# YukeWang96/TC-GNN_ATC23

Hardware: AMD Instinct MI355X
Metric: SpMM/SDDMM GTEPS + GCN/AGNN ms/epoch, Reddit h=64, 1xMI355X (higher is better)
Workload: dtype f16 x f16 -> f32 (MFMA), f32 I/O; 1 GPU; reddit-shape synthetic graph N=232965 nnz=114615892, SpMM D=64 (GCN aggregation, fwd = bwd); tc_blocks_16x8=13626429, parallelism=1 GPU

## Files before the change

tc-gnn_atc23_amd/csrc/tcgnn_device.hip:

```cpp
#include <hip/hip_runtime.h>

#include <algorithm>
#include <atomic>
#include <chrono>
#include <cmath>
#include <cstdint>
#include <cstdlib>
#include <cstring>
#include <mutex>
#include <new>
#include <numeric>
#include <type_traits>
#include <vector>

#include "tcgnn.h"
#include "tcgnn_internal.h"

using namespace tcgnn;

#define LDS_AS __attribute__((address_space(3)))
#define GLB_AS __attribute__((address_space(1)))

typedef _Float16 half8 __attribute__((ext_vector_type(8)));
typedef _Float16 half4 __attribute__((ext_vector_type(4)));
typedef float floatx4 __attribute__((ext_vector_type(4)));
typedef __attribute__((__vector_size__(4 * sizeof(__fp16)))) __fp16 fp16x4_raw;

#define HIP_TRY(expr)                                                                       \
    do {                                                                                    \
        hipError_t e_ = (expr);                                                             \
        if (e_ != hipSuccess) return fail(TCGNN_ERR_HIP, "%s -> %s", #expr, hipGetErrorString(e_)); \
    } while (0)
static inline int hip_rc(hipError_t e) { return e == hipErrorOutOfMemory ? TCGNN_ERR_OOM : TCGNN_ERR_HIP; }
template <class T> struct DevBuf {
    T* ptr = nullptr;
    size_t bytes = 0;
    DevBuf() = default;
    DevBuf(DevBuf&& o) noexcept : ptr(o.ptr), bytes(o.bytes) { o.ptr = nullptr; o.bytes = 0; }
    DevBuf& operator=(DevBuf&& o) noexcept { std::swap(ptr, o.ptr); std::swap(bytes, o.bytes); return *this; }
    DevBuf(const DevBuf&) = delete;
    DevBuf& operator=(const DevBuf&) = delete;
    ~DevBuf() { reset(); }
    hipError_t alloc(size_t count) {
        reset();
        const hipError_t e = hipMalloc(&ptr, count * sizeof(T));
        if (e == hipSuccess) bytes = count * sizeof(T); else ptr = nullptr;
        return e;
    }
    void reset() { if (ptr) (void)hipFree(ptr); ptr = nullptr; bytes = 0; }
    size_t release(T*& to) { const size_t b = bytes; to = ptr; ptr = nullptr; bytes = 0; return b; }
    operator T*() const { return ptr; }
};

struct tcgnn_plan {
    int32_t N = 0, nw = 0, nw_eff = 0;
    double near_frac = 0;
    int32_t Nc = 0;
    int32_t row_off = 0;
    int32_t* d_sym = nullptr;
    int64_t E = 0, tc_blocks = 0, total_wb = 0, max_wb = 0;
    int canonical = 0, waves = 1;
    int32_t max_degree = 0;
    const int32_t *rowptr = nullptr, *col = nullptr, *bp = nullptr, *e2c = nullptr, *e2r = nullptr;
    int64_t* d_wb_ptr = nullptr;
    int32_t* d_order = nullptr;
    int32_t* d_cols = nullptr;
    uint32_t* d_mask = nullptr;
    int32_t* d_ebase = nullptr;
    int32_t nbuckets = 0, bucket_rows = 0;
    uint32_t* d_bptr = nullptr;
    int32_t num_cus = 256;
    size_t bytes = 0;
    uint32_t* d_stage = nullptr;
    struct SyncTables {
        int32_t S = 0, R = 0, nwx = 0, kmax = 0, fb_shift = 0;
        uint32_t* d_T = nullptr;
        int32_t* d_nk = nullptr;
        double hot_frac = 0, avg_k = 0;
        int32_t max_k = 0;
        bool ok = false;
    } sync;
    struct CellStream {
        std::atomic<int32_t> nranges{0};
        int32_t nwg = 0;
        int64_t tiles = 0;
        int32_t* d_order = nullptr;
        int32_t npairs = 0;
        int32_t* d_rbase = nullptr;
        int32_t* d_rlist = nullptr;
        uint32_t* d_rl2 = nullptr;
        int32_t dense_entries = 0;
        int64_t cold_tiles = 0, hot_cols = 0, cold_cols = 0, cold_max = 0;
        uint32_t* d_parts = nullptr;
        int32_t nsplit = 0;
        int64_t* d_cold_ptr = nullptr;
        int32_t* d_cold_cols = nullptr;
        uint32_t* d_cold_mask = nullptr;
        uint32_t* d_cell_ptr = nullptr;
        uint32_t* d_cell_tiles = nullptr;
        int32_t flat_tpc = 0;
        uint32_t* d_flat = nullptr;
        int32_t* d_wcold_ptr = nullptr;
        uint32_t* d_wcold = nullptr;
        int32_t* d_eidx = nullptr;
        int32_t* d_cold_eidx = nullptr;
        uint16_t* d_eidx16 = nullptr;
        uint16_t* d_cold_eidx16 = nullptr;
    };
    CellStream lds[7];
    int64_t* d_xwb_ptr = nullptr;
    int32_t* d_xcols = nullptr;
    uint32_t* d_xmask = nullptr;
    int32_t* d_xeidx = nullptr;
    int64_t total_xwb = 0;
    std::atomic<int8_t> val_choice{-1};
    mutable std::atomic<int8_t> lds_choice[65];
    tcgnn_plan() { for (auto& c : lds_choice) c.store(-1, std::memory_order_relaxed); }
    mutable std::vector<hipEvent_t> ev;
    mutable std::atomic<int> ev_used{0};
    mutable std::atomic<const char*> last_kernel{""};
    std::atomic<int8_t> spmm_mode{-1}, range_guard{-1};
    std::vector<int32_t> h_bp;
    mutable std::atomic<int> lds_extra[2] = {{-1}, {-1}};
};

struct KernelTimer {
    const tcgnn_plan* p; hipStream_t s; int slot = -1;
    KernelTimer(const tcgnn_plan* plan, hipStream_t stream, const char* kernel_name = nullptr) : p(plan), s(stream) {
        if (p && kernel_name) p->last_kernel.store(kernel_name, std::memory_order_relaxed);
        if (p && !p->ev.empty()) {
            const int k = p->ev_used.fetch_add(1, std::memory_order_relaxed);
            if (2 * k + 1 < (int)p->ev.size()) { slot = k; (void)hipEventRecord(p->ev[2 * slot], s); }
            else p->ev_used.store((int)p->ev.size() / 2, std::memory_order_relaxed);
        }
    }
    void stop() { if (slot >= 0) { (void)hipEventRecord(p->ev[2 * slot + 1], s); slot = -1; } }
    ~KernelTimer() { stop(); }
};

static inline int round_up(int x, int m) { return (x + m - 1) / m * m; }
static constexpr int kXcds = 8;

__device__ __forceinline__ float relu_if(int on, float v) { return on ? fmaxf(v, 0.0f) : v; }
struct Epi { const float* rs; const float* bias; };
__device__ __forceinline__ float epi_apply(int relu, const Epi& e, int64_t row, int col, float v) {
#pragma clang fp contract(off)
    if (e.rs) v = v * e.rs[row];
    if (e.bias) v = v + e.bias[col];
    return relu_if(relu, v);
}

template <int NT>
struct TileImage {
    static constexpr int C = 2 * NT;
    __device__ static __forceinline__ int slot(int row, int c) {
        if constexpr (NT == 1) {
            int rp = (row & ~0xC) | ((row & 4) << 1) | ((row & 8) >> 1);
            return rp * 2 + c;
        } else if constexpr (NT == 2) {
            return row * 4 + (c ^ (((row >> 3) & 1) << 1));
        } else if constexpr (NT == 4) {
            return row * 8 + (c ^ ((((row >> 1) & 1) << 1) | (((row >> 3) & 1) << 2)));
        } else if constexpr (NT == 8) {
            return row * 16 + (c ^ (((row & 3) | (((row >> 3) & 1) << 2)) << 1));
        } else {
            return row * C + c;
        }
    }
    __device__ static __forceinline__ void unslot(int q, int& row, int& c) {
        if constexpr (NT == 1) {
            int rp = q >> 1;
            row = (rp & ~0xC) | ((rp & 4) << 1) | ((rp & 8) >> 1);
            c = q & 1;
        } else if constexpr (NT == 2) {
            row = q >> 2;
            c = (q & 3) ^ (((row >> 3) & 1) << 1);
        } else if constexpr (NT == 4) {
            row = q >> 3;
            c = (q & 7) ^ ((((row >> 1) & 1) << 1) | (((row >> 3) & 1) << 2));
        } else if constexpr (NT == 8) {
            row = q >> 4;
            c = (q & 15) ^ (((row & 3) | (((row >> 3) & 1) << 2)) << 1);
        } else {
            row = q / C;
            c = q - row * C;
        }
    }
};

__device__ __forceinline__ half4 lds_read_tr16(const char* p) {
    fp16x4_raw v = __builtin_amdgcn_ds_read_tr16_b64_v4f16((LDS_AS fp16x4_raw*)(p));
    return __builtin_bit_cast(half4, v);
}

#include "tcgnn_launch.inc"
#include "tcgnn_stage.inc"
#include "tcgnn_pack.inc"

#include "tcgnn_gather_spmm.inc"
#include "tcgnn_sync_walk.inc"


#include "tcgnn_small_spmm.inc"
#include "tcgnn_lds_spmm.inc"
#include "tcgnn_lds_flat.inc"
#include "tcgnn_lds_val.inc"

#include "tcgnn_sddmm.inc"

#include "tcgnn_agnn.inc"

#include "tcgnn_small_fallback.inc"
#include "tcgnn_heads.inc"

#include "tcgnn_transpose.inc"

#include "tcgnn_edge_softmax.inc"
#include "tcgnn_gat.inc"
#include "tcgnn_segment_max.inc"
#include "tcgnn_segment_stats.inc"
#include "tcgnn_gatv2.inc"

static const char* test_knob(const char* name) { return getenv(name); }
static int verbose_level() { const char* e = getenv("TCGNN_VERBOSE"); return e ? atoi(e) : 0; }
static constexpr int g_bucket_min_tiles = 2;
static int g_lds_auto = [] { const char* e = test_knob("TCGNN_LDS_AUTO"); return e ? atoi(e) : 1; }();
#ifdef TCGNN_DEBUG_TIMERS
static int g_lds_dbg = [] { const char* e = getenv("TCGNN_LDS_DBG"); return e ? atoi(e) : 0; }();
#else
static constexpr int g_lds_dbg = 0;
#endif
static constexpr int g_lds_fill_quota = 1;
static int g_spmm_mode = [] { const char* e = getenv("TCGNN_SPMM_MODE"); return e ? atoi(e) : 0; }();
static inline int spmm_mode_of(const tcgnn_plan* p) { const int m = p ? (int)p->spmm_mode.load(std::memory_order_relaxed) : -1; return m >= 0 ? m : g_spmm_mode; }
static constexpr size_t kBlockedMinBytes = 6u << 20;
static constexpr size_t kRangeTargetBytes = 1u << 20;

static constexpr int kAgnnMaxSlices = 16;
static size_t agnn_partial_bytes(const tcgnn_plan* plan) {
    const size_t slots = std::max<size_t>((size_t)std::max(plan->nw_eff, 1), (size_t)kAgnnMaxSlices * (((size_t)std::max(plan->nw_eff, 1) + 3) / 4));
    return (slots * sizeof(double) + 255) / 256 * 256;
}

static bool has_locality(const tcgnn_plan* plan) { return plan->near_frac > 0.5; }
static bool windows_balanced(const tcgnn_plan* plan) {
    return plan->nw_eff > 0 && plan->max_wb * (int64_t)plan->nw_eff <= 8 * std::max<int64_t>(plan->total_wb, 1);
}
static bool ranges_fit_l2(const tcgnn_plan* plan, size_t x16_bytes) {
    return plan->nbuckets > 0 && x16_bytes / (size_t)plan->nbuckets <= ((size_t)8 << 20) && plan->nw_eff >= 32 * plan->num_cus;
}
static bool range_walk_pays(const tcgnn_plan* plan, size_t x16_bytes) {
    return x16_bytes > kBlockedMinBytes && windows_balanced(plan) && ranges_fit_l2(plan, x16_bytes) && !has_locality(plan);
}
static int range_count(const tcgnn_plan* plan, size_t x16_bytes, size_t range_bytes) {
    if (const char* e = test_knob("TCGNN_RANGE_KB")) range_bytes = (size_t)atol(e) << 10;
    int nranges = 1;
    while (nranges < plan->nbuckets && x16_bytes / nranges > range_bytes) nranges <<= 1;
    return nranges;
}
static int check_output_aligned(const char* call, const char* what, const void* p) {
    if (reinterpret_cast<uintptr_t>(p) & 15) return fail(TCGNN_ERR_INVALID_ARG, "%s: %s must be 16-byte aligned, got %p", call, what, p);
    return TCGNN_OK;
// ... 201 lines not shown
```

tc-gnn_atc23_amd/csrc/tcgnn_lds_flat.inc:

```

struct SpmmFlatArgs {
    const uint32_t* blocks;
    const int32_t* order;
    const _Float16* x16;
    const uint32_t* hdr;
    float* y;
    int32_t N, D, stride , chunk0, xrows, nw, nwg;
    int32_t dbg, relu;
    const int32_t* rbase;
    const uint32_t* rl2;
    int32_t nent;
    const float* w;
    int32_t dout, accumulate;
    int32_t fill_quota;
    const int32_t* wcold_ptr;
    const uint32_t* wcold;
    SpmmSmallArgs fb;
};

typedef uint32_t uintx2 __attribute__((ext_vector_type(2)));

template <int T> struct FlatMeta { uint32_t idw[T]; uint32_t mk[(T + 3) / 4]; };
template <int T> __device__ __forceinline__ void flat_meta_block(uint32_t idaddr, uint32_t maddr, FlatMeta<T>& m) {
    if constexpr (T == 8) {
// ... 6 lines not shown
#pragma unroll
        for (int k = 0; k < 4; ++k) { m.idw[k] = q0[k]; m.idw[4 + k] = q1[k]; }
        m.mk[0] = b[0]; m.mk[1] = b[1];
    } else if constexpr (T == 4) {
        uintx4 q0; uint32_t b;
        asm volatile("ds_read_b128 %0, %2\n\t"
                     "ds_read_b32 %1, %3\n\t"
                     "s_waitcnt lgkmcnt(0)"
                     : "=&v"(q0), "=&v"(b) : "v"(idaddr), "v"(maddr) : "memory");
#pragma unroll
        for (int k = 0; k < 4; ++k) m.idw[k] = q0[k];
        m.mk[0] = b;
    } else {
        static_assert(T == 16, "flat streams: 4, 8 or 16 tiles per wavefront and range");
        uintx4 q0, q1, q2, q3, b;
        asm volatile("ds_read_b128 %0, %5\n\t"
                     "ds_read_b128 %1, %5 offset:16\n\t"
                     "ds_read_b128 %2, %5 offset:32\n\t"
                     "ds_read_b128 %3, %5 offset:48\n\t"
                     "ds_read_b128 %4, %6\n\t"
                     "s_waitcnt lgkmcnt(0)"
                     : "=&v"(q0), "=&v"(q1), "=&v"(q2), "=&v"(q3), "=&v"(b) : "v"(idaddr), "v"(maddr) : "memory");
#pragma unroll
        for (int k = 0; k < 4; ++k) { m.idw[k] = q0[k]; m.idw[4 + k] = q1[k]; m.idw[8 + k] = q2[k]; m.idw[12 + k] = q3[k]; m.mk[k] = b[k]; }
    }
}

template <int NT, int PLANE> __device__ __forceinline__ void flat_issue(uint32_t ad0, uint32_t ad1, half4* nlo, half4* nhi) {
    if constexpr (NT == 1) lds_flat_issue1<PLANE>(ad0, ad1, nlo, nhi);
    else if constexpr (NT == 2) lds_flat_issue2<PLANE>(ad0, ad1, nlo, nhi);
    else if constexpr (NT == 3) lds_flat_issue3<PLANE>(ad0, ad1, nlo, nhi);
    else lds_flat_issue4<PLANE>(ad0, ad1, nlo, nhi);
}
template <int NT, int PLANE> __device__ __forceinline__ void flat_step(uint32_t ad0, uint32_t ad1, half4* nlo, half4* nhi, half4* clo, half4* chi) {
    if constexpr (NT == 1) lds_flat_step1<PLANE>(ad0, ad1, nlo, nhi, clo, chi);
    else if constexpr (NT == 2) lds_flat_step2<PLANE>(ad0, ad1, nlo, nhi, clo, chi);
    else if constexpr (NT == 3) lds_flat_step3<PLANE>(ad0, ad1, nlo, nhi, clo, chi);
    else lds_flat_step4<PLANE>(ad0, ad1, nlo, nhi, clo, chi);
}
template <int NT, int PLANE> __device__ __forceinline__ void flat_step_if(uint32_t on, uint32_t ad0, uint32_t ad1, half4* nlo, half4* nhi, half4* clo, half4* chi) {
    if constexpr (NT == 1) lds_flat_step_if1<PLANE>(on, ad0, ad1, nlo, nhi, clo, chi);
    else if constexpr (NT == 2) lds_flat_step_if2<PLANE>(on, ad0, ad1, nlo, nhi, clo, chi);
    else if constexpr (NT == 3) lds_flat_step_if3<PLANE>(on, ad0, ad1, nlo, nhi, clo, chi);
    else lds_flat_step_if4<PLANE>(on, ad0, ad1, nlo, nhi, clo, chi);
}
template <int NT> __device__ __forceinline__ void flat_drain(half4* clo, half4* chi) {
    if constexpr (NT == 1) lds_flat_drain1(clo, chi);
    else if constexpr (NT == 2) lds_flat_drain2(clo, chi);
    else if constexpr (NT == 3) lds_flat_drain3(clo, chi);
    else lds_flat_drain4(clo, chi);
}

template <int B> __device__ __forceinline__ half8 flat_afrag(uint32_t mkw) {
    const uint32_t mm = __builtin_amdgcn_perm(mkw, mkw, 0x0c000c00u | (uint32_t)B | ((uint32_t)B << 16));
    uintx4 q;
#pragma unroll
    for (int j = 0; j < 4; ++j) {
        const ushort2v k = {(unsigned short)(1u << (14 - 2 * j)), (unsigned short)(1u << (13 - 2 * j))};
        q[j] = __builtin_bit_cast(uint32_t, (ushort2v)(__builtin_bit_cast(ushort2v, mm) * k)) & 0x40004000u;
    }
    return __builtin_bit_cast(half8, q);
}

typedef short short2v __attribute__((ext_vector_type(2)));
template <int B> __device__ __forceinline__ half8 flat_amask(uint32_t mkw) {
    const uint32_t mm = __builtin_amdgcn_perm(mkw, mkw, 0x0c000c00u | (uint32_t)B | ((uint32_t)B << 16));
    uintx4 q;
#pragma unroll
    for (int j = 0; j < 4; ++j) {
        const ushort2v k = {(unsigned short)(1u << (15 - 2 * j)), (unsigned short)(1u << (14 - 2 * j))};
        const short2v sh = __builtin_bit_cast(short2v, (ushort2v)(__builtin_bit_cast(ushort2v, mm) * k)) >> (short2v){15, 15};
        q[j] = __builtin_bit_cast(uint32_t, sh);
    }
    return __builtin_bit_cast(half8, q);
}

__global__ __launch_bounds__(256) void flat_transpose_kernel(const uint32_t* __restrict__ tiles, uint32_t* __restrict__ blocks, int64_t nblocks, int32_t T,
                                                             const uint32_t* __restrict__ rl2 = nullptr) {
    const int64_t k = (int64_t)blockIdx.x * blockDim.x + threadIdx.x;
    const int words = 32 * T;
    if (k >= nblocks * words) return;
    const int64_t blk = k / words;
    if (rl2 && (rl2[(blk / kLdsWaves) * 4] >> 31)) { blocks[k] = tiles[k]; return; }
    const int o = (int)(k - blk * words);
    const uint32_t* src = tiles + blk * words;
    uint32_t v;
    if (o < 16 * T) {
        const int c = o / T, x = o % T;
        v = src[x * 32 + c];
    } else {
        v = 0u;
        const int b0 = (o - 16 * T) * 4;
#pragma unroll
        for (int q = 0; q < 4; ++q) {
            const int b = b0 + q, lane = b / T, x = b % T;
            const int g = lane >> 4, i = lane & 15;
            v |= ((src[x * 32 + 16 + i] >> (8 * g)) & 0xffu) << (8 * q);
        }
    }
    blocks[k] = v;
}

__global__ __launch_bounds__(256) void flat_cold_records_kernel(const uint32_t* __restrict__ list, int64_t n, const int32_t* __restrict__ ccols, const uint32_t* __restrict__ cmask,
                                                                uint32_t* __restrict__ rec) {
    const int64_t k = (int64_t)blockIdx.x * blockDim.x + threadIdx.x;
    if (k >= n * 64) return;
    const uint32_t e = list[k >> 6];
    const int64_t t = e & 0x0fffffffu;
    const int o = (int)(k & 63);
    rec[k] = o < 32 ? ((uint32_t)ccols[t * kWbCols + o] | (e & 0xf0000000u)) : (o < 48 ? cmask[t * kWinRows + (o - 32)] : 0u);
}

__device__ __forceinline__ uint32_t lane_id_now() {
    uint32_t l;
    asm volatile("v_mbcnt_lo_u32_b32 %0, -1, 0\n\tv_mbcnt_hi_u32_b32 %0, -1, %0" : "=v"(l));
    return l;
}

template <int NT, int BR>
struct FlatRangeFiller {
    static constexpr int IPP = BR / 32, TOTAL = NT * IPP, kMinFillers = 12, MAXC = (TOTAL + kMinFillers - 1) / kMinFillers;
    __amdgpu_buffer_rsrc_t xrsrc;
    uint32_t zrow;
    int rank, nfill, plane0, nplanes, xrows;
    __device__ __forceinline__ FlatRangeFiller(const _Float16* x16p, int xrows_, int plane0_, int nplanes_, int rank_, int nfill_, int lane) {
        xrsrc = __builtin_amdgcn_make_buffer_rsrc((void*)x16p, (short)32, nplanes_ * xrows_, 0x00020000);
        zrow = (uint32_t)(xrows_ - 1);
        (void)lane;
        rank = rank_; nfill = nfill_; plane0 = plane0_; nplanes = nplanes_; xrows = xrows_;
    }
    __device__ __forceinline__ void fill(int r0, uint32_t buf) const {
        if (rank < 0) return;
        const uint32_t l2 = lane_id_now();
        const uint32_t lrow = l2 >> 1;
        const int hoff = (int)(l2 & 1u) * 16;
#pragma unroll
        for (int q = 0; q < MAXC; ++q) {
            const int k = rank + nfill * q;
            if (k < TOTAL) {
                const int plane = k / IPP, blk = k - plane * IPP;
                const bool real_plane = plane0 + plane < nplanes;
                const uint32_t row = (uint32_t)(blk * 32) + lrow;
                const uint32_t want = (uint32_t)r0 + row;
                const uint32_t srow = (row < (uint32_t)(BR - 8) && real_plane && want < zrow) ? want : zrow;
                const int pbase = real_plane ? (plane0 + plane) * xrows : 0;
                __builtin_amdgcn_struct_ptr_buffer_load_lds(xrsrc, (LDS_AS void*)(uintptr_t)(buf + (uint32_t)plane * (BR * 32u) + (uint32_t)blk * 1024u), 16,
                                                            pbase + (int)srow, hoff, 0, 0, 0);
            }
        }
    }
};

static constexpr bool flat_dense_ok(int nt, int maxw, int tpc) { return tpc == 1 && nt <= 2 && maxw * tpc <= 15; }
static constexpr int flat_lds_main(int nt, int maxw, int tpc) { return 2 * nt * lds_buf_rows(nt, maxw) * 32 + kLdsWaves * 2 * (maxw * tpc * 128); }
static constexpr bool flat_cold_fits(int nt, int maxw, int tpc) { return flat_lds_main(nt, maxw, tpc) + kLdsWaves * nt * 1024 <= 160 * 1024; }
static constexpr int flat_lds_bytes(int nt, int maxw, int tpc) { return flat_lds_main(nt, maxw, tpc) + (flat_cold_fits(nt, maxw, tpc) ? kLdsWaves * nt * 1024 : (flat_dense_ok(nt, maxw, tpc) ? 128 : 0)); }

#define TCGNN_KERNEL_NAME spmm_lds_flat_kernel
#define TCGNN_KERNEL_PARAM const SpmmFlatArgs a
#define TCGNN_KERNEL_PROLOGUE
#define TCGNN_KERNEL_STORE(relu, row, col, v) relu_if(relu, v)
#include "tcgnn_lds_flat_kernel.inc"
#undef TCGNN_KERNEL_NAME
#undef TCGNN_KERNEL_PARAM
#undef TCGNN_KERNEL_PROLOGUE
#undef TCGNN_KERNEL_STORE
struct SpmmFlatEpiArgs { SpmmFlatArgs a; Epi epi; };
#define TCGNN_KERNEL_NAME spmm_lds_flat_epi_kernel
#define TCGNN_KERNEL_PARAM const SpmmFlatEpiArgs e
#define TCGNN_KERNEL_PROLOGUE const SpmmFlatArgs& a = e.a;
#define TCGNN_KERNEL_STORE(relu, row, col, v) epi_apply(relu, e.epi, row, col, v)
#include "tcgnn_lds_flat_kernel.inc"
#undef TCGNN_KERNEL_NAME
#undef TCGNN_KERNEL_PARAM
#undef TCGNN_KERNEL_PROLOGUE
#undef TCGNN_KERNEL_STORE

template __global__ void spmm_lds_flat_kernel<1, 4, 1, false, false>(const SpmmFlatArgs);
template __global__ void spmm_lds_flat_kernel<1, 4, 1, false, true>(const SpmmFlatArgs);
template __global__ void spmm_lds_flat_kernel<2, 4, 1, false, false>(const SpmmFlatArgs);
template __global__ void spmm_lds_flat_kernel<2, 4, 1, false, true>(const SpmmFlatArgs);
template __global__ void spmm_lds_flat_kernel<3, 4, 1, false, false>(const SpmmFlatArgs);
template __global__ void spmm_lds_flat_kernel<4, 4, 1, false, false>(const SpmmFlatArgs);
template __global__ void spmm_lds_flat_kernel<1, 8, 1, false, false>(const SpmmFlatArgs);
template __global__ void spmm_lds_flat_kernel<1, 8, 1, false, true>(const SpmmFlatArgs);
template __global__ void spmm_lds_flat_kernel<2, 8, 1, false, false>(const SpmmFlatArgs);
template __global__ void spmm_lds_flat_kernel<2, 8, 1, false, true>(const SpmmFlatArgs);
template __global__ void spmm_lds_flat_kernel<1, 4, 2, false, false>(const SpmmFlatArgs);
template __global__ void spmm_lds_flat_kernel<2, 4, 2, false, false>(const SpmmFlatArgs);
template __global__ void spmm_lds_flat_kernel<3, 4, 2, false, false>(const SpmmFlatArgs);
template __global__ void spmm_lds_flat_kernel<4, 4, 2, false, false>(const SpmmFlatArgs);
template __global__ void spmm_lds_flat_kernel<1, 8, 2, false, false>(const SpmmFlatArgs);
template __global__ void spmm_lds_flat_kernel<2, 8, 2, false, false>(const SpmmFlatArgs);
#ifdef TCGNN_DEBUG_TIMERS
template __global__ void spmm_lds_flat_kernel<1, 4, 1, true, false>(const SpmmFlatArgs);
template __global__ void spmm_lds_flat_kernel<1, 4, 1, true, true>(const SpmmFlatArgs);
template __global__ void spmm_lds_flat_kernel<2, 4, 1, true, false>(const SpmmFlatArgs);
template __global__ void spmm_lds_flat_kernel<2, 4, 1, true, true>(const SpmmFlatArgs);
template __global__ void spmm_lds_flat_kernel<3, 4, 1, true, false>(const SpmmFlatArgs);
template __global__ void spmm_lds_flat_kernel<4, 4, 1, true, false>(const SpmmFlatArgs);
template __global__ void spmm_lds_flat_kernel<1, 8, 1, true, false>(const SpmmFlatArgs);
template __global__ void spmm_lds_flat_kernel<1, 8, 1, true, true>(const SpmmFlatArgs);
template __global__ void spmm_lds_flat_kernel<2, 8, 1, true, false>(const SpmmFlatArgs);
template __global__ void spmm_lds_flat_kernel<2, 8, 1, true, true>(const SpmmFlatArgs);
template __global__ void spmm_lds_flat_kernel<1, 4, 2, true, false>(const SpmmFlatArgs);
template __global__ void spmm_lds_flat_kernel<2, 4, 2, true, false>(const SpmmFlatArgs);
template __global__ void spmm_lds_flat_kernel<3, 4, 2, true, false>(const SpmmFlatArgs);
template __global__ void spmm_lds_flat_kernel<4, 4, 2, true, false>(const SpmmFlatArgs);
template __global__ void spmm_lds_flat_kernel<1, 8, 2, true, false>(const SpmmFlatArgs);
template __global__ void spmm_lds_flat_kernel<2, 8, 2, true, false>(const SpmmFlatArgs);
#endif

template __global__ void spmm_lds_flat_epi_kernel<1, 4, 1, false, false>(const SpmmFlatEpiArgs);
template __global__ void spmm_lds_flat_epi_kernel<1, 4, 1, false, true>(const SpmmFlatEpiArgs);
template __global__ void spmm_lds_flat_epi_kernel<2, 4, 1, false, false>(const SpmmFlatEpiArgs);
template __global__ void spmm_lds_flat_epi_kernel<2, 4, 1, false, true>(const SpmmFlatEpiArgs);
template __global__ void spmm_lds_flat_epi_kernel<3, 4, 1, false, false>(const SpmmFlatEpiArgs);
template __global__ void spmm_lds_flat_epi_kernel<4, 4, 1, false, false>(const SpmmFlatEpiArgs);
template __global__ void spmm_lds_flat_epi_kernel<1, 8, 1, false, false>(const SpmmFlatEpiArgs);
template __global__ void spmm_lds_flat_epi_kernel<1, 8, 1, false, true>(const SpmmFlatEpiArgs);
template __global__ void spmm_lds_flat_epi_kernel<2, 8, 1, false, false>(const SpmmFlatEpiArgs);
template __global__ void spmm_lds_flat_epi_kernel<2, 8, 1, false, true>(const SpmmFlatEpiArgs);
template __global__ void spmm_lds_flat_epi_kernel<1, 4, 2, false, false>(const SpmmFlatEpiArgs);
template __global__ void spmm_lds_flat_epi_kernel<2, 4, 2, false, false>(const SpmmFlatEpiArgs);
template __global__ void spmm_lds_flat_epi_kernel<3, 4, 2, false, false>(const SpmmFlatEpiArgs);
template __global__ void spmm_lds_flat_epi_kernel<4, 4, 2, false, false>(const SpmmFlatEpiArgs);
template __global__ void spmm_lds_flat_epi_kernel<1, 8, 2, false, false>(const SpmmFlatEpiArgs);
template __global__ void spmm_lds_flat_epi_kernel<2, 8, 2, false, false>(const SpmmFlatEpiArgs);

static constexpr LaunchGeom flat_geom(int nt, int maxw, int tpc) { return {kLdsWaves * 64, flat_lds_bytes(nt, maxw, tpc), kLdsWaves / 4, maxw}; }

template <int NT, int MAXW, int TPC, bool DBG, bool WITH_DENSE>
static hipError_t launch_flat_dbg(const SpmmFlatArgs& args, int nchunks, hipStream_t stream, const Epi& epi) {
    constexpr LaunchGeom g = flat_geom(NT, MAXW, TPC);
    const dim3 grid((unsigned)args.nwg, (unsigned)nchunks);
    if constexpr (DBG) return launch_kernel<spmm_lds_flat_kernel<NT, MAXW, TPC, true, WITH_DENSE>, g.lds_bytes>(grid, g, stream, args);
    else return launch_plain_or_twin<spmm_lds_flat_kernel<NT, MAXW, TPC, false, WITH_DENSE>, spmm_lds_flat_epi_kernel<NT, MAXW, TPC, false, WITH_DENSE>, g.lds_bytes>(grid, g, stream, args, epi);
}
template <int NT, int MAXW, int TPC, bool DBG>
static hipError_t launch_flat_dense(const SpmmFlatArgs& args, int nchunks, hipStream_t stream, bool dense, const Epi& epi) {
    if constexpr (flat_dense_ok(NT, MAXW, TPC)) {
        if (dense) return launch_flat_dbg<NT, MAXW, TPC, DBG, true>(args, nchunks, stream, epi);
    }
    return launch_flat_dbg<NT, MAXW, TPC, DBG, false>(args, nchunks, stream, epi);
}
template <int NT, int MAXW, int TPC>
static hipError_t launch_flat_one(const SpmmFlatArgs& args, int nchunks, hipStream_t stream, bool dense, const Epi& epi) {
#ifdef TCGNN_DEBUG_TIMERS
    if (args.dbg) return launch_flat_dense<NT, MAXW, TPC, true>(args, nchunks, stream, dense, epi);
#endif
    return launch_flat_dense<NT, MAXW, TPC, false>(args, nchunks, stream, dense, epi);
}
template <int TPC>
static hipError_t launch_flat_tpc(int maxw, int nt, const SpmmFlatArgs& args, int nchunks, hipStream_t stream, bool dense, const Epi& epi) {
    if (maxw == kLdsMaxW2) return with_width<2>(nt, [&](auto NT) { return launch_flat_one<NT, kLdsMaxW2, TPC>(args, nchunks, stream, dense, epi); });
    return with_width<4>(nt, [&](auto NT) { return launch_flat_one<NT, kLdsMaxW, TPC>(args, nchunks, stream, dense, epi); });
}
static hipError_t launch_flat_any(int maxw, int nt, int tpc, const SpmmFlatArgs& args, int nchunks, hipStream_t stream, bool dense,
                                  const Epi& epi = Epi{nullptr, nullptr}) {
    return tpc == 2 ? launch_flat_tpc<2>(maxw, nt, args, nchunks, stream, dense, epi) : launch_flat_tpc<1>(maxw, nt, args, nchunks, stream, dense, epi);
}

struct ColdPlanarArgs {
    const int64_t* cold_ptr;
    const int32_t* ccols;
    const uint32_t* cmask;
    const _Float16* x16;
    const uint32_t* hdr;
    float* y;
    int32_t N, D, xrows, nw, col0, ncols, relu;
    Epi epi;
};
__global__ __launch_bounds__(256, 2) void spmm_cold_planar_kernel(const ColdPlanarArgs a) {
    const int lane = threadIdx.x & 63, wave = threadIdx.x >> 6;
    const int w = blockIdx.x * 4 + wave;
    if (w >= a.nw) return;
    const int64_t t0 = a.cold_ptr[w], t1 = a.cold_ptr[w + 1];
    if (t0 == t1 && !a.relu && !a.epi.rs && !a.epi.bias) return;
    const int r = lane >> 2, q = lane & 3;
    const int plane = (a.col0 >> 4) + (int)blockIdx.y * 4 + q;
    const bool live = plane * 16 < a.col0 + a.ncols && plane * 16 < ((a.D + 15) & ~15);
    float acc[16];
#pragma unroll
    for (int e = 0; e < 16; ++e) acc[e] = 0.0f;
    const int zrow = a.xrows - 1;
    const half8* xp = reinterpret_cast<const half8*>(a.x16 + (int64_t)(live ? plane : 0) * a.xrows * 16);
    int32_t cv = 0; uint32_t mv = 0u;
    if (t0 < t1) { cv = a.ccols[t0 * kWbCols + (lane & 31)]; mv = a.cmask[t0 * kWinRows + r]; }
    for (int64_t t = t0; t < t1; ++t) {
    if (range_is_wide(a.hdr, 0)) return;
        int32_t cvn = 0; uint32_t mvn = 0u;
        if (t + 1 < t1) { cvn = a.ccols[(t + 1) * kWbCols + (lane & 31)]; mvn = a.cmask[(t + 1) * kWinRows + r]; }
        while (__any(mv != 0u)) {
            int c[2];
#pragma unroll
            for (int it = 0; it < 2; ++it) {
                const bool v = mv != 0u;
                const int k = v ? __builtin_ctz(mv) : 0;
                mv &= mv - 1u;
                const int cc = __shfl(cv, k);
                c[it] = (v && live && cc < zrow) ? cc : zrow;
            }
            half8 x[2][2];
#pragma unroll
            for (int it = 0; it < 2; ++it) { x[it][0] = xp[(int64_t)c[it] * 2]; x[it][1] = xp[(int64_t)c[it] * 2 + 1]; }
#pragma unroll
            for (int it = 0; it < 2; ++it)
#pragma unroll
                for (int e = 0; e < 8; ++e) { acc[e] += (float)x[it][0][e]; acc[8 + e] += (float)x[it][1][e]; }
        }
        cv = cvn; mv = mvn;
    }
    const int64_t row = (int64_t)w * kWinRows + r;
    if (!live || row >= a.N) return;
    const float inv = pow2f(-scale_exp_from_bits(a.hdr[kHdrMaxX]));
    float* dst = a.y + row * a.D + plane * 16;
    if (plane * 16 + 16 <= a.D && (a.D & 3) == 0) {
#pragma unroll
        for (int e4 = 0; e4 < 4; ++e4) {
            float4 v = reinterpret_cast<float4*>(dst)[e4];
            const int c0 = plane * 16 + 4 * e4;
            v.x = epi_apply(a.relu, a.epi, row, c0, v.x + acc[4 * e4] * inv); v.y = epi_apply(a.relu, a.epi, row, c0 + 1, v.y + acc[4 * e4 + 1] * inv);
            v.z = epi_apply(a.relu, a.epi, row, c0 + 2, v.z + acc[4 * e4 + 2] * inv); v.w = epi_apply(a.relu, a.epi, row, c0 + 3, v.w + acc[4 * e4 + 3] * inv);
            reinterpret_cast<float4*>(dst)[e4] = v;
        }
    } else {
#pragma unroll
        for (int e = 0; e < 16; ++e)
            if (plane * 16 + e < a.D) dst[e] = epi_apply(a.relu, a.epi, row, plane * 16 + e, dst[e] + acc[e] * inv);
    }
}
```

tc-gnn_atc23_amd/csrc/tcgnn_lds_flat_kernel.inc:

```
template <int NT, int MAXW, int TPC, bool DBG, bool WITH_DENSE>
__global__ __launch_bounds__(kLdsWaves * 64) void TCGNN_KERNEL_NAME(TCGNN_KERNEL_PARAM) {
    TCGNN_KERNEL_PROLOGUE
    if (range_is_wide(a.hdr, 0)) { lds_own_fallback(a.fb); return; }
    const int dbg = DBG ? a.dbg : 0;
    constexpr int kLdsBufRows = lds_buf_rows(NT, MAXW), kLdsRows = kLdsBufRows - 8;
    constexpr int T = MAXW * TPC, PADB = T * 128, kLdsChunkDims = lds_chunk_dims(MAXW);
    static_assert(NT * MAXW <= 16, "accumulators: NT * MAXW * 4 VGPRs");
    extern __shared__ __attribute__((aligned(16))) char smem[];
    constexpr int PLANEB = kLdsBufRows * 32, BUFB = NT * PLANEB;
    const int lane = threadIdx.x & 63;
    const int wave = __builtin_amdgcn_readfirstlane(threadIdx.x >> 6);
    const int g = lane >> 4, i = lane & 15;
    const int wg = blockIdx.x;
    const int chunk_id = a.chunk0 + (int)blockIdx.y;
    const int coloff = chunk_id * kLdsChunkDims;
    const uint32_t lds0 = (uint32_t)(uintptr_t)((LDS_AS char*)smem);
    const uint32_t pad0 = lds0 + 2 * BUFB + (uint32_t)wave * (2 * PADB);
    const int kx = scale_exp_from_bits(a.hdr[kHdrMaxX]);

    floatx4 acc[MAXW][NT];
#pragma unroll
    for (int j = 0; j < MAXW; ++j) {
#pragma unroll
        for (int s = 0; s < NT; ++s) acc[j][s] = floatx4{0.f, 0.f, 0.f, 0.f};
    }
    const bool last_valid = MAXW == 1 || __builtin_amdgcn_readfirstlane(a.order[cell_position(wg, wave, MAXW - 1, MAXW)]) >= 0;
    const uint32_t last_on = (uint32_t)__builtin_amdgcn_readfirstlane(last_valid ? 1 : 0);
    const uint32_t lanebase = lds0 + (uint32_t)(i & 3) * 8u;
    const uint32_t idoff = (uint32_t)(4 * g + (i >> 2)) * (uint32_t)(T * 4);
    const uint32_t moff = (uint32_t)(64 * T) + (uint32_t)lane * (uint32_t)T;
    int fill_rank = wave, fill_n = kLdsWaves;
    {
        LDS_AS uint32_t* flags = (LDS_AS uint32_t*)smem;
        if (lane == 0) flags[wave] = last_valid ? 1u : 0u;
        __syncthreads();
        const uint32_t full = (uint32_t)(__ballot(lane < kLdsWaves && flags[lane < kLdsWaves ? lane : 0] != 0u) & 0xffffull);
        __syncthreads();
        const uint32_t light = ~full & 0xffffu;
        const int nlight = __builtin_popcount(light);
        if (nlight >= FlatRangeFiller<NT, kLdsBufRows>::kMinFillers && nlight < kLdsWaves && a.fill_quota) {
            fill_n = nlight;
            fill_rank = last_valid ? -1 : __builtin_popcount(light & ((1u << wave) - 1u));
        }
    }
    const FlatRangeFiller<NT, kLdsBufRows> filler(a.x16, a.xrows, chunk_id * (kLdsChunkDims / 16), a.stride, fill_rank, fill_n, lane);
    const int rb = a.rbase[wg], nr = a.rbase[wg + 1] - rb;
    const char* const bb0 = reinterpret_cast<const char*>(a.blocks) + ((int64_t)rb * kLdsWaves + wave) * PADB;
    const uint32_t lane16 = (uint32_t)lane * 16u;
    auto meta_dma = [&](int r, uint32_t padaddr) {
        const char* src = bb0 + (int64_t)r * (kLdsWaves * PADB);
#pragma unroll
        for (int q = 0; q < (PADB + 1023) / 1024; ++q)
            if (lane16 + 1024u * q < (uint32_t)PADB)
                __builtin_amdgcn_global_load_lds((GLB_AS const void*)(src + 1024 * q + lane16), (LDS_AS void*)(uintptr_t)(padaddr + 1024u * q), 16, 0, 0);
    };
    const uint32_t* const rlp = a.rl2 + (int64_t)rb * 4;
    auto load_info = [&](int r_) -> uintx2 { return *reinterpret_cast<const uintx2*>(rlp + (int64_t)r_ * 4); };
    const uint32_t* const dscp = a.rl2 + (int64_t)a.nent * 4 + ((int64_t)rb * kLdsWaves + wave);
    auto load_desc = [&](int r_) -> uint32_t { return dscp[(int64_t)r_ * kLdsWaves]; };
    constexpr bool DENSE = WITH_DENSE && flat_dense_ok(NT, MAXW, TPC);

    constexpr bool CAN_COLD = flat_cold_fits(NT, MAXW, TPC);
    const uint32_t cbuf = lds0 + (uint32_t)flat_lds_main(NT, MAXW, TPC) + (uint32_t)wave * (NT * 1024u);
    int cold_c = 0, cold_n = 0, j_cur = 0;
    bool have_g = false, have_n = false;
    uint32_t cid_n = 0u, mw_n = 0u, mw_cur = 0u;
    auto cold_request = [&]() {
        have_n = cold_c < cold_n;
        if (have_n) {
            const uint32_t* rec = a.wcold + (int64_t)cold_c * 64;
            const uint32_t l2 = lane_id_now();
            cid_n = rec[l2 >> 1]; mw_n = rec[32 + (l2 & 15u)];
            ++cold_c;
        }
    };
    auto cold_step = [&]() {
        if (have_g) {
            const uint32_t l2 = lane_id_now();
            const uint32_t ad0 = cbuf + ((l2 >> 4) * 8u + ((l2 & 15u) >> 2)) * 32u + (l2 & 3u) * 8u;
            half4 lo[NT], hi[NT];
            flat_issue<NT, 1024>(ad0, ad0 + 128u, lo, hi);
            flat_drain<NT>(lo, hi);
            const half8 af = afrag_from_byte((mw_cur >> (8 * g)) & 0xffu);
            floatx4 cacc[NT];
#pragma unroll
            for (int s = 0; s < NT; ++s) {
                const half8 bf = __builtin_shufflevector(lo[s], hi[s], 0, 1, 2, 3, 4, 5, 6, 7);
                cacc[s] = __builtin_amdgcn_mfma_f32_16x16x32_f16(af, bf, floatx4{0.f, 0.f, 0.f, 0.f}, 0, 0, 0);
            }
#pragma unroll
            for (int jj = 0; jj < MAXW; ++jj) {
                if (j_cur == jj) {
#pragma unroll
                    for (int s = 0; s < NT; ++s) acc[jj][s] += cacc[s];
                }
            }
        }
        have_g = have_n;
        if (have_n) {
            const int plane0 = chunk_id * (kLdsChunkDims / 16);
#pragma unroll
            for (int s = 0; s < NT; ++s) {
                const bool real = plane0 + s < a.stride;
                const int64_t recrow = real ? (int64_t)(plane0 + s) * a.xrows + (int64_t)(cid_n & 0x0fffffffu) : (int64_t)a.xrows - 1;
                const char* src = reinterpret_cast<const char*>(a.x16) + (recrow << 5) + (lane & 1) * 16;
                __builtin_amdgcn_global_load_lds((GLB_AS const void*)src, (LDS_AS void*)(uintptr_t)(cbuf + (uint32_t)s * 1024u), 16, 0, 0);
            }
            mw_cur = mw_n;
            j_cur = __builtin_amdgcn_readfirstlane((int)(cid_n >> 28));
        }
        cold_request();
    };
    if constexpr (CAN_COLD) {
        if (a.wcold_ptr) {
            cold_c = a.wcold_ptr[wg * kLdsWaves + wave];
            cold_n = a.wcold_ptr[wg * kLdsWaves + wave + 1];
            cold_request();
        }
    }
    uint32_t ew0 = 0u, ew1 = 0u, ew2 = ~0u;
    uintx2 einfo = {0u, ~0u};
    if (nr > 0) {
        const uintx2 e0 = load_info(0);
        ew0 = (uint32_t)__builtin_amdgcn_readfirstlane((int)e0[0]);
        ew2 = (uint32_t)__builtin_amdgcn_readfirstlane((int)e0[1]);
        meta_dma(0, pad0);
        if (nr > 1) meta_dma(1, pad0 + PADB);
        filler.fill((int)(ew0 & 0x3fffffffu) * kLdsRows, lds0);
        einfo = load_info(nr > 1 ? 1 : 0);
    }
    wait_vm0();
    __syncthreads();
    uint32_t ph[4] = {0, 0, 0, 0};
    uint32_t buf = 0u;
    int r = 0;
    uint32_t t0 = 0u, t1 = 0u, t2 = 0u;
    auto entry_top = [&]() {
        t0 = (dbg & 16) ? (uint32_t)__builtin_readcyclecounter() : 0u;
        if (ew2 != ~0u && !(dbg & 1)) filler.fill((int)((dbg & 128) ? (ew2 & 7u) : ew2) * kLdsRows, lds0 + (buf ^ 1u) * BUFB);
        t1 = (dbg & 16) ? (uint32_t)__builtin_readcyclecounter() : 0u;
    };
    uint32_t dnext = 0u;
    auto entry_end = [&](uint32_t padaddr, bool dense_phase) {
        t2 = (dbg & 16) ? (uint32_t)__builtin_readcyclecounter() : 0u;
        wait_vm0();
        const bool more = r + 2 < nr;
        ew0 = (uint32_t)__builtin_amdgcn_readfirstlane((int)einfo[0]);
        ew2 = (uint32_t)__builtin_amdgcn_readfirstlane((int)einfo[1]);
        if (dense_phase) ew1 = (uint32_t)__builtin_amdgcn_readfirstlane((int)dnext);
        if (ew0 & 0x40000000u) buf ^= 1u;
        if constexpr (CAN_COLD) { if (have_g || have_n) cold_step(); }
        if (more) {
            einfo = load_info(r + 2);
            if (dense_phase) dnext = load_desc(r + 2);
            if (!(dbg & 4)) meta_dma(r + 2, padaddr);
        }
        const uint32_t t3 = (dbg & 16) ? (uint32_t)__builtin_readcyclecounter() : 0u;
        if (!(dbg & 8)) __builtin_amdgcn_s_barrier();
        if (dbg & 16) { const uint32_t t4 = (uint32_t)__builtin_readcyclecounter(); ph[0] += t1 - t0; ph[1] += t2 - t1; ph[2] += t3 - t2; ph[3] += t4 - t3; }
    };
    for (; r < nr && !(ew0 >> 31); ++r) {
        entry_top();
        const uint32_t padaddr = pad0 + (uint32_t)(r & 1) * PADB, bb = lanebase + buf * BUFB;
        if (!(dbg & 2)) {
            FlatMeta<T> m;
            flat_meta_block<T>(padaddr + idoff, padaddr + moff, m);
            constexpr bool PIPE = NT <= 3;
            constexpr int SETS = PIPE ? 2 : 1;
            half4 lo[SETS][NT], hi[SETS][NT];
            if constexpr (PIPE) flat_issue<NT, PLANEB>(bb + (m.idw[0] & 0xffffu), bb + (m.idw[0] >> 16), lo[0], hi[0]);
#pragma unroll
            for (int x = 0; x < T; ++x) {
                if (x / TPC == MAXW - 1 && !last_valid) break;
                if (x % TPC == 0 && !(dbg & 32)) set_wave_priority(3 - (x / TPC) * 4 / MAXW);
                const int cs = PIPE ? (x & 1) : 0;
                if constexpr (!PIPE) { flat_issue<NT, PLANEB>(bb + (m.idw[x] & 0xffffu), bb + (m.idw[x] >> 16), lo[0], hi[0]); flat_drain<NT>(lo[0], hi[0]); }
                else if (x + 1 < T && (x + 1) / TPC == MAXW - 1 && x / TPC != MAXW - 1)
                    flat_step_if<NT, PLANEB>(last_on, bb + (m.idw[x + 1] & 0xffffu), bb + (m.idw[x + 1] >> 16), lo[(x + 1) & 1], hi[(x + 1) & 1], lo[cs], hi[cs]);
                else if (x + 1 < T) flat_step<NT, PLANEB>(bb + (m.idw[x + 1] & 0xffffu), bb + (m.idw[x + 1] >> 16), lo[(x + 1) & 1], hi[(x + 1) & 1], lo[cs], hi[cs]);
                else flat_drain<NT>(lo[cs], hi[cs]);
                half8 af;
                switch (x & 3) {
                    case 0: af = flat_afrag<0>(m.mk[x >> 2]); break;
                    case 1: af = flat_afrag<1>(m.mk[x >> 2]); break;
                    case 2: af = flat_afrag<2>(m.mk[x >> 2]); break;
                    default: af = flat_afrag<3>(m.mk[x >> 2]); break;
                }
#pragma unroll
                for (int s = 0; s < NT; ++s) {
                    const half8 bf = __builtin_shufflevector(lo[cs][s], hi[cs][s], 0, 1, 2, 3, 4, 5, 6, 7);
                    acc[x / TPC][s] = __builtin_amdgcn_mfma_f32_16x16x32_f16(af, bf, acc[x / TPC][s], 0, 0, 0);
                }
            }
        }
        entry_end(padaddr, false);
    }
    if constexpr (DENSE) {
    if (__builtin_expect(r < nr, 0)) {
        const uint32_t d0 = load_desc(r), d1 = load_desc(r + 1 < nr ? r + 1 : r);
        wait_vm0();
        ew1 = (uint32_t)__builtin_amdgcn_readfirstlane((int)d0);
        dnext = d1;
    }
    for (; __builtin_expect(r < nr, 0); ++r) {
        entry_top();
        const uint32_t padaddr = pad0 + (uint32_t)(r & 1) * PADB, bb = lanebase + buf * BUFB;
        if (!(dbg & 2)) {
            const uint32_t l2 = lane_id_now();
            const uint32_t gd = l2 >> 4, id_ = l2 & 15u;
            uint32_t idaddr = padaddr + (4u * gd + (id_ >> 2)) * 4u, maddr = padaddr + 64u + id_ * 4u + gd, idw, mb;
            lds_cell_ids(idaddr, maddr, idw, mb);
#pragma unroll
            for (int j = 0; j < MAXW; ++j) {
                const int nj = (int)((ew1 >> (4 * j)) & 15u);
                if (nj) {
                    floatx4 cacc[NT];
#pragma unroll
                    for (int s = 0; s < NT; ++s) cacc[s] = floatx4{0.f, 0.f, 0.f, 0.f};
                    for (int t = 0; t < nj; ++t) {
                        const uint32_t ad0 = bb + (idw & 0xffffu), ad1 = bb + (idw >> 16);
                        const half8 af = afrag_from_byte(mb);
                        half4 lo[NT], hi[NT];
                        uint32_t nidw, nmb;
                        lds_cell_block<NT, PLANEB>(ad0, ad1, idaddr, maddr, lo, hi, nidw, nmb);
#pragma unroll
                        for (int s = 0; s < NT; ++s) {
                            const half8 bf = __builtin_shufflevector(lo[s], hi[s], 0, 1, 2, 3, 4, 5, 6, 7);
                            cacc[s] = __builtin_amdgcn_mfma_f32_16x16x32_f16(af, bf, cacc[s], 0, 0, 0);
                        }
                        idw = nidw; mb = nmb;
                        idaddr += 128u; maddr += 128u;
                    }
#pragma unroll
                    for (int s = 0; s < NT; ++s) acc[j][s] += cacc[s];
                }
            }
        }
        entry_end(padaddr, true);
    }
    }
    if (!(dbg & 32)) __builtin_amdgcn_s_setprio(0);
    if constexpr (CAN_COLD) {
        while (have_g || have_n) { wait_vm0(); cold_step(); }
    }
    if (dbg & 16) {
        if (wg == 0 && blockIdx.y == 0 && lane == 0) {
#pragma unroll
            for (int k = 0; k < 4; ++k) a.y[wave * 8 + k] = (float)ph[k];
            a.y[wave * 8 + 7] = (float)(nr * T);
        }
        return;
    }

    const float inv1 = pow2f(-kx - 1);
    int wj[MAXW];
#pragma unroll
    for (int j = 0; j < MAXW; ++j) wj[j] = __builtin_amdgcn_readfirstlane(a.order[cell_position(wg, wave, j, MAXW)]);
    if (a.w) {
        __syncthreads();
        constexpr int DIN = NT * 16, LDP = DIN + 1;
        float* scratch = reinterpret_cast<float*>(smem) + wave * (16 * LDP);
        const int din = a.D - coloff < DIN ? a.D - coloff : DIN;
        const int tiles = (a.dout + 15) >> 4;
#pragma unroll
        for (int j = 0; j < MAXW; ++j) {
            if (wj[j] < 0) continue;
            __builtin_amdgcn_fence(__ATOMIC_RELEASE, "wavefront"); __builtin_amdgcn_wave_barrier();
#pragma unroll
            for (int s = 0; s < NT; ++s)
#pragma unroll
                for (int ii = 0; ii < 4; ++ii) scratch[(4 * g + ii) * LDP + 16 * s + i] = acc[j][s][ii] * inv1;
            __builtin_amdgcn_fence(__ATOMIC_RELEASE, "wavefront"); __builtin_amdgcn_wave_barrier();
            const int64_t row0 = (int64_t)wj[j] * kWinRows + 4 * g;
            for (int t = 0; t < tiles; ++t) {
                const floatx4 c = dense_update_tile(scratch, LDP, din, a.w, coloff, a.dout, t, g, i);
                const int colg = 16 * t + i;
                if (colg < a.dout) {
#pragma unroll
                    for (int ii = 0; ii < 4; ++ii) {
                        if (row0 + ii >= a.N) continue;
                        float* dst = a.y + (row0 + ii) * (int64_t)a.dout + colg;
                        if (a.accumulate) atomicAdd(dst, c[ii]);
                        else *dst = relu_if(a.relu, c[ii]);
                    }
                }
            }
        }
        return;
    }
#pragma unroll
    for (int j = 0; j < MAXW; ++j) {
        if (wj[j] < 0) continue;
        const int64_t row0 = (int64_t)wj[j] * kWinRows + 4 * g;
#pragma unroll
        for (int s = 0; s < NT; ++s) {
            const int colg = coloff + 16 * s + i;
            if (colg < a.D) {
#pragma unroll
                for (int ii = 0; ii < 4; ++ii)
                    if (row0 + ii < a.N) a.y[(row0 + ii) * a.D + colg] = TCGNN_KERNEL_STORE(a.relu, row0 + ii, colg, acc[j][s][ii] * inv1);
            }
        }
    }
}
```

tc-gnn_atc23_amd/csrc/tcgnn_lds_plan.inc:

```
static int g_lds_maxw = [] { const char* e = test_knob("TCGNN_LDS_MAXW"); const int v = e ? atoi(e) : 0; return (v == 4 || v == 8) ? v : 0; }();
struct LdsPass { int maxw, nt, chunk0, nchunks; };
static int lds_passes(int dpad, LdsPass (&passes)[2]) {
    int n = 0;
    if (g_lds_maxw) {
        const int cd = lds_chunk_dims(g_lds_maxw);
        if (dpad / cd) passes[n++] = {g_lds_maxw, cd / 16, 0, dpad / cd};
        if (dpad % cd) passes[n++] = {g_lds_maxw, (dpad % cd) / 16, dpad / cd, 1};
    } else {
        const int full = dpad / 64, rem = (dpad % 64) / 16;
        if (full || rem == 3) passes[n++] = {kLdsMaxW2, 2, 0, 2 * (full + (rem == 3 ? 1 : 0))};
        if (rem && rem != 3) passes[n++] = {kLdsMaxW, rem, full, 1};
    }
    return n;
}
static bool lds_has_hubs(const tcgnn_plan* p) {
    int64_t mx = 0;
    for (int w = 0; w < p->nw_eff; ++w) mx = std::max<int64_t>(mx, p->h_bp[(size_t)w]);
    return mx * p->nw_eff > 4 * std::max<int64_t>(p->tc_blocks, 1);
}
enum { kPlaceLocal = 0, kPlaceLocalSplit = 1, kPlaceGlobal = 2 };
static int lds_place_forced() {
    const char* env = test_knob("TCGNN_LDS_PLACE");
    if (!env) return -1;
    return !strcmp(env, "global") ? kPlaceGlobal : (!strcmp(env, "localsplit") ? kPlaceLocalSplit : kPlaceLocal);
}
static int lds_buf_rows_for_maxw(int maxw) { return maxw == kLdsMaxW2 ? 768 : 512; }
static double lds_window_weight(const tcgnn_plan* p, int w, double nranges_d) {
    const double cols = 8.0 * std::max(p->h_bp[(size_t)w], 1);
    return std::ceil(cols / 32.0 + nranges_d * (1.0 - std::exp(-cols / nranges_d)));
}
static int lds_workgroups_unsplit(const tcgnn_plan* p, int maxw, int extra_slots) {
    const int per_wg = kLdsWaves * maxw;
    const int64_t slots = (int64_t)p->nw_eff + extra_slots;
    int nwg = (int)((slots + per_wg - 1) / per_wg);
    const int cu_target = maxw == kLdsMaxW2 ? std::max(1, p->num_cus / 2) : p->num_cus;
    if (nwg < cu_target) nwg = std::max(nwg, std::min(cu_target, (p->nw_eff + kLdsWaves - 1) / kLdsWaves));
    return nwg;
}
static constexpr int kLdsMaxParts = 8, kLdsMaxFollowers = 32;
static int lds_split_parts(const tcgnn_plan* p, int maxw, std::vector<uint8_t>* parts, const std::vector<double>* exact = nullptr) {
    const int nw = p->nw_eff;
    if (parts) parts->assign((size_t)nw, 1);
    if (nw <= 0 || !lds_has_hubs(p)) return 0;
    const double nranges_d = std::max(1.0, std::ceil((double)p->Nc / (lds_buf_rows_for_maxw(maxw) - 8)));
    auto weight = [&](int w) { return exact ? (*exact)[(size_t)w] : lds_window_weight(p, w, nranges_d); };
    double total = 0;
    for (int w = 0; w < nw; ++w) total += weight(w);
    const double share = total / ((double)lds_workgroups_unsplit(p, maxw, 0) * kLdsWaves);
    int extra = 0;
    for (int w = 0; w < nw; ++w) {
        const double wt = weight(w);
        if (wt <= 1.5 * share) continue;
        const int k = (int)std::min<double>(kLdsMaxParts, std::ceil(wt / share));
        if (k < 2) continue;
        if (parts) (*parts)[(size_t)w] = (uint8_t)k;
        extra += k - 1;
    }
    return extra;
}
static int lds_workgroups(const tcgnn_plan* p, int maxw) {
    const int which = maxw == kLdsMaxW2 ? 1 : 0;
    int extra = p->lds_extra[which].load(std::memory_order_relaxed);
    if (extra < 0) { extra = lds_split_parts(p, maxw, nullptr); p->lds_extra[which].store(extra, std::memory_order_relaxed); }
    return lds_workgroups_unsplit(p, maxw, extra);
}

static double lds_estimate_us(const tcgnn_plan* p, int dpad) {
    LdsPass passes[2];
    const int np = lds_passes(dpad, passes);
    const double cols_per_window = 32.0 * (double)p->total_wb / std::max(p->nw_eff, 1);
    double t = 25.0;
    for (int i = 0; i < np; ++i) {
        const int maxw = passes[i].maxw, nt = passes[i].nt;
        const int rows = lds_stream_buf_rows(lds_stream_of(nt, maxw)) - 8;
        const double nranges = std::ceil((double)p->Nc / rows);
        const int nwg = lds_workgroups(p, maxw);
        const double rounds = std::ceil((double)nwg * passes[i].nchunks / std::max(p->num_cus, 1));
        const double c = cols_per_window / nranges;
        const double tiles_per_cell = c <= 24.0 ? 1.0 - std::exp(-c) : c / 32.0 + 0.5;
        const double windows_per_wave = (double)p->nw_eff / ((double)nwg * kLdsWaves);
        static const double fixed4[4] = {0.47, 0.60, 0.89, 1.16};
        const double a = maxw == kLdsMaxW2 ? 0.80 : fixed4[std::min(nt, 4) - 1];
        t += rounds * nranges * (a + 0.135 * windows_per_wave * tiles_per_cell);
    }
    return t;
}
static double gather_estimate_us(const tcgnn_plan* p, int dpad) {
    const double image = ((double)p->Nc + 1) * x16_pitch(dpad) * 2.0;
    double ps;
    if (image <= (double)kBlockedMinBytes) ps = 4.6 + std::max(0, dpad - 16) * (1.8 / 48.0);
    else if (dpad <= 32) ps = 8.5;
    else if (dpad <= 64) ps = 8.5 + (dpad - 32) * (1.1 / 32.0);
    else ps = 9.6 + (dpad - 64) * (6.9 / 64.0);
    if (image > 45.0e6) ps *= std::pow(image / 45.0e6, 0.3);
    return 20.0 + (double)p->E * ps * 1e-6;
}
static bool lds_chosen(const tcgnn_plan* p, int dpad) {
    if (!g_lds_auto || p->nw_eff <= 0 || p->total_wb <= 0) return false;
    const int k = dpad / 16;
    if (k <= 64 && p->lds_choice[k] >= 0) return p->lds_choice[k] != 0;
    LdsPass passes[2];
    const int np = lds_passes(dpad, passes);
    double cells = 0;
    for (int i = 0; i < np; ++i) {
        const int rows = lds_stream_buf_rows(lds_stream_of(passes[i].nt, passes[i].maxw)) - 8;
        cells += (double)lds_workgroups(p, passes[i].maxw) * kLdsWaves * passes[i].maxw * std::ceil((double)p->Nc / rows);
    }
    const bool yes = cells < 2.0e8 && lds_estimate_us(p, dpad) <= 0.95 * gather_estimate_us(p, dpad);
    if (k <= 64) p->lds_choice[k] = yes ? 1 : 0;
    return yes;
}

static bool lds_deal_workgroup(int g, int maxw, const std::vector<int32_t>& items, const std::vector<uint8_t>& k, const std::vector<double>& wt,
                               std::vector<int32_t>& order, std::vector<uint32_t>& parts_out, int& nsplit) {
    double load[kLdsWaves] = {0};
    int used[kLdsWaves] = {0};
    uint32_t next_fol = 0;
    for (const int32_t w : items) {
        const int kk = k.empty() ? 1 : k[(size_t)w];
        uint32_t taken = 0u;
        const uint32_t fol0 = next_fol;
        for (int part = 0; part < kk; ++part) {
            int best = -1;
            for (int v = 0; v < kLdsWaves; ++v)
                if (used[v] < maxw && !((taken >> v) & 1u) && (best < 0 || load[v] < load[best])) best = v;
            if (best < 0)
                for (int v = 0; v < kLdsWaves; ++v) if (used[v] < maxw && (best < 0 || load[v] < load[best])) best = v;
            if (best < 0) return false;
            const size_t pos = (size_t)cell_position(g, best, used[best], maxw);
            order[pos] = w;
            if (kk > 1) parts_out[pos] = (uint32_t)part | ((uint32_t)kk << 8) | ((part == 0 ? fol0 : fol0 + (uint32_t)part - 1u) << 16);
            taken |= 1u << best;
            load[best] += wt[(size_t)w] / kk;
            ++used[best];
        }
        if (kk > 1) { next_fol += (uint32_t)kk - 1u; ++nsplit; }
    }
    return true;
}
static bool lds_place_windows(const tcgnn_plan* p, int nwg, int maxw, std::vector<int32_t>& order, std::vector<uint32_t>& parts_out, int& nsplit,
                              const std::vector<double>& exact, int mode) {
    const int nw = p->nw_eff, cap = kLdsWaves * maxw;
    order.assign((size_t)nwg * cap, -1);
    parts_out.clear();
    nsplit = 0;
    if (mode == kPlaceGlobal) {
        std::vector<uint8_t> k;
        const int extra = lds_split_parts(p, maxw, &k, &exact);
        const std::vector<double>& wt = exact;
        std::vector<int32_t> idx((size_t)nw);
        std::iota(idx.begin(), idx.end(), 0);
        std::stable_sort(idx.begin(), idx.end(), [&](int32_t x, int32_t y) { return wt[(size_t)x] > wt[(size_t)y]; });
        std::vector<double> wg_load((size_t)nwg, 0.0);
        std::vector<int> wg_free((size_t)nwg, cap), wg_fol((size_t)nwg, 0);
// ... 16 lines not shown
        if (extra > 0) parts_out.assign((size_t)nwg * cap, 0u); else k.clear();
        for (int g = 0; g < nwg; ++g)
            if (!lds_deal_workgroup(g, maxw, wg_items[(size_t)g], k, wt, order, parts_out, nsplit)) return false;
        if (nsplit == 0) parts_out.clear();
        return true;
    }
    const std::vector<double>& wt = exact;
    double total = 0;
    for (int w = 0; w < nw; ++w) total += wt[(size_t)w];
    std::vector<uint8_t> k;
    const int extra = mode == kPlaceLocalSplit ? lds_split_parts(p, maxw, &k, &exact) : 0;
    if (extra > 0) {
        int64_t slots = 0;
        for (int w = 0; w < nw; ++w) slots += k[(size_t)w];
        for (int level = kLdsMaxParts; slots > (int64_t)nwg * cap && level > 1; --level)
            for (int w = 0; w < nw && slots > (int64_t)nwg * cap; ++w)
                if (k[(size_t)w] == level) { --k[(size_t)w]; --slots; }
        parts_out.assign((size_t)nwg * cap, 0u);
    } else k.clear();
    std::vector<int64_t> slots_after((size_t)nw + 1, 0);
    for (int w = nw - 1; w >= 0; --w) slots_after[(size_t)w] = slots_after[(size_t)w + 1] + (k.empty() ? 1 : k[(size_t)w]);
    std::vector<int32_t> blk;
    double acc = 0;
    int wg = 0, blk_slots = 0, blk_fol = 0;
    bool ok = true;
    auto deal = [&]() {
        double mx = 0, sum = 0;
        for (const int32_t w : blk) { mx = std::max(mx, wt[(size_t)w]); sum += wt[(size_t)w]; }
        if (mx * (double)blk.size() > 1.5 * sum) {
            const double heavy = 2.0 * sum / (double)blk.size();
            auto mid = std::stable_partition(blk.begin(), blk.end(), [&](int32_t x) { return wt[(size_t)x] > heavy; });
            std::stable_sort(blk.begin(), mid, [&](int32_t x, int32_t y) { return wt[(size_t)x] > wt[(size_t)y]; });
        }
        ok = lds_deal_workgroup(wg, maxw, blk, k, wt, order, parts_out, nsplit) && ok;
        blk.clear(); blk_slots = 0; blk_fol = 0;
    };
    for (int w = 0; w < nw && ok; ++w) {
        int kk = k.empty() ? 1 : k[(size_t)w];
        const int wgs_left0 = nwg - (wg + 1);
        if (kk > 1 && blk_fol + kk - 1 > kLdsMaxFollowers) { k[(size_t)w] = 1; kk = 1; }
        if (blk_slots + kk > cap) {
            if (wgs_left0 > 0 && slots_after[(size_t)w] <= (int64_t)wgs_left0 * cap) { deal(); ++wg; }
            else { if (kk > 1) k[(size_t)w] = 1; kk = 1; }
            if (blk_slots + kk > cap) { ok = false; break; }
        }
        blk.push_back(w);
        blk_slots += kk; blk_fol += kk - 1;
        acc += wt[(size_t)w];
        const int wgs_left = nwg - (wg + 1);
        const bool full = blk_slots == cap;
        const bool heavy_enough = acc >= total * (double)(wg + 1) / nwg;
        if (wgs_left > 0 && (full || (heavy_enough && slots_after[(size_t)w + 1] <= (int64_t)wgs_left * cap))) { deal(); ++wg; }
    }
    if (ok && !blk.empty()) deal();
    if (nsplit == 0) parts_out.clear();
    return ok;
}


struct CellPlacement {
    int mode = kPlaceLocal, nsplit = 0;
    uint32_t hot_min = 1u;
    double est_us = 0;
    std::vector<int32_t> sorder;
    std::vector<uint32_t> sparts, paircols, pairmax, pairover, pairtiles;
    DevBuf<uint32_t> d_cellcols, d_firstq, d_parts;
    DevBuf<int32_t> d_sorder;
};
struct FlatEntries {
    std::vector<int32_t> ent2, nd, wg_first;
    std::vector<uint32_t> xbase, rl2;
    int64_t nentries = 0;
};
static FlatEntries flat_entries(int nwg, int maxw, const std::vector<int32_t>& rbase, const std::vector<int32_t>& rlist, const std::vector<uint32_t>& cnt,
                                const std::vector<uint32_t>& dense_mx, bool dense_on, bool records) {
    FlatEntries f;
    const int64_t npairs = rbase[(size_t)nwg];
    f.ent2.assign((size_t)npairs * 2 + 2, -1); f.nd.assign((size_t)npairs, 0); f.wg_first.assign((size_t)nwg + 1, 0);
    int32_t eidx = 0;
    for (int wg = 0; wg < nwg; ++wg) {
        f.wg_first[(size_t)wg] = eidx;
        for (int64_t k = rbase[(size_t)wg]; k < rbase[(size_t)wg + 1]; ++k) f.ent2[(size_t)k * 2] = eidx++;
        for (int64_t k = rbase[(size_t)wg]; k < rbase[(size_t)wg + 1]; ++k) {
            f.nd[(size_t)k] = dense_on ? (int32_t)((dense_mx[(size_t)k] + maxw - 1) / maxw) : 0;
            f.ent2[(size_t)k * 2 + 1] = f.nd[(size_t)k] ? eidx : -1;
            eidx += f.nd[(size_t)k];
        }
    }
    f.wg_first[(size_t)nwg] = eidx;
    f.nentries = eidx;
    if (!records) return f;
    const std::vector<int32_t>& nd = f.nd;
    std::vector<uint32_t>& xbase = f.xbase;
    if (dense_on) {
        xbase.assign((size_t)(npairs * kLdsWaves * maxw), 0u);
        for (int64_t k = 0; k < npairs; ++k) {
            if (!nd[(size_t)k]) continue;
            for (int v = 0; v < kLdsWaves; ++v) {
                uint32_t run = 0;
                for (int j = 0; j < maxw; ++j) { const size_t c = (size_t)((k * kLdsWaves + v) * maxw + j); xbase[c] = run; run += cnt[c] > 1u ? cnt[c] - 1u : 0u; }
            }
        }
    }
    const int64_t nrec = std::max<int64_t>(f.nentries, 1);
    f.rl2.assign((size_t)nrec * (4 + kLdsWaves), 0u);
    auto put = [&](int64_t en, int v, uint32_t w0, uint32_t w1, uint32_t w2) {
        uint32_t* q = &f.rl2[(size_t)(en * 4)];
        q[0] = w0; q[1] = w2; q[3] = 0u;
        f.rl2[(size_t)(nrec * 4 + en * kLdsWaves + v)] = w1;
    };
    for (int wg = 0; wg < nwg; ++wg)
        for (int64_t en = f.wg_first[(size_t)wg]; en < f.wg_first[(size_t)wg + 1]; ++en) f.rl2[(size_t)(en * 4 + 2)] = (uint32_t)(rbase[(size_t)wg + 1] - rbase[(size_t)wg]);
    for (int wg = 0; wg < nwg; ++wg) {
        const int64_t k0 = rbase[(size_t)wg], k1 = rbase[(size_t)wg + 1];
        std::vector<int64_t> dk;
        for (int64_t k = k0; k < k1; ++k) if (nd[(size_t)k]) dk.push_back(k);
        for (int64_t k = k0; k < k1; ++k) {
            const uint32_t r = (uint32_t)rlist[(size_t)k];
            const uint32_t nextr = k + 1 < k1 ? (uint32_t)rlist[(size_t)k + 1] : (dk.empty() ? 0xffffffffu : (uint32_t)rlist[(size_t)dk[0]]);
            for (int v = 0; v < kLdsWaves; ++v) put(f.ent2[(size_t)k * 2], v, r | (k > k0 ? 0x40000000u : 0u), 0u, nextr);
        }
        for (size_t gi = 0; gi < dk.size(); ++gi) {
            const int64_t k = dk[gi];
            const uint32_t r = (uint32_t)rlist[(size_t)k];
            const uint32_t nextr = gi + 1 < dk.size() ? (uint32_t)rlist[(size_t)dk[gi + 1]] : 0xffffffffu;
            for (int64_t d = 0; d < nd[(size_t)k]; ++d)
                for (int v = 0; v < kLdsWaves; ++v) {
                    uint32_t desc = 0u;
                    for (int j = 0; j < maxw; ++j) {
                        const size_t c = (size_t)((k * kLdsWaves + v) * maxw + j);
                        const int64_t lo = xbase[c], hi = lo + (cnt[c] > 1u ? cnt[c] - 1u : 0u);
                        const int64_t a0 = std::max<int64_t>(lo, d * maxw), a1 = std::min<int64_t>(hi, (d + 1) * maxw);
                        if (a1 > a0) desc |= (uint32_t)(a1 - a0) << (4 * j);
                    }
                    put(f.ent2[(size_t)k * 2 + 1] + d, v, r | 0x80000000u | (d == 0 ? 0x40000000u : 0u), desc, d == 0 ? nextr : 0xffffffffu);
                }
        }
    }
    return f;
}

struct CellBuild {
    tcgnn_plan* p; hipStream_t stream; int slot;
    bool val;
    const int64_t* s_wb; const int32_t* s_cols; const uint32_t* s_mask; const int32_t* s_eidx;
    int maxw, rows, nranges, per_wg, nwg, nw;
    int64_t ncell, npairs_all;
    bool verbose;
    std::vector<double> exact;
    CellPlacement best;
    std::vector<int32_t> kmap, rbase, rlist;
    int64_t npairs = 0, ncell_hot = 0, hot_cols = 0, cold_cols = 0;
    std::vector<uint32_t> cnt;
    std::vector<uint32_t> dense_mx;
    int64_t over_dense = 0, dense_steps = 0, ndense_pairs = 0, ndense_entries = 0;
    int flat_tpc = 0;
    int64_t over_cols = 0;
    FlatEntries ent;
    int64_t ntiles = 0, nwords = 0, cold_tiles = 0, cold_max = 0;
    std::vector<int64_t> cptr;
    std::vector<int32_t> wptr;
    std::vector<uint32_t> wlist;
    DevBuf<int32_t> d_kmap, d_rbase, d_rlist, d_ent, d_ccols, d_eidx, d_cold_eidx, d_wcold_ptr;
    DevBuf<uint32_t> d_cnt, d_tiles, d_flat, d_rl2, d_xbase, d_cmask, d_wcold;
    DevBuf<int64_t> d_cold_ptr;
    bool with_dense() const { return flat_tpc == 1 && ndense_pairs > 0; }
};

static int cells_window_weights(CellBuild& b) {
    const tcgnn_plan* p = b.p;
    b.exact.assign((size_t)p->nw_eff, 1.0);
    DevBuf<uint32_t> d_wt;
    std::vector<uint32_t> h_wt((size_t)p->nw_eff, 0u);
    hipError_t e = d_wt.alloc(h_wt.size());
    if (e == hipSuccess) e = hipMemsetAsync(d_wt, 0, h_wt.size() * sizeof(uint32_t), b.stream);
    if (e == hipSuccess) {
        const int64_t nth = (int64_t)p->nw_eff * b.nranges;
        hipLaunchKernelGGL(window_tiles_kernel, dim3((unsigned)((nth + 255) / 256)), dim3(256), 0, b.stream, b.s_wb, b.s_cols, p->nw_eff, b.nranges, p->Nc, b.rows, d_wt.ptr);
        e = hipGetLastError();
    }
    if (e == hipSuccess) e = hipMemcpyAsync(h_wt.data(), d_wt, h_wt.size() * sizeof(uint32_t), hipMemcpyDeviceToHost, b.stream);
    if (e == hipSuccess) e = hipStreamSynchronize(b.stream);
    if (e != hipSuccess) return fail(hip_rc(e), "window weights: %s", hipGetErrorString(e));
    for (size_t w = 0; w < h_wt.size(); ++w) b.exact[w] = std::max<double>(1.0, h_wt[w]);
    return TCGNN_OK;
}
static hipError_t cells_prepare_placement(const CellBuild& b, int mode, CellPlacement& c) {
    const tcgnn_plan* p = b.p;
    const int nwg = b.nwg, nranges = b.nranges, maxw = b.maxw;
    const int64_t npairs_all = b.npairs_all;
    c.mode = mode;
    if (!lds_place_windows(p, nwg, maxw, c.sorder, c.sparts, c.nsplit, b.exact, mode)) {
        c.mode = kPlaceLocal;
        if (!lds_place_windows(p, nwg, maxw, c.sorder, c.sparts, c.nsplit, b.exact, kPlaceLocal)) return hipErrorInvalidValue;
    }
    c.hot_min = maxw == kLdsMaxW2 ? 1000u : 400u;
    if (spmm_mode_of(p) == 3 || c.mode == kPlaceGlobal) c.hot_min = 1u;
    if (const char* env = test_knob("TCGNN_LDS_HOT_COLS")) c.hot_min = (uint32_t)std::max(1, atoi(env));
    DevBuf<uint32_t> d_pc, d_pm, d_po, d_pt;
    hipError_t e = c.d_cellcols.alloc((size_t)(b.ncell + 1));
    if (e == hipSuccess && c.nsplit > 0) {
        e = c.d_parts.alloc(c.sparts.size());
        if (e == hipSuccess) e = hipMemcpyAsync(c.d_parts, c.sparts.data(), c.sparts.size() * sizeof(uint32_t), hipMemcpyHostToDevice, b.stream);
    }
    if (e == hipSuccess) e = c.d_firstq.alloc((size_t)b.nw * nranges);
    if (e == hipSuccess) e = c.d_sorder.alloc(c.sorder.size());
    if (e == hipSuccess) e = d_pc.alloc((size_t)npairs_all);
    if (e == hipSuccess) e = d_pm.alloc((size_t)npairs_all);
    if (e == hipSuccess) e = d_po.alloc((size_t)npairs_all * 2);
    if (e == hipSuccess) e = d_pt.alloc((size_t)npairs_all);
    if (e == hipSuccess) e = hipMemcpyAsync(c.d_sorder, c.sorder.data(), c.sorder.size() * sizeof(int32_t), hipMemcpyHostToDevice, b.stream);
    if (e == hipSuccess) e = hipMemsetAsync(c.d_cellcols, 0, (size_t)(b.ncell + 1) * sizeof(uint32_t), b.stream);
    c.pairmax.resize((size_t)npairs_all);
    c.paircols.resize((size_t)npairs_all);
    c.pairover.resize((size_t)npairs_all * 2);
    c.pairtiles.resize((size_t)npairs_all);
    if (e == hipSuccess) {
        const int64_t nthreads = (int64_t)b.nw * nranges;
        hipLaunchKernelGGL(cell_count_kernel, dim3((unsigned)((nthreads + 255) / 256)), dim3(256), 0, b.stream, b.s_wb, c.d_sorder.ptr, b.s_cols, b.nw, nwg,
                           nranges, p->Nc, maxw, b.rows, c.d_cellcols.ptr, c.d_firstq.ptr, c.d_parts.ptr);
        hipLaunchKernelGGL(cell_pair_cols_kernel, dim3((unsigned)((npairs_all + 255) / 256)), dim3(256), 0, b.stream, c.d_cellcols.ptr, npairs_all, b.per_wg, maxw, d_pc.ptr, d_pm.ptr,
                           d_po.ptr, d_pt.ptr);
        e = hipGetLastError();
    }
    if (e == hipSuccess) e = hipMemcpyAsync(c.paircols.data(), d_pc, c.paircols.size() * sizeof(uint32_t), hipMemcpyDeviceToHost, b.stream);
    if (e == hipSuccess) e = hipMemcpyAsync(c.pairover.data(), d_po, c.pairover.size() * sizeof(uint32_t), hipMemcpyDeviceToHost, b.stream);
    if (e == hipSuccess) e = hipMemcpyAsync(c.pairtiles.data(), d_pt, c.pairtiles.size() * sizeof(uint32_t), hipMemcpyDeviceToHost, b.stream);
    if (e == hipSuccess) e = hipMemcpyAsync(c.pairmax.data(), d_pm, c.pairmax.size() * sizeof(uint32_t), hipMemcpyDeviceToHost, b.stream);
    if (e == hipSuccess) e = hipStreamSynchronize(b.stream);
    if (e != hipSuccess) return e;
    const double rounds = std::max(1.0, std::ceil((double)nwg * (maxw == kLdsMaxW2 ? 2 : 1) / std::max(p->num_cus, 1)));
    auto estimate = [&](uint32_t hot_min) {
        double worst = 0, cold = 0;
        for (int wg = 0; wg < nwg; ++wg) {
            double t = 0;
            for (int r = 0; r < nranges; ++r) {
                const size_t k = (size_t)wg * nranges + r;
                if (c.paircols[k] >= hot_min) t += 0.80 + 0.135 * c.pairmax[k]; else cold += c.paircols[k];
            }
            worst = std::max(worst, t);
        }
        return worst * rounds + cold * 20e-6;
    };
    c.est_us = estimate(c.hot_min);
    if (b.verbose && c.mode != kPlaceGlobal)
        for (uint32_t h : {1u, 125u, 250u, 500u, 1000u, 2000u}) fprintf(stderr, "[tcgnn]   placement %d, hot threshold %u: estimated %.0f us\n", c.mode, h, estimate(h));
    return hipSuccess;
}
static int cells_choose_placement(CellBuild& b) {
    const int forced = lds_place_forced();
    const bool hubs = lds_has_hubs(b.p);
    hipError_t e = cells_prepare_placement(b, forced >= 0 ? forced : (hubs ? kPlaceGlobal : kPlaceLocal), b.best);
    if (e == hipSuccess && forced < 0 && hubs) {
        CellPlacement other;
        e = cells_prepare_placement(b, kPlaceLocalSplit, other);
        if (b.verbose) fprintf(stderr, "[tcgnn] cell stream %d: estimated %.0f us longest-first over the graph, %.0f us contiguous blocks (+ cold remainder)\n", b.slot, b.best.est_us, other.est_us);
        if (e == hipSuccess && other.est_us < b.best.est_us) std::swap(b.best, other);
    }
    if (e != hipSuccess) return fail(hip_rc(e), "cell table: %s", hipGetErrorString(e));
    return TCGNN_OK;
}
static int cells_hot_pairs(CellBuild& b) {
    const std::vector<uint32_t>& paircols = b.best.paircols;
    hipError_t e = b.d_kmap.alloc((size_t)b.npairs_all);
    if (e != hipSuccess) return fail(hip_rc(e), "cell table: %s", hipGetErrorString(e));
    b.kmap.assign((size_t)b.npairs_all, -1); b.rbase.assign((size_t)b.nwg + 1, 0);
    std::vector<int32_t>& rlist = b.rlist;
    for (int wg = 0; wg < b.nwg; ++wg) {
        b.rbase[(size_t)wg] = (int32_t)rlist.size();
        for (int r = 0; r < b.nranges; ++r) {
            const uint32_t c = paircols[(size_t)wg * b.nranges + r];
            if (c >= b.best.hot_min) { b.kmap[(size_t)wg * b.nranges + r] = (int32_t)rlist.size(); rlist.push_back(r); b.hot_cols += c; }
            else b.cold_cols += c;
        }
    }
    b.rbase[(size_t)b.nwg] = (int32_t)rlist.size();
    b.npairs = (int64_t)rlist.size();
    rlist.resize(rlist.size() + 4, 0);
    b.ncell_hot = b.npairs * b.per_wg;
    e = b.d_cnt.alloc((size_t)(b.ncell_hot + 1));
    if (e == hipSuccess) e = b.d_rbase.alloc(b.rbase.size());
    if (e == hipSuccess) e = b.d_rlist.alloc(rlist.size());
    if (e == hipSuccess) e = hipMemsetAsync(b.d_cnt, 0, (size_t)(b.ncell_hot + 1) * sizeof(uint32_t), b.stream);
    if (e == hipSuccess) e = hipMemcpyAsync(b.d_kmap, b.kmap.data(), b.kmap.size() * sizeof(int32_t), hipMemcpyHostToDevice, b.stream);
    if (e == hipSuccess) e = hipMemcpyAsync(b.d_rbase, b.rbase.data(), b.rbase.size() * sizeof(int32_t), hipMemcpyHostToDevice, b.stream);
    if (e == hipSuccess) e = hipMemcpyAsync(b.d_rlist, rlist.data(), rlist.size() * sizeof(int32_t), hipMemcpyHostToDevice, b.stream);
    if (e != hipSuccess) return fail(hip_rc(e), "cell table: %s", hipGetErrorString(e));
    if (b.ncell > 0) hipLaunchKernelGGL(cell_compact_kernel, dim3((unsigned)((b.ncell + 255) / 256)), dim3(256), 0, b.stream, b.best.d_cellcols.ptr, b.d_kmap.ptr, b.npairs_all, b.per_wg, b.d_cnt.ptr);
    b.cnt.resize((size_t)b.ncell_hot + 1);
    e = hipGetLastError();
    if (e == hipSuccess) e = hipMemcpyAsync(b.cnt.data(), b.d_cnt, b.cnt.size() * sizeof(uint32_t), hipMemcpyDeviceToHost, b.stream);
    if (e == hipSuccess) e = hipStreamSynchronize(b.stream);
    if (e != hipSuccess) return fail(TCGNN_ERR_HIP, "cell count: %s", hipGetErrorString(e));
    return TCGNN_OK;
}
static void cells_dense_pairs(CellBuild& b) {
    const int maxw = b.maxw;
    uint32_t dense_min = 1024u, dense_cell_tiles = 3u;
    if (const char* env = test_knob("TCGNN_LDS_DENSE_COLS")) { dense_min = (uint32_t)std::max(1, atoi(env)); dense_cell_tiles = 0xffffffffu; }
    if (!flat_dense_ok(lds_stream_nt(b.slot), maxw, 1)) dense_min = dense_cell_tiles = 0xffffffffu;
    std::vector<int64_t> kall_of((size_t)b.npairs, 0);
    for (int64_t ka = 0; ka < b.npairs_all; ++ka) if (b.kmap[(size_t)ka] >= 0) kall_of[(size_t)b.kmap[(size_t)ka]] = ka;
    b.dense_mx.assign((size_t)b.npairs, 0u);
    for (int64_t k = 0; k < b.npairs; ++k) {
        if (dense_min == 0xffffffffu && dense_cell_tiles == 0xffffffffu) break;
        uint32_t mx = 0, cell_mx = 0;
        for (int v = 0; v < kLdsWaves; ++v) {
            uint32_t ex = 0;
            for (int j = 0; j < maxw; ++j) { const uint32_t c = b.cnt[(size_t)((k * kLdsWaves + v) * maxw + j)]; ex += c > 1u ? c - 1u : 0u; cell_mx = std::max(cell_mx, c); }
            mx = std::max(mx, ex);
        }
        if (!mx || (b.best.pairover[(size_t)kall_of[(size_t)k]] < dense_min && cell_mx < dense_cell_tiles)) continue;
        b.dense_mx[(size_t)k] = mx;
        b.over_dense += b.best.pairover[(size_t)kall_of[(size_t)k]];
        b.dense_steps += mx; ++b.ndense_pairs; b.ndense_entries += (mx + maxw - 1) / maxw;
    }
}
static void cells_flat_or_ordinary(CellBuild& b) {
    const CellPlacement& best = b.best;
    const int maxw = b.maxw;
    const int64_t npairs = b.npairs, npairs_all = b.npairs_all;
    int64_t classic_tiles = 0, classic_steps = 0, over[2] = {0, 0};
    for (int64_t k = 0; k < npairs_all; ++k)
        if (b.kmap[(size_t)k] >= 0) { classic_tiles += best.pairtiles[(size_t)k]; classic_steps += best.pairmax[(size_t)k];
                                      over[0] += best.pairover[(size_t)k]; over[1] += best.pairover[(size_t)(npairs_all + k)]; }
    const char* fenv = test_knob("TCGNN_LDS_FLAT");
    const int forced_flat = fenv ? atoi(fenv) : -1;
    if (best.nsplit == 0 && npairs > 0 && forced_flat != 0) {
        double best_cost = 0.0;
        for (int tpc = 1; tpc <= 2; ++tpc) {
            if (maxw * tpc > 16 || (b.val && tpc != 1)) break;
            const int64_t kept = tpc == 1 ? b.over_dense : 0, extra_steps = tpc == 1 ? b.dense_steps : 0;
            const bool few_cold = (double)(b.cold_cols + over[tpc - 1] - kept) <= 0.04 * (double)std::max<int64_t>(b.hot_cols + b.cold_cols, 1);
            const bool no_more_steps = (double)(npairs * maxw * tpc + extra_steps) <= 1.2 * (double)std::max<int64_t>(classic_steps, 1);
            if (forced_flat == tpc) { b.flat_tpc = tpc; b.over_cols = over[tpc - 1] - kept; break; }
            if (forced_flat >= 0 || !few_cold || !no_more_steps) continue;
            const double cost = (double)(npairs * maxw * tpc) + (tpc == 1 ? 1.6 * (double)b.dense_steps + 4.0 * (double)b.ndense_entries : 0.0);
            if (!b.flat_tpc || cost < best_cost) { b.flat_tpc = tpc; b.over_cols = over[tpc - 1] - kept; best_cost = cost; }
        }
    }
    if (b.verbose) fprintf(stderr, "[tcgnn] cell stream %d: %lld tiles ordinary, %lld steps of the busiest wavefronts; flat would take %lld steps (+%lld columns cold; %lld dense pairs keep %lld columns "
                                   "in %lld dense entries, %lld steps) / %lld (+%lld): %s\n", b.slot,
                           (long long)classic_tiles, (long long)classic_steps, (long long)(npairs * maxw), (long long)(over[0] - b.over_dense), (long long)b.ndense_pairs, (long long)b.over_dense,
                           (long long)b.ndense_entries, (long long)b.dense_steps, (long long)(2 * npairs * maxw), (long long)over[1],
                           b.flat_tpc ? (b.flat_tpc == 1 ? "flat, 1 tile per cell" : "flat, 2 tiles per cell") : "ordinary");
}
static int cells_hub_row_trial(CellBuild& b) {
    hipError_t e = hipSuccess;
    if (b.with_dense()) {
        b.ent = flat_entries(b.nwg, b.maxw, b.rbase, b.rlist, b.cnt, b.dense_mx, true, false);
        e = b.d_ent.alloc(b.ent.ent2.size());
        if (e == hipSuccess) e = hipMemcpyAsync(b.d_ent, b.ent.ent2.data(), b.ent.ent2.size() * sizeof(int32_t), hipMemcpyHostToDevice, b.stream);
        if (e != hipSuccess) return fail(hip_rc(e), "flat stream entries: %s", hipGetErrorString(e));
    }
    if (!b.flat_tpc || test_knob("TCGNN_LDS_FLAT")) return TCGNN_OK;
    DevBuf<uint32_t> d_trial;
    std::vector<uint32_t> trial((size_t)b.p->nw_eff, 0u);
    e = d_trial.alloc(trial.size());
    if (e == hipSuccess) e = hipMemsetAsync(d_trial, 0, trial.size() * sizeof(uint32_t), b.stream);
    if (e == hipSuccess) {
        hipLaunchKernelGGL(cell_cold_count_kernel, dim3((unsigned)((b.nw + 255) / 256)), dim3(256), 0, b.stream, b.best.d_cellcols.ptr, b.d_kmap.ptr, b.best.d_sorder.ptr, b.nw, b.nranges, b.maxw,
                           d_trial.ptr, (uint32_t)(32 * b.flat_tpc), b.d_ent.ptr);
        e = hipGetLastError();
    }
    if (e == hipSuccess) e = hipMemcpyAsync(trial.data(), d_trial, trial.size() * sizeof(uint32_t), hipMemcpyDeviceToHost, b.stream);
    if (e == hipSuccess) e = hipStreamSynchronize(b.stream);
    if (e != hipSuccess) return fail(hip_rc(e), "cell table: %s", hipGetErrorString(e));
    uint32_t worst = 0;
    for (uint32_t c : trial) worst = std::max(worst, (c + 31u) / 32u);
    if (worst > 16u) {
        if (b.verbose) fprintf(stderr, "[tcgnn] cell stream %d: ordinary after all - one window would leave %u cold tiles behind\n", b.slot, worst);
        b.flat_tpc = 0; b.over_cols = 0;
    }
    return TCGNN_OK;
}
static int cells_entries(CellBuild& b) {
    if (!b.with_dense()) { (void)hipStreamSynchronize(b.stream); b.d_ent.reset(); }
    FlatEntries ent = flat_entries(b.nwg, b.maxw, b.rbase, b.rlist, b.cnt, b.dense_mx, b.with_dense(), b.flat_tpc != 0);
    hipError_t e = hipSuccess;
    if (b.flat_tpc) {
        e = b.d_rl2.alloc(ent.rl2.size());
        if (e == hipSuccess) e = hipMemcpyAsync(b.d_rl2, ent.rl2.data(), ent.rl2.size() * sizeof(uint32_t), hipMemcpyHostToDevice, b.stream);
        if (e == hipSuccess && b.with_dense()) {
            e = b.d_xbase.alloc(ent.xbase.size());
            if (e == hipSuccess) e = hipMemcpyAsync(b.d_xbase, ent.xbase.data(), ent.xbase.size() * sizeof(uint32_t), hipMemcpyHostToDevice, b.stream);
        }
        if (e == hipSuccess) e = hipStreamSynchronize(b.stream);
    }
    if (e != hipSuccess) return fail(hip_rc(e), "flat stream entries: %s", hipGetErrorString(e));
    b.ent = std::move(ent);
    return TCGNN_OK;
}
static int cells_fill_tiles(CellBuild& b) {
    const tcgnn_plan* p = b.p;
    const int flat_tpc = b.flat_tpc;
    b.hot_cols -= b.over_cols; b.cold_cols += b.over_cols;
    uint64_t run = 0;
    if (flat_tpc) run = (uint64_t)b.ent.nentries * (uint64_t)b.per_wg * (uint64_t)flat_tpc;
    else for (size_t k = 0; k < b.cnt.size(); ++k) { const uint32_t c = b.cnt[k]; b.cnt[k] = (uint32_t)run; run += c; }
    if (run >= (1ull << 32)) return fail(TCGNN_ERR_BAD_GRAPH, "LDS-range SpMM: %llu tiles overflow the 32-bit cell table", (unsigned long long)run);
    const int64_t ntiles = b.ntiles = (int64_t)run;
    const int64_t nwords = b.nwords = std::max<int64_t>(ntiles, 1) * kCellWords;
    hipError_t e = b.d_tiles.alloc((size_t)nwords);
    if (e == hipSuccess) e = hipMemcpyAsync(b.d_cnt, b.cnt.data(), b.cnt.size() * sizeof(uint32_t), hipMemcpyHostToDevice, b.stream);
    if (e != hipSuccess) return fail(hip_rc(e), "cell stream (%lld tiles): %s", (long long)ntiles, hipGetErrorString(e));
    hipLaunchKernelGGL(cell_init_kernel, dim3((unsigned)((nwords + 255) / 256)), dim3(256), 0, b.stream, b.d_tiles.ptr, nwords, b.rows);
    if (b.val) {
        e = b.d_eidx.alloc((size_t)std::max<int64_t>(ntiles, 1) * 32);
        if (e == hipSuccess) e = hipMemsetAsync(b.d_eidx, 0xff, b.d_eidx.bytes, b.stream);
        if (e != hipSuccess) return fail(hip_rc(e), "edge index of the cell stream: %s", hipGetErrorString(e));
    }
    hipLaunchKernelGGL(cell_fill_kernel, dim3((unsigned)b.nw), dim3(256), 0, b.stream, b.s_wb, b.best.d_sorder.ptr, b.s_cols, b.s_mask, b.nwg, b.nranges, p->Nc,
                       b.maxw, b.rows, b.d_cnt.ptr, b.best.d_firstq.ptr, b.d_tiles.ptr, b.d_kmap.ptr, b.best.d_parts.ptr, b.best.d_cellcols.ptr, flat_tpc, b.s_eidx, b.d_eidx.ptr, b.d_ent.ptr, b.d_xbase.ptr);
    if (ntiles > 0) hipLaunchKernelGGL(cell_optimize_kernel, dim3((unsigned)((ntiles + 255) / 256)), dim3(256), 0, b.stream, b.d_tiles.ptr, ntiles, b.rows, b.d_eidx.ptr);
    e = hipGetLastError();
    if (e != hipSuccess) return fail(hip_rc(e), "cell fill: %s", hipGetErrorString(e));
    if (!flat_tpc) return TCGNN_OK;
    e = b.d_flat.alloc((size_t)nwords);
    if (e == hipSuccess) {
        hipLaunchKernelGGL(flat_transpose_kernel, dim3((unsigned)((nwords + 255) / 256)), dim3(256), 0, b.stream, b.d_tiles.ptr, b.d_flat.ptr, b.ent.nentries * kLdsWaves, b.maxw * flat_tpc, b.d_rl2.ptr);
        e = hipGetLastError();
    }
    if (e == hipSuccess) e = hipStreamSynchronize(b.stream);
    b.d_tiles.reset();
    b.d_cnt.reset();
    if (e != hipSuccess) return fail(hip_rc(e), "flat cell stream: %s", hipGetErrorString(e));
    return TCGNN_OK;
}
static int cells_cold_remainder(CellBuild& b) {
    if (b.cold_cols <= 0) return TCGNN_OK;
    const tcgnn_plan* p = b.p;
    const int nwe = p->nw_eff;
    const uint32_t cap = (uint32_t)(32 * b.flat_tpc);
    std::vector<uint32_t> coldc((size_t)nwe, 0);
    DevBuf<uint32_t> d_coldcols;
    hipError_t e = d_coldcols.alloc((size_t)nwe);
    if (e == hipSuccess) e = hipMemsetAsync(d_coldcols, 0, (size_t)nwe * sizeof(uint32_t), b.stream);
    if (e == hipSuccess) {
        hipLaunchKernelGGL(cell_cold_count_kernel, dim3((unsigned)((b.nw + 255) / 256)), dim3(256), 0, b.stream, b.best.d_cellcols.ptr, b.d_kmap.ptr, b.best.d_sorder.ptr, b.nw, b.nranges, b.maxw,
                           d_coldcols.ptr, cap, b.d_ent.ptr);
        e = hipGetLastError();
    }
    if (e == hipSuccess) e = hipMemcpyAsync(coldc.data(), d_coldcols, coldc.size() * sizeof(uint32_t), hipMemcpyDeviceToHost, b.stream);
    if (e == hipSuccess) e = hipStreamSynchronize(b.stream);
    b.cptr.assign((size_t)nwe + 1, 0);
    for (int w = 0; w < nwe; ++w) { b.cptr[(size_t)w + 1] = b.cptr[(size_t)w] + (coldc[(size_t)w] + 31) / 32; b.cold_max = std::max<int64_t>(b.cold_max, (coldc[(size_t)w] + 31) / 32); }
    b.cold_tiles = b.cptr[(size_t)nwe];
    const size_t ncold = (size_t)std::max<int64_t>(b.cold_tiles, 1);
    if (e == hipSuccess) e = b.d_cold_ptr.alloc(b.cptr.size());
    if (e == hipSuccess) e = b.d_ccols.alloc(ncold * kWbCols);
    if (e == hipSuccess) e = b.d_cmask.alloc(ncold * kWinRows);
    if (e == hipSuccess) e = hipMemcpyAsync(b.d_cold_ptr, b.cptr.data(), b.d_cold_ptr.bytes, hipMemcpyHostToDevice, b.stream);
    if (e == hipSuccess) e = hipMemsetAsync(b.d_cmask, 0, b.d_cmask.bytes, b.stream);
    if (e == hipSuccess) {
        const int64_t nfill = (int64_t)ncold * kWbCols;
        hipLaunchKernelGGL(fill_i32_kernel, dim3((unsigned)std::min<int64_t>((nfill + 255) / 256, 65535)), dim3(256), 0, b.stream, b.d_ccols.ptr, nfill, p->Nc);
        e = hipGetLastError();
    }
    if (e == hipSuccess && b.val) {
        e = b.d_cold_eidx.alloc(ncold * 32);
        if (e == hipSuccess) e = hipMemsetAsync(b.d_cold_eidx, 0xff, b.d_cold_eidx.bytes, b.stream);
    }
    if (e == hipSuccess) {
        hipLaunchKernelGGL(cell_cold_fill_kernel, dim3((unsigned)b.nw), dim3(256), 0, b.stream, b.s_wb, b.best.d_sorder.ptr, b.s_cols, b.s_mask, b.d_kmap.ptr, b.nranges, p->Nc,
                           b.maxw, b.rows, b.d_cold_ptr.ptr, b.d_ccols.ptr, b.d_cmask.ptr, b.best.d_parts.ptr, b.best.d_firstq.ptr, cap, b.s_eidx, b.d_cold_eidx.ptr, b.d_ent.ptr);
        e = hipGetLastError();
    }
    if (e != hipSuccess) return fail(hip_rc(e), "cell fill: %s", hipGetErrorString(e));
    return TCGNN_OK;
}
static int cells_wavefront_cold_lists(CellBuild& b) {
    hipError_t e = hipSuccess;
    if (!b.val && b.flat_tpc && b.cold_tiles > 0 && b.cold_tiles < (1ll << 28) && flat_cold_fits(lds_stream_nt(b.slot), b.maxw, b.flat_tpc)) {
        std::vector<int32_t>& wptr = b.wptr;
        std::vector<uint32_t>& wlist = b.wlist;
        wptr.assign((size_t)b.nwg * kLdsWaves + 1, 0);
        wlist.reserve((size_t)b.cold_tiles);
        for (int g2 = 0; g2 < b.nwg; ++g2)
            for (int v = 0; v < kLdsWaves; ++v) {
                wptr[(size_t)g2 * kLdsWaves + v] = (int32_t)wlist.size();
                for (int j = 0; j < b.maxw; ++j) {
                    const int w = b.best.sorder[(size_t)cell_position(g2, v, j, b.maxw)];
                    if (w < 0) continue;
                    for (int64_t t = b.cptr[(size_t)w]; t < b.cptr[(size_t)w + 1]; ++t) wlist.push_back((uint32_t)t | ((uint32_t)j << 28));
                }
            }
        wptr[(size_t)b.nwg * kLdsWaves] = (int32_t)wlist.size();
        DevBuf<uint32_t> d_wlist;
        e = b.d_wcold_ptr.alloc(wptr.size());
        if (e == hipSuccess) e = d_wlist.alloc(std::max<size_t>(wlist.size(), 1));
        if (e == hipSuccess) e = b.d_wcold.alloc(std::max<size_t>(wlist.size(), 1) * 64);
        if (e == hipSuccess) e = hipMemcpyAsync(b.d_wcold_ptr, wptr.data(), wptr.size() * sizeof(int32_t), hipMemcpyHostToDevice, b.stream);
        if (e == hipSuccess && !wlist.empty()) e = hipMemcpyAsync(d_wlist, wlist.data(), wlist.size() * sizeof(uint32_t), hipMemcpyHostToDevice, b.stream);
        if (e == hipSuccess && !wlist.empty()) {
            const int64_t nwordsw = (int64_t)wlist.size() * 64;
            hipLaunchKernelGGL(flat_cold_records_kernel, dim3((unsigned)((nwordsw + 255) / 256)), dim3(256), 0, b.stream, d_wlist.ptr, (int64_t)wlist.size(), b.d_ccols.ptr, b.d_cmask.ptr, b.d_wcold.ptr);
            e = hipGetLastError();
        }
        if (e == hipSuccess) e = hipStreamSynchronize(b.stream);
    }
    if (e == hipSuccess) e = hipStreamSynchronize(b.stream);
    if (e != hipSuccess) return fail(hip_rc(e), "cell fill: %s", hipGetErrorString(e));
    return TCGNN_OK;
}
static int cells_flat_rbase(CellBuild& b) {
    if (!b.flat_tpc) return TCGNN_OK;
    hipError_t e = hipMemcpyAsync(b.d_rbase, b.ent.wg_first.data(), b.ent.wg_first.size() * sizeof(int32_t), hipMemcpyHostToDevice, b.stream);
    if (e == hipSuccess) e = hipStreamSynchronize(b.stream);
    if (e != hipSuccess) return fail(TCGNN_ERR_HIP, "flat stream entries: %s", hipGetErrorString(e));
    return TCGNN_OK;
}
static void cells_publish(CellBuild& b, size_t* build_only_bytes) {
    tcgnn_plan::CellStream& cs = b.p->lds[b.slot];
    const int64_t nentries = b.ent.nentries;
    const bool wcold = b.d_wcold_ptr != nullptr;
    size_t bytes = 0, build_only = 0;
    bytes += b.best.d_sorder.release(cs.d_order);
    bytes += b.d_cnt.release(cs.d_cell_ptr);
    bytes += b.d_tiles.release(cs.d_cell_tiles);
    bytes += b.d_flat.release(cs.d_flat);
    bytes += b.d_wcold_ptr.release(cs.d_wcold_ptr);
    bytes += b.d_wcold.release(cs.d_wcold);
    build_only += b.d_eidx.release(cs.d_eidx);
    build_only += b.d_cold_eidx.release(cs.d_cold_eidx);
    bytes += b.d_rbase.release(cs.d_rbase);
    bytes += b.d_rlist.release(cs.d_rlist);
    bytes += b.d_rl2.release(cs.d_rl2);
    bytes += b.best.d_parts.release(cs.d_parts);
    bytes += b.d_cold_ptr.release(cs.d_cold_ptr);
    bytes += b.d_ccols.release(cs.d_cold_cols);
    bytes += b.d_cmask.release(cs.d_cold_mask);
    cs.flat_tpc = b.flat_tpc;
    cs.nwg = b.nwg; cs.tiles = b.ntiles;
    cs.npairs = (int32_t)nentries; cs.dense_entries = (int32_t)(nentries - b.npairs);
    cs.cold_tiles = b.cold_tiles; cs.hot_cols = b.hot_cols; cs.cold_cols = b.cold_cols; cs.cold_max = b.cold_max;
    cs.nsplit = b.best.nsplit;
    if (b.verbose)
        fprintf(stderr, "[tcgnn] cell stream %d (%d windows per wavefront, %d-row ranges): %d workgroups x %d ranges, %lld of %lld pairs hot (>= %u columns), "
                        "%lld columns hot / %lld cold, %lld tiles + %lld cold gather tiles, placement %s\n",
                b.slot, b.maxw, b.rows, b.nwg, b.nranges, (long long)b.npairs, (long long)b.npairs_all, b.best.hot_min, (long long)b.hot_cols, (long long)b.cold_cols,
                (long long)b.ntiles, (long long)b.cold_tiles, b.best.mode == kPlaceGlobal ? "longest-first over the graph" : "contiguous blocks");
    if (b.verbose && b.flat_tpc) fprintf(stderr, "[tcgnn]   flat: %d tile(s) per cell, %lld entries (%lld dense), %lld columns beyond the cells' tiles moved to the cold remainder (%s)\n", b.flat_tpc,
                                         (long long)nentries, (long long)(nentries - b.npairs), (long long)b.over_cols,
                                         wcold ? "multiplied inside the kernel, one tile per range" : "added by spmm_cold_planar_kernel");
    if (b.verbose && b.best.nsplit) fprintf(stderr, "[tcgnn]   %d windows split over several wavefronts\n", b.best.nsplit);
    b.p->bytes += bytes + build_only;
    if (build_only_bytes) *build_only_bytes = build_only;
    cs.nranges.store(b.nranges, std::memory_order_release);
}

static void release_cell_stream(tcgnn_plan::CellStream& cs) {
    for (void* q : {(void*)cs.d_order, (void*)cs.d_rbase, (void*)cs.d_rlist, (void*)cs.d_rl2, (void*)cs.d_parts, (void*)cs.d_cold_ptr, (void*)cs.d_cold_cols, (void*)cs.d_cold_mask,
                    (void*)cs.d_cell_ptr, (void*)cs.d_cell_tiles, (void*)cs.d_flat, (void*)cs.d_wcold_ptr, (void*)cs.d_wcold, (void*)cs.d_eidx, (void*)cs.d_cold_eidx, (void*)cs.d_eidx16,
                    (void*)cs.d_cold_eidx16}) (void)hipFree(q);
}

static int build_lds_cells(tcgnn_plan* p, hipStream_t stream, int slot, size_t* build_only_bytes = nullptr) {
    static std::mutex mu;
    std::lock_guard<std::mutex> lock(mu);
    if (p->lds[slot].nranges > 0) return TCGNN_OK;
    if (p->nw_eff <= 0 || p->Nc <= 0) return fail(TCGNN_ERR_INVALID_ARG, "LDS-range SpMM: empty graph");
    CellBuild b;
    b.p = p; b.stream = stream; b.slot = slot;
    b.val = slot == kLdsValSlot;
    if (b.val && !p->d_xwb_ptr) return fail(TCGNN_ERR_INVALID_ARG, "edge-valued LDS-resident SpMM: the single-edge stream has not been built");
    b.s_wb = b.val ? p->d_xwb_ptr : p->d_wb_ptr;
    b.s_cols = b.val ? p->d_xcols : p->d_cols;
    b.s_mask = b.val ? p->d_xmask : p->d_mask;
    b.s_eidx = b.val ? p->d_xeidx : nullptr;
    b.maxw = lds_stream_maxw(slot);
    b.rows = lds_stream_buf_rows(slot) - 8;
    b.nranges = (p->Nc + b.rows - 1) / b.rows;
    b.per_wg = kLdsWaves * b.maxw;
    b.nwg = lds_workgroups(p, b.maxw);
    b.nw = b.nwg * b.per_wg;
    b.ncell = (int64_t)b.nwg * b.nranges * b.per_wg;
    b.npairs_all = (int64_t)b.nwg * b.nranges;
    b.verbose = verbose_level() > 0;
    if (const int rc = cells_window_weights(b)) return rc;
    if (const int rc = cells_choose_placement(b)) return rc;
    if (const int rc = cells_hot_pairs(b)) return rc;
    cells_dense_pairs(b);
    cells_flat_or_ordinary(b);
    if (const int rc = cells_hub_row_trial(b)) return rc;
    if (const int rc = cells_entries(b)) return rc;
    if (b.val && b.flat_tpc != 1)
        return fail(TCGNN_ERR_UNSUPPORTED, "edge-valued LDS-resident SpMM: the single-edge cells of this graph are not uniform enough for a flat stream");
    if (const int rc = cells_fill_tiles(b)) return rc;
    if (const int rc = cells_cold_remainder(b)) return rc;
    if (const int rc = cells_wavefront_cold_lists(b)) return rc;
    if (const int rc = cells_flat_rbase(b)) return rc;
    cells_publish(b, build_only_bytes);
    return TCGNN_OK;
}

static int val_source_stream(tcgnn_plan* p, hipStream_t stream, bool* usable, size_t* bytes) {
    const int nw = p->nw_eff;
    *usable = false; *bytes = 0;
    DevBuf<int32_t> d_ew, d_flags, d_xc, d_xe;
    DevBuf<int64_t> d_xp;
    DevBuf<uint32_t> d_xm;
    std::vector<int32_t> ew((size_t)nw, 0);
    hipError_t e = d_ew.alloc((size_t)nw);
    if (e == hipSuccess) e = d_flags.alloc(1);
    if (e == hipSuccess) e = hipMemsetAsync(d_flags, 0, sizeof(int32_t), stream);
    if (e == hipSuccess) {
        hipLaunchKernelGGL(window_edges_kernel, dim3((unsigned)((nw + 255) / 256)), dim3(256), 0, stream, p->rowptr, p->N, nw, d_ew.ptr);
        e = hipGetLastError();
    }
    if (e == hipSuccess) e = hipMemcpyAsync(ew.data(), d_ew, (size_t)nw * sizeof(int32_t), hipMemcpyDeviceToHost, stream);
    if (e == hipSuccess) e = hipStreamSynchronize(stream);
    d_ew.reset();
    std::vector<int64_t> xptr((size_t)nw + 1, 0);
    for (int w = 0; w < nw; ++w) xptr[(size_t)w + 1] = xptr[(size_t)w] + (ew[(size_t)w] + kWbCols - 1) / kWbCols;
    const int64_t total = std::max<int64_t>(xptr[(size_t)nw], 1);
    if (e == hipSuccess) e = d_xp.alloc(xptr.size());
    if (e == hipSuccess) e = d_xc.alloc((size_t)total * kWbCols);
    if (e == hipSuccess) e = d_xe.alloc((size_t)total * kWbCols);
    if (e == hipSuccess) e = d_xm.alloc((size_t)total * kWinRows);
    if (e == hipSuccess) e = hipMemcpyAsync(d_xp, xptr.data(), xptr.size() * sizeof(int64_t), hipMemcpyHostToDevice, stream);
    if (e == hipSuccess) e = hipMemsetAsync(d_xe, 0xff, d_xe.bytes, stream);
    if (e == hipSuccess) e = hipMemsetAsync(d_xm, 0, d_xm.bytes, stream);
    if (e == hipSuccess) {
        const int64_t nfill = total * kWbCols;
        hipLaunchKernelGGL(fill_i32_kernel, dim3((unsigned)std::min<int64_t>((nfill + 255) / 256, 65535)), dim3(256), 0, stream, d_xc.ptr, nfill, p->Nc);
        e = hipGetLastError();
        if (e == hipSuccess) e = hipStreamSynchronize(stream);
    }
    int32_t bad = 0;
    if (e == hipSuccess && nw > 0) {
        hipLaunchKernelGGL(expand_edges_kernel, dim3((unsigned)nw), dim3(256), 0, stream, p->d_wb_ptr, p->d_cols, p->d_mask, p->d_ebase, d_xp.ptr, d_xc.ptr, d_xm.ptr, d_xe.ptr, p->Nc, d_flags.ptr);
        e = hipGetLastError();
    }
    if (e == hipSuccess) e = hipMemcpyAsync(&bad, d_flags, sizeof(int32_t), hipMemcpyDeviceToHost, stream);
    if (e == hipSuccess) e = hipStreamSynchronize(stream);
    if (e != hipSuccess) return fail(hip_rc(e), "single-edge tile stream: %s", hipGetErrorString(e));
    if (bad) return TCGNN_OK;
    *bytes = d_xp.release(p->d_xwb_ptr) + d_xc.release(p->d_xcols) + d_xm.release(p->d_xmask) + d_xe.release(p->d_xeidx);
    p->total_xwb = xptr[(size_t)nw];
    p->bytes += *bytes;
    *usable = true;
    return TCGNN_OK;
}
static bool val_index16(tcgnn_plan* p, hipStream_t stream) {
    tcgnn_plan::CellStream& cs = p->lds[kLdsValSlot];
    const size_t nt = (size_t)std::max<int64_t>(cs.tiles, 1), nc = (size_t)std::max<int64_t>(cs.cold_tiles, 1);
    DevBuf<uint16_t> d_e16, d_cold_e16;
    DevBuf<int32_t> d_bad;
    int32_t bad = 0;
    hipError_t e = d_e16.alloc(nt * 32);
    if (e == hipSuccess) e = d_cold_e16.alloc(nc * 32);
    if (e == hipSuccess) e = d_bad.alloc(1);
    if (e == hipSuccess) e = hipMemsetAsync(d_bad, 0, sizeof(int32_t), stream);
    if (e == hipSuccess) e = hipMemsetAsync(d_e16, 0xff, d_e16.bytes, stream);
    if (e == hipSuccess) {
        hipLaunchKernelGGL(val_index16_kernel, dim3((unsigned)(cs.nwg * kLdsWaves * kLdsMaxW2)), dim3(256), 0, stream, p->rowptr, cs.d_order, cs.d_eidx, cs.d_rbase, d_e16.ptr, p->N,
                           kLdsMaxW2, cs.cold_tiles > 0 ? cs.d_cold_ptr : nullptr, cs.d_cold_eidx, d_cold_e16.ptr, d_bad.ptr, cs.d_rl2, std::max(cs.npairs, 1));
        e = hipGetLastError();
    }
    if (e == hipSuccess) e = hipMemcpyAsync(&bad, d_bad, sizeof(int32_t), hipMemcpyDeviceToHost, stream);
    if (e == hipSuccess) e = hipStreamSynchronize(stream);
    if (e != hipSuccess || bad) return false;
    p->bytes += d_e16.release(cs.d_eidx16) + d_cold_e16.release(cs.d_cold_eidx16);
    return true;
}
static int build_val_stream(tcgnn_plan* p, hipStream_t stream) {
    static std::mutex mu;
    std::lock_guard<std::mutex> lock(mu);
    if (p->val_choice.load(std::memory_order_acquire) >= 0) return TCGNN_OK;
    bool usable;
    size_t source_bytes, eidx_bytes = 0;
    const int src = val_source_stream(p, stream, &usable, &source_bytes);
    if (!usable) { p->val_choice.store(0, std::memory_order_release); return src; }
    const int rc = build_lds_cells(p, stream, kLdsValSlot, &eidx_bytes);
    tcgnn_plan::CellStream& cs = p->lds[kLdsValSlot];
    const bool ok = rc == TCGNN_OK && cs.nranges > 0 && cs.flat_tpc == 1 && cs.nsplit == 0 && cs.d_eidx && val_index16(p, stream);
    if (cs.d_eidx) {
        (void)hipStreamSynchronize(stream);
        p->bytes -= eidx_bytes;
        (void)hipFree(cs.d_eidx); (void)hipFree(cs.d_cold_eidx); cs.d_eidx = nullptr; cs.d_cold_eidx = nullptr;
    }
    (void)hipStreamSynchronize(stream);
    p->bytes -= source_bytes;
    (void)hipFree(p->d_xwb_ptr); (void)hipFree(p->d_xcols); (void)hipFree(p->d_xmask); (void)hipFree(p->d_xeidx);
    p->d_xwb_ptr = nullptr; p->d_xcols = nullptr; p->d_xmask = nullptr; p->d_xeidx = nullptr;
    p->val_choice.store(ok ? 1 : 0, std::memory_order_release);
    return (rc == TCGNN_ERR_OOM || rc == TCGNN_ERR_HIP) ? rc : TCGNN_OK;
}
static size_t val_stream_bytes(const tcgnn_plan* p) {
    const tcgnn_plan::CellStream& cs = p->lds[kLdsValSlot];
    if (p->val_choice.load(std::memory_order_acquire) != 1) return 0;
    return ((size_t)(std::max<int64_t>(cs.tiles, 1) + std::max<int64_t>(cs.cold_tiles, 0)) * 64 + 255) / 256 * 256;
}
```

tc-gnn_atc23_amd/csrc/tcgnn_lds_spmm.inc:

```

static constexpr int kLdsWaves = 16;
static constexpr int kLdsMaxW = 4;
static constexpr int kLdsMaxW2 = 8;
static constexpr int kLdsStreams = 7;
static constexpr int kLdsValSlot = 6;
__host__ __device__ constexpr int lds_stream_of(int nt, int maxw) { return maxw == 8 ? (nt == 2 ? 4 : 5) : (nt >= 4 ? 0 : (nt == 2 ? 1 : (nt == 1 ? 2 : 3))); }
__host__ __device__ constexpr int lds_stream_buf_rows(int slot) { return slot == 0 ? 512 : (slot == 1 ? 768 : (slot == 2 ? 1536 : (slot == 3 ? 640 : (slot == 4 || slot == 6 ? 768 : 512)))); }
__host__ __device__ constexpr int lds_stream_maxw(int slot) { return slot >= 4 ? 8 : 4; }
__host__ __device__ constexpr int lds_stream_nt(int slot) { return slot == 0 ? 4 : (slot == 1 ? 2 : (slot == 2 ? 1 : (slot == 3 ? 3 : (slot == 4 || slot == 6 ? 2 : 1)))); }
__host__ __device__ constexpr int lds_buf_rows(int nt, int maxw) { return lds_stream_buf_rows(lds_stream_of(nt, maxw)); }
static constexpr int lds_pad_tiles(int maxw, int buf_rows) { return maxw != 4 ? (buf_rows == 768 ? 12 : 16) : (buf_rows == 512 ? 6 : (buf_rows == 1536 ? 12 : 8)); }
static constexpr int kCellWords = 32;
static constexpr int lds_chunk_dims(int maxw) { return 256 / maxw; }

__device__ __forceinline__ void lds_own_fallback(const SpmmSmallArgs& fb) {
    if (!fb.guard) return;
    const int wave = (int)(threadIdx.x >> 6), wpb = (int)(blockDim.x >> 6);
    const int lin = (int)blockIdx.x + (int)gridDim.x * (int)blockIdx.y;
    const int total = (int)(gridDim.x * gridDim.y) * wpb;
    for (int coloff = 0; coloff < fb.D; coloff += 64) spmm_small_windows(fb, lin * wpb + wave, total, coloff, (int)(threadIdx.x & 63));
}

struct SpmmLdsArgs {
    const uint32_t* cell_ptr;
    const uint32_t* tiles;
    const int32_t* order;
    const _Float16* x16;
    const uint32_t* hdr;
    float* y;
    int32_t N, D, stride , chunk0, xrows, nranges, nw, nwg;
    int32_t dbg, relu;
    const int32_t* rbase;
    const int32_t* rlist;
    const float* w;
    int32_t dout, accumulate;
    const uint32_t* parts;
    SpmmSmallArgs fb;
    Epi epi;
};

__host__ __device__ inline void cell_place(int p, int maxw, int& wg, int& wave, int& j) {
    j = p % maxw;
    wave = (p / maxw) % kLdsWaves;
    wg = p / (maxw * kLdsWaves);
}
__host__ __device__ inline int cell_position(int wg, int wave, int j, int maxw) { return (wg * kLdsWaves + wave) * maxw + j; }

__device__ __forceinline__ int64_t cell_lower_bound(const int32_t* base, int64_t n, int32_t x) {
    int64_t lo = 0, hi = n;
    while (lo < hi) {
        const int64_t mid = (lo + hi) >> 1;
        if (base[mid] < x) lo = mid + 1; else hi = mid;
    }
    return lo;
}

__global__ __launch_bounds__(256) void window_tiles_kernel(const int64_t* __restrict__ wb_ptr, const int32_t* __restrict__ cols, int32_t nw, int32_t nranges,
                                                           int32_t Nc, int32_t rows, uint32_t* __restrict__ tiles_of) {
    const int64_t idx = (int64_t)blockIdx.x * blockDim.x + threadIdx.x;
    if (idx >= (int64_t)nw * nranges) return;
    const int w = (int)(idx / nranges), r = (int)(idx % nranges);
    const int32_t* base = cols + wb_ptr[w] * kWbCols;
    const int64_t n = (wb_ptr[w + 1] - wb_ptr[w]) * kWbCols;
    const int64_t x0 = (int64_t)r * rows, x1 = x0 + rows;
    const int64_t lo = cell_lower_bound(base, n, (int32_t)(x0 < Nc ? x0 : Nc));
    const int64_t hi = cell_lower_bound(base, n, (int32_t)(x1 < Nc ? x1 : Nc));
    if (hi > lo) atomicAdd(&tiles_of[w], (uint32_t)((hi - lo + 31) / 32));
}

__global__ __launch_bounds__(256) void cell_count_kernel(const int64_t* __restrict__ wb_ptr, const int32_t* __restrict__ order,
                                                         const int32_t* __restrict__ cols, int32_t nw, int32_t nwg, int32_t nranges,
                                                         int32_t Nc, int32_t maxw, int32_t rows, uint32_t* __restrict__ cnt, uint32_t* __restrict__ firstq,
                                                         const uint32_t* __restrict__ parts) {
    const int64_t idx = (int64_t)blockIdx.x * blockDim.x + threadIdx.x;
    if (idx >= (int64_t)nw * nranges) return;
    const int p = (int)(idx / nranges), r = (int)(idx % nranges);
    const int w = order[p];
    if (w < 0) { firstq[idx] = 0u; return; }
    const int32_t* base = cols + wb_ptr[w] * kWbCols;
    const int64_t n = (wb_ptr[w + 1] - wb_ptr[w]) * kWbCols;
    const int64_t x0 = (int64_t)r * rows, x1 = x0 + rows;
    int64_t lo = cell_lower_bound(base, n, (int32_t)(x0 < Nc ? x0 : Nc));
    int64_t hi = cell_lower_bound(base, n, (int32_t)(x1 < Nc ? x1 : Nc));
    if (parts) {
        const uint32_t pi = parts[p], k = (pi >> 8) & 0xffu;
        if (k > 1u) {
            const int64_t q = pi & 0xffu, nt = (hi - lo + 31) / 32;
            const int64_t a = lo + 32 * (nt * q / k), b = lo + 32 * (nt * (q + 1) / k);
            lo = a < hi ? a : hi;
            hi = b < hi ? b : hi;
        }
    }
    int wg, wave, j;
    cell_place(p, maxw, wg, wave, j);
    cnt[(((int64_t)wg * nranges + r) * kLdsWaves + wave) * maxw + j] = (uint32_t)(hi - lo);
    firstq[idx] = (uint32_t)lo;
}

__global__ __launch_bounds__(256) void cell_pair_cols_kernel(const uint32_t* __restrict__ cellcols, int64_t npairs, int32_t per_wg, int32_t maxw,
                                                             uint32_t* __restrict__ paircols, uint32_t* __restrict__ pairmax,
                                                             uint32_t* __restrict__ pairover, uint32_t* __restrict__ pairtiles) {
    const int64_t k = (int64_t)blockIdx.x * blockDim.x + threadIdx.x;
    if (k >= npairs) return;
    uint32_t s = 0, mx = 0, o1 = 0, o2 = 0, tt = 0;
    for (int v = 0; v < per_wg / maxw; ++v) {
        uint32_t t = 0;
        for (int j = 0; j < maxw; ++j) {
            const uint32_t c = cellcols[k * per_wg + v * maxw + j];
            s += c; t += (c + 31u) / 32u;
            o1 += c > 32u ? c - 32u : 0u; o2 += c > 64u ? c - 64u : 0u;
        }
        mx = t > mx ? t : mx;
        tt += t;
    }
    paircols[k] = s;
    pairmax[k] = mx;
    if (pairover) { pairover[k] = o1; pairover[npairs + k] = o2; }
    if (pairtiles) pairtiles[k] = tt;
}
__global__ __launch_bounds__(256) void cell_compact_kernel(const uint32_t* __restrict__ cellcols, const int32_t* __restrict__ kmap, int64_t npairs, int32_t per_wg,
                                                           uint32_t* __restrict__ cnt) {
    const int64_t idx = (int64_t)blockIdx.x * blockDim.x + threadIdx.x;
    if (idx >= npairs * per_wg) return;
    const int64_t pair = idx / per_wg;
    const int k = kmap[pair];
    if (k >= 0) cnt[(int64_t)k * per_wg + (idx - pair * per_wg)] = (cellcols[idx] + 31u) / 32u;
}
__device__ __forceinline__ bool pair_is_dense(const int32_t* ent, int32_t k) { return ent && ent[2 * k + 1] >= 0; }
__global__ __launch_bounds__(256) void cell_cold_count_kernel(const uint32_t* __restrict__ cellcols, const int32_t* __restrict__ kmap, const int32_t* __restrict__ order,
                                                              int32_t nslots, int32_t nranges, int32_t maxw, uint32_t* __restrict__ coldcols, uint32_t cap,
                                                              const int32_t* __restrict__ ent = nullptr) {
    const int p = blockIdx.x * blockDim.x + threadIdx.x;
    if (p >= nslots) return;
    const int w = order[p];
    if (w < 0) return;
    int wg, wave, j;
    cell_place(p, maxw, wg, wave, j);
    uint32_t s = 0;
    for (int r = 0; r < nranges; ++r) {
        const uint32_t c = cellcols[(((int64_t)wg * nranges + r) * kLdsWaves + wave) * maxw + j];
        const int32_t kp = kmap[(int64_t)wg * nranges + r];
        if (kp < 0) s += c;
        else if (cap && c > cap && !pair_is_dense(ent, kp)) s += c - cap;
    }
    if (s) atomicAdd(&coldcols[w], s);
}
__global__ __launch_bounds__(256) void cell_cold_fill_kernel(const int64_t* __restrict__ wb_ptr, const int32_t* __restrict__ order, const int32_t* __restrict__ cols,
                                                             const uint32_t* __restrict__ mask, const int32_t* __restrict__ kmap, int32_t nranges, int32_t Nc,
                                                             int32_t maxw, int32_t rows, const int64_t* __restrict__ cold_ptr, int32_t* __restrict__ ccols,
                                                             uint32_t* __restrict__ cmask, const uint32_t* __restrict__ parts,
                                                             const uint32_t* __restrict__ firstq, uint32_t cap,
                                                             const int32_t* __restrict__ eidx_src = nullptr, int32_t* __restrict__ ceidx = nullptr,
                                                             const int32_t* __restrict__ ent = nullptr) {
    __shared__ uint32_t wsum[4];
    __shared__ uint32_t base_s;
    const int p = blockIdx.x;
    const int w = order[p];
    if (w < 0) return;
    if (parts && ((parts[p] >> 8) & 0xffu) > 1u && (parts[p] & 0xffu) != 0u) return;
    int wg, wave, j;
    cell_place(p, maxw, wg, wave, j);
    const int64_t tb = wb_ptr[w];
    const int64_t n = (wb_ptr[w + 1] - tb) * kWbCols;
    const int64_t cb = cold_ptr[w];
    if (cold_ptr[w + 1] == cb) return;
    if (threadIdx.x == 0) base_s = 0u;
    __syncthreads();
    const int lane = threadIdx.x & 63, wv = threadIdx.x >> 6;
    for (int64_t q0 = 0; q0 < n; q0 += blockDim.x) {
        const int64_t q = q0 + threadIdx.x;
        int32_t c = Nc;
        if (q < n) c = cols[tb * kWbCols + q];
        const int32_t kpc = c < Nc ? kmap[(int64_t)wg * nranges + c / rows] : 0;
        const bool cold = c < Nc && (kpc < 0 || (cap && (uint32_t)q - firstq[(int64_t)p * nranges + c / rows] >= cap && !pair_is_dense(ent, kpc)));
        const uint64_t bal = __ballot(cold);
        const uint32_t before = (uint32_t)__popcll(bal & ((1ull << lane) - 1ull));
        if (lane == 0) wsum[wv] = (uint32_t)__popcll(bal);
        __syncthreads();
        uint32_t off = base_s;
        for (int k = 0; k < wv; ++k) off += wsum[k];
        if (cold) {
            const uint32_t pos = off + before;
            const int64_t t = cb + (pos >> 5);
            const uint32_t k = pos & 31u;
            ccols[t * kWbCols + k] = c;
            if (ceidx) ceidx[t * 32 + k] = eidx_src[tb * kWbCols + q];
            const uint32_t* m = mask + (tb + (q >> 5)) * kWinRows;
            const uint32_t b = (uint32_t)(q & 31);
#pragma unroll
            for (int rr = 0; rr < kWinRows; ++rr)
                if ((m[rr] >> b) & 1u) atomicOr(&cmask[t * kWinRows + rr], 1u << k);
        }
        __syncthreads();
        if (threadIdx.x == 0) base_s += wsum[0] + wsum[1] + wsum[2] + wsum[3];
        __syncthreads();
    }
}

__host__ __device__ constexpr int cell_slot(int q, int h) { return ((q >> 1) * 2 + (h >> 2)) * 8 + (q & 1) * 4 + (h & 3); }
__host__ __device__ constexpr int cell_home(int k) { return ((k >> 3) & 1) * 4 + (k & 3); }
__global__ __launch_bounds__(256) void cell_init_kernel(uint32_t* __restrict__ tiles, int64_t nwords, int32_t rows) {
    const int64_t k = (int64_t)blockIdx.x * blockDim.x + threadIdx.x;
    if (k >= nwords) return;
    const int w = (int)(k & 31);
    tiles[k] = w >= 16 ? 0u : ((uint32_t)(rows + cell_home(2 * w)) | ((uint32_t)(rows + cell_home(2 * w + 1)) << 16));
}

__global__ __launch_bounds__(256) void cell_fill_kernel(const int64_t* __restrict__ wb_ptr, const int32_t* __restrict__ order,
                                                        const int32_t* __restrict__ cols, const uint32_t* __restrict__ mask, int32_t nwg,
                                                        int32_t nranges, int32_t Nc, int32_t maxw, int32_t rows, const uint32_t* __restrict__ cell_ptr,
                                                        const uint32_t* __restrict__ firstq, uint32_t* __restrict__ tiles, const int32_t* __restrict__ kmap,
                                                        const uint32_t* __restrict__ parts, const uint32_t* __restrict__ cellcols, int32_t tpc,
                                                        const int32_t* __restrict__ eidx_src = nullptr, int32_t* __restrict__ eidx_out = nullptr,
                                                        const int32_t* __restrict__ ent = nullptr, const uint32_t* __restrict__ xbase = nullptr) {
    const int p = blockIdx.x;
    const int w = order[p];
    if (w < 0) return;
    const bool split = parts && ((parts[p] >> 8) & 0xffu) > 1u;
    const int64_t tb = wb_ptr[w];
    const int64_t n = (wb_ptr[w + 1] - tb) * kWbCols;
    int wg, wave, j;
    cell_place(p, maxw, wg, wave, j);
    for (int64_t q = threadIdx.x; q < n; q += blockDim.x) {
        const int32_t c = cols[tb * kWbCols + q];
        if (c >= Nc) continue;
        const int r = c / rows;
        const int kp = kmap[(int64_t)wg * nranges + r];
        if (kp < 0) continue;
        const uint32_t first = firstq[(int64_t)p * nranges + r];
        if (split && ((uint32_t)q < first || (uint32_t)q >= first + cellcols[(((int64_t)wg * nranges + r) * kLdsWaves + wave) * maxw + j])) continue;
        const uint32_t pos = (uint32_t)q - first;
        const int64_t cell = ((int64_t)kp * kLdsWaves + wave) * maxw + j;
        int64_t t;
        if (!tpc) t = (int64_t)cell_ptr[cell] + (pos >> 5);
        else {
            const int64_t e = ent ? ent[2 * kp] : kp;
            if (pos < 32u * (uint32_t)tpc) t = (((int64_t)e * kLdsWaves + wave) * maxw + j) * tpc + (pos >> 5);
            else if (pair_is_dense(ent, kp)) {
                const int64_t P = (int64_t)xbase[cell] + (pos >> 5) - 1;
                t = ((int64_t)(ent[2 * kp + 1] + P / maxw) * kLdsWaves + wave) * maxw + P % maxw;
            } else continue;
        }
        const uint32_t k = pos & 31u;
        reinterpret_cast<uint16_t*>(tiles + t * kCellWords)[k] = (uint16_t)(c - r * rows);
        if (eidx_out) eidx_out[t * 32 + k] = eidx_src[tb * kWbCols + q];
        const uint32_t* m = mask + (tb + (q >> 5)) * kWinRows;
        const uint32_t b = (uint32_t)(q & 31);
#pragma unroll
        for (int rr = 0; rr < kWinRows; ++rr)
            if ((m[rr] >> b) & 1u) atomicOr(&tiles[t * kCellWords + 16 + rr], 1u << k);
    }
}

__global__ __launch_bounds__(256) void cell_optimize_kernel(uint32_t* __restrict__ tiles, int64_t ntiles, int32_t rows, int32_t* __restrict__ eidx = nullptr) {
    const int64_t t = (int64_t)blockIdx.x * blockDim.x + threadIdx.x;
    if (t >= ntiles) return;
    uint32_t* tile = tiles + t * kCellWords;
    uint32_t idw[16], mk[16];
#pragma unroll
    for (int k = 0; k < 16; ++k) { idw[k] = tile[k]; mk[k] = tile[16 + k]; }
    uint32_t taken = 0u, placed = 0u;
    uint8_t dst[32];
    for (int k = 0; k < 32; ++k) {
        const uint32_t id = (idw[k >> 1] >> (16 * (k & 1))) & 0xffffu;
        dst[k] = 255;
        if (id >= (uint32_t)rows) { placed |= 1u << k; continue; }
        for (int q = 0; q < 4; ++q) {
            const int ns = cell_slot(q, (int)(id & 7u));
            if (!((taken >> ns) & 1u)) { taken |= 1u << ns; dst[k] = (uint8_t)ns; placed |= 1u << k; break; }
        }
    }
    for (int k = 0; k < 32; ++k) {
        if ((placed >> k) & 1u) continue;
        const int ns = __ffs((int)~taken) - 1;
        taken |= 1u << ns;
        dst[k] = (uint8_t)ns;
    }
    uint16_t nid[32];
    for (int ns = 0; ns < 32; ++ns) nid[ns] = (uint16_t)(rows + cell_home(ns));
// ... 342 lines not shown
```

tc-gnn_atc23_amd/csrc/tcgnn_spmm_dispatch.inc:

```
static constexpr int kMaxGatherBlockDims = 4096;

struct Scales { const float* col = nullptr; const float* row = nullptr; const float* bias = nullptr; };
enum class StagedLayout { kNone, kRowMajor, kPlanar };
struct SpmmCall {
    const tcgnn_plan* plan = nullptr;
    const float *d_X = nullptr, *d_val = nullptr, *d_gate = nullptr;
    float* d_Y = nullptr;
    int32_t D = 0, relu = 0;
    void* ws = nullptr; size_t ws_bytes = 0;
    hipStream_t stream = nullptr;
    const void* d_image = nullptr; StagedLayout staged = StagedLayout::kNone;
    int64_t ld = 0; bool block_of_wider = false;
    const float* d_W = nullptr; int32_t D_out = 0;
    Scales sc;
    bool scaled() const { return sc.col || sc.row || sc.bias; }
    Epi epi() const { return Epi{sc.row, sc.bias}; }
    int64_t stride() const { return ld ? ld : D; }
    int dpad() const { return round_up(D, 16); }
};
enum class Walk { kValCsr, kSmall, kColumnBlocks, kLds, kValLds, kValSliced, kSync, kBlocked, kPerWindow };
struct SpmmRoute {
    Walk walk = Walk::kPerWindow;
    LdsPass passes[2]; int npass = 0;
    const tcgnn_plan::CellStream* cold = nullptr;
    bool own_fb = false;
    int accumulate = 0;
    int nslices = 0;
    bool planar() const { return walk == Walk::kLds || walk == Walk::kValLds; }
};
static bool lds_wanted(const tcgnn_plan* plan, int mode, int dpad) { return plan->nw_eff > 0 && (mode == 3 || (mode == 0 && lds_chosen(plan, dpad))); }
static bool planar_records_fit(const tcgnn_plan* plan, int dpad) { return (int64_t)(dpad / 16) * ((int64_t)plan->Nc + 1) * 32 < ((int64_t)1 << 32); }
static bool val_lds_width(int dp) { return (dp % 64 == 0 || dp % 64 == 48) && dp <= 2 * kMaxChunkDims; }
static bool val_lds_width_ok(const tcgnn_plan* plan, int dp) { return val_lds_width(dp) && plan->canonical && plan->nw_eff > 0 && planar_records_fit(plan, dp); }
static bool val_lds_wanted(const tcgnn_plan* plan, int mode, int dp) { return (mode == 0 || mode == 3) && val_lds_width_ok(plan, dp) && (mode == 3 || lds_chosen(plan, dp)); }
static void settle_on_gather_walks(const tcgnn_plan* plan, int dpad) { if (dpad / 16 <= 64) plan->lds_choice[dpad / 16] = 0; }
static bool flat_cold_behind(const tcgnn_plan::CellStream& cs) { return cs.flat_tpc && cs.cold_tiles > 0 && !cs.d_wcold_ptr; }
struct LdsStreamFacts { bool all_built, rows_cold, flat_cold, thin; };
static LdsStreamFacts lds_stream_facts(const tcgnn_plan* plan, const LdsPass* passes, int npass) {
    LdsStreamFacts f{npass > 0, false, false, false};
    for (int i = 0; i < npass; ++i) {
        const tcgnn_plan::CellStream& ci = plan->lds[lds_stream_of(passes[i].nt, passes[i].maxw)];
        if (ci.nranges == 0) { f.all_built = false; continue; }
        if (ci.flat_tpc) f.flat_cold = f.flat_cold || flat_cold_behind(ci);
        else f.rows_cold = f.rows_cold || ci.cold_tiles > 0;
        f.thin = f.thin || ci.hot_cols * 2 < ci.hot_cols + ci.cold_cols;
    }
    return f;
}
static bool lds_streams_serve(const tcgnn_plan* plan, int mode, const LdsPass* passes, int npass, bool dense_update, bool planar_staged, bool* settle,
                              const tcgnn_plan::CellStream** cold) {
    const LdsStreamFacts f = lds_stream_facts(plan, passes, npass);
    *settle = false; *cold = nullptr;
    if ((f.rows_cold && (npass > 1 || dense_update)) || (f.flat_cold && dense_update)) {
        *settle = f.rows_cold && npass > 1 && mode != 3;
        return false;
    }
    if (f.thin && mode != 3) { *settle = true; return false; }
    if (f.rows_cold && planar_staged) return false;
    if (f.rows_cold) *cold = &plan->lds[lds_stream_of(passes[0].nt, passes[0].maxw)];
    return true;
}
static bool stream_is_capturing(hipStream_t stream) {
    hipStreamCaptureStatus capturing = hipStreamCaptureStatusNone;
    return hipStreamIsCapturing(stream, &capturing) == hipSuccess && capturing != hipStreamCaptureStatusNone;
}
enum class LdsBuild {
    kInCall,
    kPrepare,
    kQuery
};
static int ensure_lds_streams(const tcgnn_plan* plan, hipStream_t stream, int mode, int dpad, const LdsPass* passes, int npass, LdsBuild who, bool* ok) {
    *ok = true;
    for (int i = 0; i < npass; ++i) {
        const int slot = lds_stream_of(passes[i].nt, passes[i].maxw);
        if (plan->lds[slot].nranges > 0) continue;
        if (who == LdsBuild::kInCall && stream_is_capturing(stream)) {
            *ok = false;
            return mode == 3 ? fail(TCGNN_ERR_INVALID_ARG, "LDS-resident SpMM: the cell stream of this width has to be built before the call is captured into a graph") : TCGNN_OK;
        }
        const int b = build_lds_cells(const_cast<tcgnn_plan*>(plan), stream, slot);
        if (!b) continue;
        *ok = false;
        if (who == LdsBuild::kQuery) return TCGNN_OK;
        if (mode == 3) return b;
        settle_on_gather_walks(plan, dpad);
        if (who == LdsBuild::kInCall) return TCGNN_OK;
    }
    return TCGNN_OK;
}
static int ensure_val_stream(const tcgnn_plan* plan, hipStream_t stream, int mode, bool in_call) {
    if (plan->val_choice.load(std::memory_order_acquire) >= 0 || (in_call && stream_is_capturing(stream))) return TCGNN_OK;
    const int b = build_val_stream(const_cast<tcgnn_plan*>(plan), stream);
    if (b && mode == 3) return b;
    if (b) const_cast<tcgnn_plan*>(plan)->val_choice.store(0, std::memory_order_release);
    return TCGNN_OK;
}
static int route_spmm(const SpmmCall& c, SpmmRoute* r) {
    const tcgnn_plan* const plan = c.plan;
    const int32_t D = c.D;
    const int dpad = c.dpad();
    const bool staged = c.staged != StagedLayout::kNone, planar_staged = c.staged == StagedLayout::kPlanar;
    if (c.d_val && (!plan->canonical || plan->E < 4)) { r->walk = Walk::kValCsr; return TCGNN_OK; }
    const int mode = spmm_mode_of(plan);
    if (!c.d_val && !staged && !c.d_W && plan->nw_eff > 0 && (mode == 4 || (mode == 0 && plan->total_wb <= kSmallMaxTiles))) { r->walk = Walk::kSmall; return TCGNN_OK; }
    bool lds = !c.d_val && (!staged || planar_staged) && !c.block_of_wider && lds_wanted(plan, mode, dpad) && planar_records_fit(plan, dpad);
    if (lds && c.d_W && !(dpad <= 64 && !g_lds_maxw)) lds = false;
    if (lds) {
        r->npass = lds_passes(dpad, r->passes);
        if (const int rc = ensure_lds_streams(plan, c.stream, mode, dpad, r->passes, r->npass, LdsBuild::kInCall, &lds)) return rc;
    }
    if (lds) {
        bool settle;
        lds = lds_streams_serve(plan, mode, r->passes, r->npass, c.d_W != nullptr, planar_staged, &settle, &r->cold);
        if (settle) settle_on_gather_walks(plan, dpad);
    }
    if (planar_staged && !lds)
        return fail(TCGNN_ERR_UNSUPPORTED, "tcgnn_spmm_staged_planar: the LDS-resident kernel does not take this plan at %d columns (tcgnn_spmm_staged_layout tells; stage row-major and call tcgnn_spmm_staged)", D);
    if (lds) {
        int total_chunks = 0;
        for (int i = 0; i < r->npass; ++i) total_chunks += r->passes[i].nchunks;
        r->accumulate = (c.d_W && total_chunks > 1) ? 1 : 0;
        r->own_fb = r->npass == 1 && !r->cold && !c.d_W && !staged && c.stride() == D && !flat_cold_behind(plan->lds[lds_stream_of(r->passes[0].nt, r->passes[0].maxw)]) &&
                    !c.scaled();
        r->walk = Walk::kLds;
        return TCGNN_OK;
    }
    if (!pitch_fits_descriptor(D)) {
        if (staged) return fail(TCGNN_ERR_UNSUPPORTED, "tcgnn_spmm_staged: rows of %d columns exceed the %d-byte descriptor stride", D, kMaxStructStride);
        if (c.block_of_wider) return fail(TCGNN_ERR_INVALID_ARG, "tcgnn_spmm: nested column blocks");
        r->walk = Walk::kColumnBlocks;
        return TCGNN_OK;
    }
    const bool plain_val = c.d_val && !staged && !c.block_of_wider && !c.d_gate && !c.relu;
    if (plain_val && !c.d_W && val_lds_wanted(plan, mode, dpad)) {
        if (const int rc = ensure_val_stream(plan, c.stream, mode, true)) return rc;
        if (plan->val_choice.load(std::memory_order_acquire) == 1 && c.ws_bytes >= workspace_bytes_for(plan->Nc, D) + val_stream_bytes(plan)) { r->walk = Walk::kValLds; return TCGNN_OK; }
    }
    if (plain_val && plan->nw_eff > 0 && mode == 0 && dpad > 32 && dpad <= kMaxChunkDims && agnn_supported(plan, D)) {
        const size_t need = workspace_bytes_for(plan->Nc, D) + agnn_partial_bytes(plan) + agnn_slice_bytes(plan, D);
        const AgnnRoute bw = agnn_plan_walk(plan, D, true);
        if (bw.walk == AgnnWalk::kSliced && bw.nslices > 0 && c.ws_bytes >= need) { r->nslices = bw.nslices; r->walk = Walk::kValSliced; return TCGNN_OK; }
    }
    const int pitch = x16_pitch(dpad);
    if (plan->nw_eff > 0 && !c.d_W && !image_is_big(plan->Nc, pitch) && sync_chosen(plan, pitch * 2, mode, c.d_val ? kSyncVal : kSyncSpmm, dpad / 16)) { r->walk = Walk::kSync; return TCGNN_OK; }
    const size_t x16_bytes = image_bytes(plan, pitch);
    const bool blocked = !c.d_W && plan->nbuckets > 0 && mode != 1 && (mode == 2 || (range_walk_pays(plan, x16_bytes) && (!c.d_val || x16_bytes > ((size_t)64 << 20))));
    r->walk = blocked ? Walk::kBlocked : Walk::kPerWindow;
    return TCGNN_OK;
}
static SpmmSmallArgs small_args(const SpmmCall& c, const uint32_t* guard_hdr) {
    const tcgnn_plan* const plan = c.plan;
    SpmmSmallArgs a{};
    a.wb_ptr = plan->d_wb_ptr; a.cols = plan->d_cols; a.mask = plan->d_mask; a.x = c.d_X; a.gate = c.d_gate; a.y = c.d_Y;
    a.N = plan->N; a.Nc = plan->Nc; a.D = c.D; a.relu = c.relu; a.nw = plan->nw_eff; a.guard = guard_hdr;
    return a;
}
static SpmmArgs spmm_args(const tcgnn_plan* plan, const StagedImage& im, float* d_Y, int32_t D) {
    SpmmArgs a{};
    a.wb_ptr = plan->d_wb_ptr; a.order = plan->d_order; a.cols = plan->d_cols; a.mask = plan->d_mask; a.ebase = plan->d_ebase;
    a.x16 = im.x16; a.hdr = im.hdr; a.y = d_Y;
    a.N = plan->N; a.D = D; a.stride = im.pitch; a.E = plan->E; a.xrows = plan->Nc + 1; a.ldy = D;
    a.big = image_is_big(plan->Nc, im.pitch);
    return a;
}
template <class F>
static int for_column_chunks(int dpad, F&& launch) {
    const int nfull = dpad / kMaxChunkDims, rem = (dpad % kMaxChunkDims) / 16;
    if (nfull) HIP_TRY(launch(8, 0, nfull));
    if (rem) HIP_TRY(launch(rem, nfull, 1));
    return TCGNN_OK;
}
static void launch_small_pair(const SpmmCall& c, unsigned grid_x, const uint32_t* guard_hdr) {
    const SpmmSmallArgs sa = small_args(c, guard_hdr);
    const dim3 grid(grid_x, (unsigned)((c.D + 63) / 64));
    if (c.scaled()) hipLaunchKernelGGL(spmm_small_scaled_kernel, grid, dim3(64), 0, c.stream, SpmmSmallScaledArgs{sa, c.sc.col, c.epi()});
    else hipLaunchKernelGGL(spmm_small_kernel, grid, dim3(64), 0, c.stream, sa);
}
static int launch_wide_fallback(const SpmmCall& c, const StagedImage& im) {
    const tcgnn_plan* const plan = c.plan;
    if (c.d_image) return TCGNN_OK;
    const int32_t D = c.D;
    const int64_t ld = c.stride();
    const unsigned grid = (unsigned)std::min<int64_t>(((int64_t)plan->N + 3) / 4, 4096);
    if (c.d_W) hipLaunchKernelGGL(spmm_gemm_wide_fallback_kernel, dim3(grid), dim3(256), 0, c.stream, im.hdr, plan->rowptr, plan->col, c.d_X, c.d_W, c.d_Y, plan->N, D, c.D_out, c.relu);
    else if (!c.d_val && ld == D) launch_small_pair(c, (unsigned)std::min(plan->nw_eff, 2048), im.hdr);
    else if (c.scaled()) hipLaunchKernelGGL(spmm_wide_fallback_scaled_kernel, dim3(grid), dim3(256), 0, c.stream, im.hdr, plan->rowptr, plan->col, c.d_X, c.d_gate, c.sc.col, c.epi(), c.d_Y,
                                            plan->N, D, ld, ld, c.relu, plan->canonical ? 0 : 1);
    else hipLaunchKernelGGL(spmm_wide_fallback_kernel, dim3(grid), dim3(256), 0, c.stream, im.hdr, c.d_val ? 1 : 0, plan->rowptr, plan->col, c.d_val, (const float*)nullptr, c.d_X, c.d_gate, c.d_Y,
                            plan->N, D, ld, ld, c.relu, (!c.d_val && !plan->canonical) ? 1 : 0);
    HIP_TRY(hipGetLastError());
    return TCGNN_OK;
}
static int run_spmm(const SpmmCall& c);
static int run_column_blocks(const SpmmCall& c) {
    const tcgnn_plan* const plan = c.plan;
    if (const int rc = check_workspace("staging", c.ws, c.ws_bytes, workspace_bytes_for(plan->Nc, c.D))) return rc;
    if (const int rc = fill_header(plan, static_cast<uint32_t*>(c.ws), c.d_X, c.d_gate, c.sc.col, c.D, guard_spmm(plan), c.d_val, plan->E, c.stream)) return rc;
    for (int c0 = 0; c0 < c.D; c0 += kMaxGatherBlockDims) {
        SpmmCall b = c;
        b.d_X = c.d_X + c0; b.d_Y = c.d_Y + c0; b.D = std::min(kMaxGatherBlockDims, c.D - c0);
        if (c.d_gate) b.d_gate = c.d_gate + c0;
        if (c.sc.bias) b.sc.bias = c.sc.bias + c0;
        b.ld = c.D; b.block_of_wider = true;
        if (const int rc = run_spmm(b)) return rc;
    }
    return TCGNN_OK;
}
static int launch_val_lds(const SpmmCall& c, const StagedImage& im) {
    const tcgnn_plan* const plan = c.plan;
    hipStream_t stream = c.stream;
    const tcgnn_plan::CellStream& cs = plan->lds[kLdsValSlot];
    const size_t image = workspace_bytes_for(plan->Nc, c.D);
    _Float16* const vals = reinterpret_cast<_Float16*>(static_cast<char*>(c.ws) + image);
    _Float16* const cvals = vals + (size_t)std::max<int64_t>(cs.tiles, 1) * 32;
    KernelTimer timer(plan, stream, cs.cold_tiles > 0 ? "val_permute_kernel + spmm_lds_val_kernel + spmm_cold_val_kernel (cold remainder)" : "val_permute_kernel + spmm_lds_val_kernel");
    constexpr LaunchGeom permute{kValThreads, kValSpanHalves * 2, 0, 0};
    HIP_TRY((launch_kernel<val_permute_kernel, permute.lds_bytes>(dim3((unsigned)(cs.nwg * kLdsWaves * (kLdsMaxW2 / kValWpb))), permute, stream, c.d_val, plan->rowptr, cs.d_order, cs.d_eidx16, cs.d_rbase, im.hdr,
                                                                 vals, plan->N, cs.cold_tiles > 0 ? cs.d_cold_ptr : nullptr, cs.d_cold_eidx16, cvals, cs.d_rl2, cs.dense_entries > 0 ? 1 : 0, std::max(cs.npairs, 1))));
    SpmmValArgs va{};
    va.blocks = cs.d_flat; va.vals = vals; va.order = cs.d_order; va.x16 = im.x16; va.hdr = im.hdr; va.y = c.d_Y;
    va.N = plan->N; va.D = c.D; va.stride = im.dpad / 16; va.xrows = plan->Nc + 1; va.nw = plan->nw_eff; va.nwg = cs.nwg;
    va.rbase = cs.d_rbase; va.rl2 = cs.d_rl2; va.nent = std::max(cs.npairs, 1);
    HIP_TRY(launch_lds_val(va, (im.dpad + 31) / 32, stream));
    if (cs.cold_tiles > 0) {
        ColdValArgs ca{};
        ca.cold_ptr = cs.d_cold_ptr; ca.ccols = cs.d_cold_cols; ca.cmask = cs.d_cold_mask; ca.cvals = cvals; ca.x16 = im.x16; ca.hdr = im.hdr; ca.y = c.d_Y;
        ca.N = plan->N; ca.D = c.D; ca.xrows = plan->Nc + 1; ca.nw = plan->nw_eff; ca.ncols = im.dpad;
        hipLaunchKernelGGL(spmm_cold_val_kernel, dim3((unsigned)((plan->nw_eff + 3) / 4), (unsigned)((im.dpad + 63) / 64)), dim3(256), 0, stream, ca);
        HIP_TRY(hipGetLastError());
    }
    return TCGNN_OK;
}
static int launch_cold_rows(const SpmmCall& c, const tcgnn_plan::CellStream* cold, const StagedImage& im, const _Float16* x16_rows) {
    const tcgnn_plan* const plan = c.plan;
    const int pitch_r = x16_pitch(im.dpad);
    SpmmArgs a = spmm_args(plan, im, c.d_Y, c.D);
    a.wb_ptr = cold->d_cold_ptr; a.cols = cold->d_cold_cols; a.mask = cold->d_cold_mask; a.ebase = reinterpret_cast<const int32_t*>(cold->d_cold_mask);
    a.x16 = x16_rows; a.stride = pitch_r; a.big = image_is_big(plan->Nc, pitch_r); a.relu = c.relu; a.accumulate = 1;
    constexpr int cold_w4 = 48;
    const int waves = (cold->cold_tiles >= (int64_t)cold_w4 * plan->nw_eff || cold->cold_max >= 512) ? 4 : 1;
    return for_column_chunks(im.dpad, [&](int nt, int chunk0, int nchunks) {
        a.chunk0 = chunk0;
        return launch_spmm_any(false, waves, nt, a, plan->nw_eff, nchunks, c.stream, c.epi());
    });
}
static int launch_lds(const SpmmCall& c, const SpmmRoute& r, const StagedImage& im) {
    const tcgnn_plan* const plan = c.plan;
    hipStream_t stream = c.stream;
    const int32_t D = c.D;
    const Epi epi = c.epi(), no_epi{nullptr, nullptr};
    if (r.accumulate) {
        if (c.relu) return fail(TCGNN_ERR_UNSUPPORTED, "tcgnn_spmm_gemm: ReLU cannot be fused when the product is accumulated over column passes");
        HIP_TRY(hipMemsetAsync(c.d_Y, 0, (size_t)plan->N * c.D_out * sizeof(float), stream));
    }
    const _Float16* x16_rows = nullptr;
    if (r.cold) {
        const size_t image = workspace_bytes_for(plan->Nc, D);
        if (c.ws_bytes < 2 * image) return fail(TCGNN_ERR_WORKSPACE, "tcgnn_spmm: a plan with a cold remainder stages two images: %zu bytes, got %zu", 2 * image, c.ws_bytes);
        StageOpts o; o.d_gate = c.d_gate; o.hdr_from = im.hdr; o.d_cs = c.sc.col;
        StagedImage rows;
        if (const int rc = stage_features(plan, c.d_X, nullptr, D, static_cast<char*>(c.ws) + image, c.ws_bytes - image, stream, o, &rows)) return rc;
        x16_rows = rows.x16;
    }
    const tcgnn_plan::CellStream& cs0 = plan->lds[lds_stream_of(r.passes[0].nt, r.passes[0].maxw)];
    const SpmmSmallArgs fb = small_args(c, r.own_fb ? im.hdr : nullptr);
    KernelTimer timer(plan, stream, r.cold ? "spmm_lds_kernel + spmm_kernel (cold remainder)" :
                                    (cs0.flat_tpc ? (flat_cold_behind(cs0) ? "spmm_lds_flat_kernel + spmm_cold_planar_kernel (cold remainder)" : "spmm_lds_flat_kernel") : "spmm_lds_kernel"));
    for (int i = 0; i < r.npass; ++i) {
        const LdsPass& p = r.passes[i];
        const tcgnn_plan::CellStream& cs = plan->lds[lds_stream_of(p.nt, p.maxw)];
        if (cs.flat_tpc) {
            const bool has_cold = flat_cold_behind(cs);
            SpmmFlatArgs f{};
            f.blocks = cs.d_flat; f.order = cs.d_order; f.x16 = im.x16; f.hdr = im.hdr; f.y = c.d_Y;
            f.N = plan->N; f.D = D; f.stride = im.dpad / 16; f.chunk0 = p.chunk0; f.xrows = plan->Nc + 1; f.nw = plan->nw_eff; f.nwg = cs.nwg;
            f.dbg = g_lds_dbg; f.relu = has_cold ? 0 : c.relu; f.rbase = cs.d_rbase; f.rl2 = cs.d_rl2; f.nent = std::max(cs.npairs, 1);
            f.w = c.d_W; f.dout = c.D_out; f.accumulate = r.accumulate; f.fill_quota = g_lds_fill_quota; f.wcold_ptr = cs.d_wcold_ptr; f.wcold = cs.d_wcold; f.fb = fb;
            HIP_TRY(launch_flat_any(p.maxw, p.nt, cs.flat_tpc, f, p.nchunks, stream, cs.dense_entries > 0, has_cold ? no_epi : epi));
            if (has_cold && !(g_lds_dbg & 16)) {
                const int cd = lds_chunk_dims(p.maxw);
                const int col0 = p.chunk0 * cd, ncols = std::min(p.nchunks * cd, im.dpad - col0);
                ColdPlanarArgs ca{};
                ca.cold_ptr = cs.d_cold_ptr; ca.ccols = cs.d_cold_cols; ca.cmask = cs.d_cold_mask; ca.x16 = im.x16; ca.hdr = im.hdr; ca.y = c.d_Y;
                ca.N = plan->N; ca.D = D; ca.xrows = plan->Nc + 1; ca.nw = plan->nw_eff; ca.col0 = col0; ca.ncols = ncols; ca.relu = c.relu; ca.epi = epi;
                hipLaunchKernelGGL(spmm_cold_planar_kernel, dim3((unsigned)((plan->nw_eff + 3) / 4), (unsigned)((ncols + 63) / 64)), dim3(256), 0, stream, ca);
                HIP_TRY(hipGetLastError());
            }
            continue;
        }
        SpmmLdsArgs l{};
        l.cell_ptr = cs.d_cell_ptr; l.tiles = cs.d_cell_tiles; l.order = cs.d_order; l.x16 = im.x16; l.hdr = im.hdr; l.y = c.d_Y;
        l.N = plan->N; l.D = D; l.stride = im.dpad / 16; l.chunk0 = p.chunk0; l.xrows = plan->Nc + 1; l.nranges = cs.nranges; l.nw = plan->nw_eff; l.nwg = cs.nwg;
        l.dbg = g_lds_dbg; l.relu = r.cold ? 0 : c.relu; l.rbase = cs.d_rbase; l.rlist = cs.d_rlist;
        l.w = c.d_W; l.dout = c.D_out; l.accumulate = r.accumulate; l.parts = cs.d_parts; l.fb = fb; l.epi = r.cold ? no_epi : epi;
        HIP_TRY(launch_lds_any(p.maxw, p.nt, l, p.nchunks, stream));
    }
    return r.cold ? launch_cold_rows(c, r.cold, im, x16_rows) : TCGNN_OK;
}
static SpmmArgs gather_args(const SpmmCall& c, const StagedImage& im) {
    SpmmArgs a = spmm_args(c.plan, im, c.d_Y, c.D);
    a.edge_val = c.d_val; a.relu = c.relu; a.ldy = c.d_W ? c.D_out : (int32_t)c.stride();
    a.w = c.d_W; a.dout = c.D_out; a.unguarded = c.d_image ? 1 : 0;
    return a;
}
static int launch_sync(const SpmmCall& c, const StagedImage& im) {
    const tcgnn_plan* const plan = c.plan;
    const bool val = c.d_val != nullptr;
    KernelTimer timer(plan, c.stream, "spmm_sync_kernel");
    SpmmSyncArgs sa{gather_args(c, im), sync_args(plan, im.pitch * 2)};
    auto wgs = [&](int nt) {
        const LaunchGeom g = sync_geom(nt, val);
        const int per_xcd = std::min((plan->sync.S + 4 * g.maxw - 1) / (4 * g.maxw), plan->num_cus / kXcds * g.wgs_per_cu());
        return kXcds * std::max(per_xcd, 1);
    };
    for (int r = 0; r < plan->sync.R; ++r) {
        sa.s.round = r;
        const int rc = for_column_chunks(im.dpad, [&](int nt, int chunk0, int nchunks) {
            sa.base.chunk0 = chunk0;
            return launch_sync_any(val, nt, sa, wgs(nt), nchunks, c.stream, c.epi());
        });
        if (rc) return rc;
    }
    return TCGNN_OK;
}
static int launch_blocked(const SpmmCall& c, const StagedImage& im) {
    const tcgnn_plan* const plan = c.plan;
    const bool val = c.d_val != nullptr;
    KernelTimer timer(plan, c.stream, "spmm_blocked_kernel");
    const int nranges = range_count(plan, image_bytes(plan, im.pitch), kRangeTargetBytes);
    SpmmBlockedArgs b{gather_args(c, im), plan->d_bptr, plan->nbuckets, plan->nbuckets / nranges, nranges, plan->nw_eff, 0};
    return for_column_chunks(im.dpad, [&](int nt, int chunk0, int nchunks) {
        const LaunchGeom g = blocked_geom(nt, val);
        b.base.chunk0 = chunk0;
        b.ngroups = (plan->nw_eff + g.maxw - 1) / g.maxw;
        return launch_blocked_any(val, nt, b, std::min((b.ngroups + 3) / 4, plan->num_cus * g.wgs_per_cu()), nchunks, c.stream, c.epi());
    });
}
static int launch_per_window(const SpmmCall& c, const StagedImage& im) {
    const tcgnn_plan* const plan = c.plan;
    KernelTimer timer(plan, c.stream, "spmm_kernel");
    SpmmArgs a = gather_args(c, im);
    return for_column_chunks(im.dpad, [&](int nt, int chunk0, int nchunks) {
        a.chunk0 = chunk0;
        return launch_spmm_any(c.d_val != nullptr, plan->waves, nt, a, plan->nw_eff, nchunks, c.stream, c.epi());
    });
}
static int fill_uncovered_rows(const SpmmCall& c) {
    const tcgnn_plan* const plan = c.plan;
    if (c.block_of_wider || (int64_t)plan->nw_eff * kWinRows >= plan->N) return TCGNN_OK;
    HIP_TRY(hipMemsetAsync(c.d_Y, 0, (size_t)plan->N * (c.d_W ? c.D_out : c.D) * sizeof(float), c.stream));
    if (c.sc.row || c.sc.bias) {
        const int64_t n = ((int64_t)plan->N - (int64_t)plan->nw_eff * kWinRows) * c.D;
        hipLaunchKernelGGL(epi_fill_kernel, dim3((unsigned)std::min<int64_t>((n + 255) / 256, 4096)), dim3(256), 0, c.stream, c.d_Y, (int64_t)plan->nw_eff * kWinRows, plan->N, c.D, c.relu, c.epi());
        HIP_TRY(hipGetLastError());
    }
    return TCGNN_OK;
}
static int run_spmm(const SpmmCall& c) {
    const tcgnn_plan* const plan = c.plan;
    if (!plan || c.D < 1 || (plan->N > 0 && ((!c.d_X && !c.d_image) || !c.d_Y))) return fail(TCGNN_ERR_INVALID_ARG, "tcgnn_spmm: null argument or D < 1");
    if (plan->N == 0) return TCGNN_OK;
    if (!c.block_of_wider) {
        if (const int rc = check_output_aligned("tcgnn_spmm", "Y", c.d_Y)) return rc;
        if (!c.d_image) { if (const int rc = check_workspace("tcgnn_spmm", c.ws, c.ws_bytes, tcgnn_workspace_bytes(plan, c.D))) return rc; }
    }
    if (const int rc = fill_uncovered_rows(c)) return rc;
    SpmmRoute r;
    if (const int rc = route_spmm(c, &r)) return rc;
    if (r.walk == Walk::kValCsr) {
        hipLaunchKernelGGL(spmm_val_csr_kernel, dim3((unsigned)((plan->N + 3) / 4)), dim3(256), 0, c.stream, plan->rowptr, plan->col, c.d_val, c.d_X, c.d_Y, plan->N, c.D);
        HIP_TRY(hipGetLastError());
        return TCGNN_OK;
    }
    if (r.walk == Walk::kSmall) {
        KernelTimer timer(plan, c.stream, "spmm_small_kernel");
        launch_small_pair(c, (unsigned)plan->nw_eff, nullptr);
        HIP_TRY(hipGetLastError());
        return TCGNN_OK;
    }
    if (r.walk == Walk::kColumnBlocks) return run_column_blocks(c);
    StagedImage im;
    if (c.d_image) {
        im.hdr = static_cast<const uint32_t*>(c.d_image);
        im.x16 = reinterpret_cast<const _Float16*>(static_cast<const char*>(c.d_image) + kHdrBytes);
        im.dpad = c.dpad();
        im.pitch = x16_pitch(im.dpad);
    } else {
        StageOpts o; o.planar = r.planar(); o.d_gate = c.d_gate; o.ldx = c.block_of_wider ? c.ld : 0; o.block_of_wider = c.block_of_wider; o.d_cs = c.sc.col;
        if (const int rc = stage_features(plan, c.d_X, c.d_val, c.D, c.ws, c.ws_bytes, c.stream, o, &im)) return rc;
    }
    if (plan->nw_eff == 0) return TCGNN_OK;
    int rc = TCGNN_OK;
    switch (r.walk) {
        case Walk::kValLds:    rc = launch_val_lds(c, im); break;
        case Walk::kValSliced: rc = launch_val_sliced(plan, im, c.d_val, c.d_Y, c.D, c.ws, r.nslices, c.stream); break;
        case Walk::kLds:       rc = launch_lds(c, r, im); break;
        case Walk::kSync:      rc = launch_sync(c, im); break;
        case Walk::kBlocked:   rc = launch_blocked(c, im); break;
        default:               rc = launch_per_window(c, im); break;
    }
    return (rc || r.own_fb) ? rc : launch_wide_fallback(c, im);
}

struct HeadsCall {
    const tcgnn_plan* plan = nullptr;
    const float *d_X = nullptr, *d_val = nullptr;
    float* d_Y = nullptr;
    int32_t H = 0, F = 0;
    void* ws = nullptr; size_t ws_bytes = 0;
    hipStream_t stream = nullptr;
};
enum class HeadsWay { kSingle, kFused, kCsr, kPerHead };
static int heads_per_pass(int F) {
    if (F < 8 || F % 8 || F > kMaxHeadsPassDims / 2) return 0;
    const int g = std::min(kMaxHeadsPerPass, kMaxHeadsPassDims / F);
    return F % 16 == 0 ? g : (g & ~1);
}
static HeadsWay route_heads(const tcgnn_plan* plan, int32_t H, int32_t F) {
    if (H == 1) return HeadsWay::kSingle;
    if (!plan->canonical || plan->E < 4) return HeadsWay::kCsr;
    const int D = H * F;
    if (heads_per_pass(F) > 0 && plan->nw_eff > 0 && pitch_fits_descriptor(D) && !image_is_big(plan->Nc, x16_pitch(round_up(D, 16)))) return HeadsWay::kFused;
    return HeadsWay::kPerHead;
}
static size_t heads_workspace_bytes(const tcgnn_plan* plan, int32_t H, int32_t F) {
    switch (route_heads(plan, H, F)) {
        case HeadsWay::kSingle: return tcgnn_workspace_bytes(plan, F);
        case HeadsWay::kFused:  return workspace_bytes_for(plan->Nc, H * F);
        default:                return workspace_bytes_for(plan->Nc, std::min(F, kMaxGatherBlockDims));
    }
}
// ... 60 lines not shown
```

Before: 209.6 GTEPS (SpMM, edges/s/1e9).

## Add long-range LDS flat SpMM stream with 960-row windows and shared cold tiles

Adds an eighth cell stream for the 8-window, two-tile flat SpMM that stages 960 feature rows per LDS buffer instead of 768. It frees LDS by sharing one cold gather tile among four wavefronts, which take turns every two entries. After the main walk, the cold buffer moves to per-wave space so the leftover cold work can drain. The planner builds both layouts, estimates a price for each, and picks the long one when it looks cheaper, with a knob to force it. It also moves the per-pair dense statistics loop from host to a small GPU kernel. The risk is that cold gathers stall while wavefronts wait for their turn.

```diff
diff --git a/tc-gnn_atc23_amd/csrc/tcgnn_device.hip b/tc-gnn_atc23_amd/csrc/tcgnn_device.hip
--- a/tc-gnn_atc23_amd/csrc/tcgnn_device.hip
+++ b/tc-gnn_atc23_amd/csrc/tcgnn_device.hip
@@ -7,6 +7,7 @@
 #include <cstdint>
 #include <cstdlib>
 #include <cstring>
+#include <memory>
 #include <mutex>
 #include <new>
 #include <numeric>
@@ -107,7 +108,8 @@
         uint16_t* d_eidx16 = nullptr;
         uint16_t* d_cold_eidx16 = nullptr;
     };
-    CellStream lds[7];
+    CellStream lds[8];
+    mutable std::atomic<int8_t> lds_long{-1};
     int64_t* d_xwb_ptr = nullptr;
     int32_t* d_xcols = nullptr;
     uint32_t* d_xmask = nullptr;
diff --git a/tc-gnn_atc23_amd/csrc/tcgnn_lds_flat.inc b/tc-gnn_atc23_amd/csrc/tcgnn_lds_flat.inc
--- a/tc-gnn_atc23_amd/csrc/tcgnn_lds_flat.inc
+++ b/tc-gnn_atc23_amd/csrc/tcgnn_lds_flat.inc
@@ -182,10 +182,17 @@
 };
 
 static constexpr bool flat_dense_ok(int nt, int maxw, int tpc) { return tpc == 1 && nt <= 2 && maxw * tpc <= 15; }
-static constexpr int flat_lds_main(int nt, int maxw, int tpc) { return 2 * nt * lds_buf_rows(nt, maxw) * 32 + kLdsWaves * 2 * (maxw * tpc * 128); }
-static constexpr bool flat_cold_fits(int nt, int maxw, int tpc) { return flat_lds_main(nt, maxw, tpc) + kLdsWaves * nt * 1024 <= 160 * 1024; }
-static constexpr int flat_lds_bytes(int nt, int maxw, int tpc) { return flat_lds_main(nt, maxw, tpc) + (flat_cold_fits(nt, maxw, tpc) ? kLdsWaves * nt * 1024 : (flat_dense_ok(nt, maxw, tpc) ? 128 : 0)); }
-
+static constexpr int kLongPoolTiles = 4;
+static constexpr int kLongTurn = 8;
+static constexpr int flat_cold_tiles(bool lng) { return lng ? kLongPoolTiles : kLdsWaves; }
+static constexpr int flat_lds_main(int nt, int maxw, int tpc, bool lng = false) { return 2 * nt * lds_buf_rows(nt, maxw, lng) * 32 + kLdsWaves * 2 * (maxw * tpc * 128); }
+static constexpr bool flat_cold_fits(int nt, int maxw, int tpc, bool lng = false) { return flat_lds_main(nt, maxw, tpc, lng) + flat_cold_tiles(lng) * nt * 1024 <= 160 * 1024; }
+static constexpr int flat_lds_bytes(int nt, int maxw, int tpc, bool lng = false) { return flat_lds_main(nt, maxw, tpc, lng) + (flat_cold_fits(nt, maxw, tpc, lng) ? flat_cold_tiles(lng) * nt * 1024 : (flat_dense_ok(nt, maxw, tpc) ? 128 : 0)); }
+static_assert(flat_lds_bytes(2, 8, 1, true) == 160 * 1024 && flat_cold_fits(2, 8, 1, true), "the long walk: 2 x 2 planes x 960 rows, 32 KB of pads, four 2 KB gather tiles");
+static_assert(flat_lds_bytes(2, 8, 1) == 160 * 1024 && flat_lds_bytes(1, 8, 1) == 80 * 1024, "the shipped 8-window layouts keep their LDS");
+static_assert(lds_buf_rows(2, 8, true) * 32 < 32768 && kLongPoolTiles * 4 == kLdsWaves && kLongTurn == 2 * 4, "plane offsets as immediates, 16-bit row offsets; four wavefronts per pool tile, a turn every two entries");
+
+#define TCGNN_KERNEL_LONG false
 #define TCGNN_KERNEL_NAME spmm_lds_flat_kernel
 #define TCGNN_KERNEL_PARAM const SpmmFlatArgs a
 #define TCGNN_KERNEL_PROLOGUE
@@ -205,6 +212,27 @@
 #undef TCGNN_KERNEL_PARAM
 #undef TCGNN_KERNEL_PROLOGUE
 #undef TCGNN_KERNEL_STORE
+#undef TCGNN_KERNEL_LONG
+#define TCGNN_KERNEL_LONG true
+#define TCGNN_KERNEL_NAME spmm_lds_flat_long_kernel
+#define TCGNN_KERNEL_PARAM const SpmmFlatArgs a
+#define TCGNN_KERNEL_PROLOGUE
+#define TCGNN_KERNEL_STORE(relu, row, col, v) relu_if(relu, v)
+#include "tcgnn_lds_flat_kernel.inc"
+#undef TCGNN_KERNEL_NAME
+#undef TCGNN_KERNEL_PARAM
+#undef TCGNN_KERNEL_PROLOGUE
+#undef TCGNN_KERNEL_STORE
+#define TCGNN_KERNEL_NAME spmm_lds_flat_long_epi_kernel
+#define TCGNN_KERNEL_PARAM const SpmmFlatEpiArgs e
+#define TCGNN_KERNEL_PROLOGUE const SpmmFlatArgs& a = e.a;
+#define TCGNN_KERNEL_STORE(relu, row, col, v) epi_apply(relu, e.epi, row, col, v)
+#include "tcgnn_lds_flat_kernel.inc"
+#undef TCGNN_KERNEL_NAME
+#undef TCGNN_KERNEL_PARAM
+#undef TCGNN_KERNEL_PROLOGUE
+#undef TCGNN_KERNEL_STORE
+#undef TCGNN_KERNEL_LONG
 
 template __global__ void spmm_lds_flat_kernel<1, 4, 1, false, false>(const SpmmFlatArgs);
 template __global__ void spmm_lds_flat_kernel<1, 4, 1, false, true>(const SpmmFlatArgs);
@@ -222,7 +250,11 @@
 template __global__ void spmm_lds_flat_kernel<4, 4, 2, false, false>(const SpmmFlatArgs);
 template __global__ void spmm_lds_flat_kernel<1, 8, 2, false, false>(const SpmmFlatArgs);
 template __global__ void spmm_lds_flat_kernel<2, 8, 2, false, false>(const SpmmFlatArgs);
+template __global__ void spmm_lds_flat_long_kernel<2, 8, 1, false, false>(const SpmmFlatArgs);
+template __global__ void spmm_lds_flat_long_kernel<2, 8, 1, false, true>(const SpmmFlatArgs);
 #ifdef TCGNN_DEBUG_TIMERS
+template __global__ void spmm_lds_flat_long_kernel<2, 8, 1, true, false>(const SpmmFlatArgs);
+template __global__ void spmm_lds_flat_long_kernel<2, 8, 1, true, true>(const SpmmFlatArgs);
 template __global__ void spmm_lds_flat_kernel<1, 4, 1, true, false>(const SpmmFlatArgs);
 template __global__ void spmm_lds_flat_kernel<1, 4, 1, true, true>(const SpmmFlatArgs);
 template __global__ void spmm_lds_flat_kernel<2, 4, 1, true, false>(const SpmmFlatArgs);
@@ -257,8 +289,10 @@
 template __global__ void spmm_lds_flat_epi_kernel<4, 4, 2, false, false>(const SpmmFlatEpiArgs);
 template __global__ void spmm_lds_flat_epi_kernel<1, 8, 2, false, false>(const SpmmFlatEpiArgs);
 template __global__ void spmm_lds_flat_epi_kernel<2, 8, 2, false, false>(const SpmmFlatEpiArgs);
-
-static constexpr LaunchGeom flat_geom(int nt, int maxw, int tpc) { return {kLdsWaves * 64, flat_lds_bytes(nt, maxw, tpc), kLdsWaves / 4, maxw}; }
+template __global__ void spmm_lds_flat_long_epi_kernel<2, 8, 1, false, false>(const SpmmFlatEpiArgs);
+template __global__ void spmm_lds_flat_long_epi_kernel<2, 8, 1, false, true>(const SpmmFlatEpiArgs);
+
+static constexpr LaunchGeom flat_geom(int nt, int maxw, int tpc, bool lng = false) { return {kLdsWaves * 64, flat_lds_bytes(nt, maxw, tpc, lng), kLdsWaves / 4, maxw}; }
 
 template <int NT, int MAXW, int TPC, bool DBG, bool WITH_DENSE>
 static hipError_t launch_flat_dbg(const SpmmFlatArgs& args, int nchunks, hipStream_t stream, const Epi& epi) {
@@ -286,8 +320,22 @@
     if (maxw == kLdsMaxW2) return with_width<2>(nt, [&](auto NT) { return launch_flat_one<NT, kLdsMaxW2, TPC>(args, nchunks, stream, dense, epi); });
     return with_width<4>(nt, [&](auto NT) { return launch_flat_one<NT, kLdsMaxW, TPC>(args, nchunks, stream, dense, epi); });
 }
+template <bool DBG, bool WITH_DENSE>
+static hipError_t launch_flat_long_dbg(const SpmmFlatArgs& args, int nchunks, hipStream_t stream, const Epi& epi) {
+    constexpr LaunchGeom g = flat_geom(2, kLdsMaxW2, 1, true);
+    const dim3 grid((unsigned)args.nwg, (unsigned)nchunks);
+    if constexpr (DBG) return launch_kernel<spmm_lds_flat_long_kernel<2, kLdsMaxW2, 1, true, WITH_DENSE>, g.lds_bytes>(grid, g, stream, args);
+    else return launch_plain_or_twin<spmm_lds_flat_long_kernel<2, kLdsMaxW2, 1, false, WITH_DENSE>, spmm_lds_flat_long_epi_kernel<2, kLdsMaxW2, 1, false, WITH_DENSE>, g.lds_bytes>(grid, g, stream, args, epi);
+}
+static hipError_t launch_flat_long(const SpmmFlatArgs& args, int nchunks, hipStream_t stream, bool dense, const Epi& epi) {
+#ifdef TCGNN_DEBUG_TIMERS
+    if (args.dbg) return dense ? launch_flat_long_dbg<true, true>(args, nchunks, stream, epi) : launch_flat_long_dbg<true, false>(args, nchunks, stream, epi);
+#endif
+    return dense ? launch_flat_long_dbg<false, true>(args, nchunks, stream, epi) : launch_flat_long_dbg<false, false>(args, nchunks, stream, epi);
+}
 static hipError_t launch_flat_any(int maxw, int nt, int tpc, const SpmmFlatArgs& args, int nchunks, hipStream_t stream, bool dense,
-                                  const Epi& epi = Epi{nullptr, nullptr}) {
+                                  const Epi& epi = Epi{nullptr, nullptr}, bool long_ranges = false) {
+    if (long_ranges) return (maxw == kLdsMaxW2 && nt == 2 && tpc == 1) ? launch_flat_long(args, nchunks, stream, dense, epi) : hipErrorInvalidValue;
     return tpc == 2 ? launch_flat_tpc<2>(maxw, nt, args, nchunks, stream, dense, epi) : launch_flat_tpc<1>(maxw, nt, args, nchunks, stream, dense, epi);
 }
 
diff --git a/tc-gnn_atc23_amd/csrc/tcgnn_lds_flat_kernel.inc b/tc-gnn_atc23_amd/csrc/tcgnn_lds_flat_kernel.inc
--- a/tc-gnn_atc23_amd/csrc/tcgnn_lds_flat_kernel.inc
+++ b/tc-gnn_atc23_amd/csrc/tcgnn_lds_flat_kernel.inc
@@ -3,7 +3,9 @@
     TCGNN_KERNEL_PROLOGUE
     if (range_is_wide(a.hdr, 0)) { lds_own_fallback(a.fb); return; }
     const int dbg = DBG ? a.dbg : 0;
-    constexpr int kLdsBufRows = lds_buf_rows(NT, MAXW), kLdsRows = kLdsBufRows - 8;
+    constexpr bool LONG = TCGNN_KERNEL_LONG;
+    static_assert(!LONG || (NT == 2 && MAXW == 8 && TPC == 1), "the long ranges exist for whole 64-column chunks only");
+    constexpr int kLdsBufRows = lds_buf_rows(NT, MAXW, LONG), kLdsRows = kLdsBufRows - 8;
     constexpr int T = MAXW * TPC, PADB = T * 128, kLdsChunkDims = lds_chunk_dims(MAXW);
     static_assert(NT * MAXW <= 16, "accumulators: NT * MAXW * 4 VGPRs");
     extern __shared__ __attribute__((aligned(16))) char smem[];
@@ -60,8 +62,9 @@
     auto load_desc = [&](int r_) -> uint32_t { return dscp[(int64_t)r_ * kLdsWaves]; };
     constexpr bool DENSE = WITH_DENSE && flat_dense_ok(NT, MAXW, TPC);
 
-    constexpr bool CAN_COLD = flat_cold_fits(NT, MAXW, TPC);
-    const uint32_t cbuf = lds0 + (uint32_t)flat_lds_main(NT, MAXW, TPC) + (uint32_t)wave * (NT * 1024u);
+    constexpr bool CAN_COLD = flat_cold_fits(NT, MAXW, TPC, LONG);
+    uint32_t cbuf = lds0 + (uint32_t)flat_lds_main(NT, MAXW, TPC, LONG) + (uint32_t)(LONG ? wave >> 2 : wave) * (NT * 1024u);
+    const int cold_turn = 2 * (wave & 3);
     int cold_c = 0, cold_n = 0, j_cur = 0;
     bool have_g = false, have_n = false;
     uint32_t cid_n = 0u, mw_n = 0u, mw_cur = 0u;
@@ -74,7 +77,7 @@
             ++cold_c;
         }
     };
-    auto cold_step = [&]() {
+    auto cold_step = [&](bool issue_ok) {
         if (have_g) {
             const uint32_t l2 = lane_id_now();
             const uint32_t ad0 = cbuf + ((l2 >> 4) * 8u + ((l2 & 15u) >> 2)) * 32u + (l2 & 3u) * 8u;
@@ -96,8 +99,9 @@
                 }
             }
         }
-        have_g = have_n;
-        if (have_n) {
+        const bool go = have_n && issue_ok;
+        have_g = go;
+        if (go) {
             const int plane0 = chunk_id * (kLdsChunkDims / 16);
 #pragma unroll
             for (int s = 0; s < NT; ++s) {
@@ -109,7 +113,7 @@
             mw_cur = mw_n;
             j_cur = __builtin_amdgcn_readfirstlane((int)(cid_n >> 28));
         }
-        cold_request();
+        if (issue_ok) cold_request();
     };
     if constexpr (CAN_COLD) {
         if (a.wcold_ptr) {
@@ -149,7 +153,8 @@
         ew2 = (uint32_t)__builtin_amdgcn_readfirstlane((int)einfo[1]);
         if (dense_phase) ew1 = (uint32_t)__builtin_amdgcn_readfirstlane((int)dnext);
         if (ew0 & 0x40000000u) buf ^= 1u;
-        if constexpr (CAN_COLD) { if (have_g || have_n) cold_step(); }
+        if constexpr (CAN_COLD && LONG) { const bool turn = (r & 7) == cold_turn; if (have_g || (have_n && turn)) cold_step(turn); }
+        else if constexpr (CAN_COLD) { if (have_g || have_n) cold_step(true); }
         if (more) {
             einfo = load_info(r + 2);
             if (dense_phase) dnext = load_desc(r + 2);
@@ -241,7 +246,11 @@
     }
     if (!(dbg & 32)) __builtin_amdgcn_s_setprio(0);
     if constexpr (CAN_COLD) {
-        while (have_g || have_n) { wait_vm0(); cold_step(); }
+        if constexpr (LONG) {
+            if (have_g) { wait_vm0(); cold_step(false); }
+            cbuf = lds0 + (uint32_t)wave * (NT * 1024u);
+        }
+        while (have_g || have_n) { wait_vm0(); cold_step(true); }
     }
     if (dbg & 16) {
         if (wg == 0 && blockIdx.y == 0 && lane == 0) {
diff --git a/tc-gnn_atc23_amd/csrc/tcgnn_lds_plan.inc b/tc-gnn_atc23_amd/csrc/tcgnn_lds_plan.inc
--- a/tc-gnn_atc23_amd/csrc/tcgnn_lds_plan.inc
+++ b/tc-gnn_atc23_amd/csrc/tcgnn_lds_plan.inc
@@ -1,5 +1,9 @@
 static int g_lds_maxw = [] { const char* e = test_knob("TCGNN_LDS_MAXW"); const int v = e ? atoi(e) : 0; return (v == 4 || v == 8) ? v : 0; }();
 struct LdsPass { int maxw, nt, chunk0, nchunks; };
+static int lds_long_knob() { const char* e = test_knob("TCGNN_LDS_LONG"); return e ? (atoi(e) != 0 ? 1 : 0) : -1; }
+static int lds_pass_slot(const tcgnn_plan* p, const LdsPass& pass) {
+    return lds_stream_of(pass.nt, pass.maxw, pass.maxw == kLdsMaxW2 && pass.nt == 2 && p->lds_long.load(std::memory_order_acquire) == 1);
+}
 static int lds_passes(int dpad, LdsPass (&passes)[2]) {
     int n = 0;
     if (g_lds_maxw) {
@@ -322,6 +326,7 @@
     std::vector<int32_t> kmap, rbase, rlist;
     int64_t npairs = 0, ncell_hot = 0, hot_cols = 0, cold_cols = 0;
     std::vector<uint32_t> cnt;
+    std::vector<uint32_t> pair_extra, pair_cellmx;
     std::vector<uint32_t> dense_mx;
     int64_t over_dense = 0, dense_steps = 0, ndense_pairs = 0, ndense_entries = 0;
     int flat_tpc = 0;
@@ -334,6 +339,9 @@
     DevBuf<int32_t> d_kmap, d_rbase, d_rlist, d_ent, d_ccols, d_eidx, d_cold_eidx, d_wcold_ptr;
     DevBuf<uint32_t> d_cnt, d_tiles, d_flat, d_rl2, d_xbase, d_cmask, d_wcold;
     DevBuf<int64_t> d_cold_ptr;
+    int64_t classic_steps = 0, trial_tiles = 0, worst_tail = 0;
+    double price = 0;
+    bool long_ranges() const { return slot == kLdsLongSlot; }
     bool with_dense() const { return flat_tpc == 1 && ndense_pairs > 0; }
 };
 
@@ -457,9 +465,18 @@
     if (e == hipSuccess) e = hipMemcpyAsync(b.d_rlist, rlist.data(), rlist.size() * sizeof(int32_t), hipMemcpyHostToDevice, b.stream);
     if (e != hipSuccess) return fail(hip_rc(e), "cell table: %s", hipGetErrorString(e));
     if (b.ncell > 0) hipLaunchKernelGGL(cell_compact_kernel, dim3((unsigned)((b.ncell + 255) / 256)), dim3(256), 0, b.stream, b.best.d_cellcols.ptr, b.d_kmap.ptr, b.npairs_all, b.per_wg, b.d_cnt.ptr);
-    b.cnt.resize((size_t)b.ncell_hot + 1);
     e = hipGetLastError();
-    if (e == hipSuccess) e = hipMemcpyAsync(b.cnt.data(), b.d_cnt, b.cnt.size() * sizeof(uint32_t), hipMemcpyDeviceToHost, b.stream);
+    DevBuf<uint32_t> d_stats;
+    b.pair_extra.assign((size_t)b.npairs, 0u); b.pair_cellmx.assign((size_t)b.npairs, 0u);
+    if (e == hipSuccess && b.npairs > 0) {
+        e = d_stats.alloc((size_t)b.npairs * 2);
+        if (e == hipSuccess) {
+            hipLaunchKernelGGL(cell_dense_stats_kernel, dim3((unsigned)((b.npairs + 255) / 256)), dim3(256), 0, b.stream, b.d_cnt.ptr, b.npairs, b.maxw, d_stats.ptr, d_stats.ptr + b.npairs);
+            e = hipGetLastError();
+        }
+        if (e == hipSuccess) e = hipMemcpyAsync(b.pair_extra.data(), d_stats, (size_t)b.npairs * sizeof(uint32_t), hipMemcpyDeviceToHost, b.stream);
+        if (e == hipSuccess) e = hipMemcpyAsync(b.pair_cellmx.data(), d_stats.ptr + b.npairs, (size_t)b.npairs * sizeof(uint32_t), hipMemcpyDeviceToHost, b.stream);
+    }
     if (e == hipSuccess) e = hipStreamSynchronize(b.stream);
     if (e != hipSuccess) return fail(TCGNN_ERR_HIP, "cell count: %s", hipGetErrorString(e));
     return TCGNN_OK;
@@ -474,12 +491,7 @@
     b.dense_mx.assign((size_t)b.npairs, 0u);
     for (int64_t k = 0; k < b.npairs; ++k) {
         if (dense_min == 0xffffffffu && dense_cell_tiles == 0xffffffffu) break;
-        uint32_t mx = 0, cell_mx = 0;
-        for (int v = 0; v < kLdsWaves; ++v) {
-            uint32_t ex = 0;
-            for (int j = 0; j < maxw; ++j) { const uint32_t c = b.cnt[(size_t)((k * kLdsWaves + v) * maxw + j)]; ex += c > 1u ? c - 1u : 0u; cell_mx = std::max(cell_mx, c); }
-            mx = std::max(mx, ex);
-        }
+        const uint32_t mx = b.pair_extra[(size_t)k], cell_mx = b.pair_cellmx[(size_t)k];
         if (!mx || (b.best.pairover[(size_t)kall_of[(size_t)k]] < dense_min && cell_mx < dense_cell_tiles)) continue;
         b.dense_mx[(size_t)k] = mx;
         b.over_dense += b.best.pairover[(size_t)kall_of[(size_t)k]];
@@ -494,6 +506,7 @@
     for (int64_t k = 0; k < npairs_all; ++k)
         if (b.kmap[(size_t)k] >= 0) { classic_tiles += best.pairtiles[(size_t)k]; classic_steps += best.pairmax[(size_t)k];
                                       over[0] += best.pairover[(size_t)k]; over[1] += best.pairover[(size_t)(npairs_all + k)]; }
+    b.classic_steps = classic_steps;
     const char* fenv = test_knob("TCGNN_LDS_FLAT");
     const int forced_flat = fenv ? atoi(fenv) : -1;
     if (best.nsplit == 0 && npairs > 0 && forced_flat != 0) {
@@ -538,14 +551,34 @@
     if (e != hipSuccess) return fail(hip_rc(e), "cell table: %s", hipGetErrorString(e));
     uint32_t worst = 0;
     for (uint32_t c : trial) worst = std::max(worst, (c + 31u) / 32u);
-    if (worst > 16u) {
-        if (b.verbose) fprintf(stderr, "[tcgnn] cell stream %d: ordinary after all - one window would leave %u cold tiles behind\n", b.slot, worst);
+    const int turn = b.long_ranges() ? kLongTurn : 1;
+    for (int g2 = 0; g2 < b.nwg; ++g2) {
+        const int64_t entries = b.with_dense() ? b.ent.wg_first[(size_t)g2 + 1] - b.ent.wg_first[(size_t)g2] : b.rbase[(size_t)g2 + 1] - b.rbase[(size_t)g2];
+        for (int v = 0; v < kLdsWaves; ++v) {
+            int64_t tiles = 0;
+            for (int j = 0; j < b.maxw; ++j) {
+                const int w = b.best.sorder[(size_t)cell_position(g2, v, j, b.maxw)];
+                if (w >= 0) tiles += (trial[(size_t)w] + 31u) / 32u;
+            }
+            b.trial_tiles += tiles;
+            b.worst_tail = std::max(b.worst_tail, tiles - entries / turn);
+        }
+    }
+    if (worst > 16u || (b.long_ranges() && b.worst_tail > 16)) {
+        if (b.verbose) fprintf(stderr, "[tcgnn] cell stream %d: ordinary after all - one window would leave %u cold tiles behind, one wavefront %lld beyond its walk\n", b.slot, worst,
+                               (long long)b.worst_tail);
         b.flat_tpc = 0; b.over_cols = 0;
     }
     return TCGNN_OK;
 }
 static int cells_entries(CellBuild& b) {
     if (!b.with_dense()) { (void)hipStreamSynchronize(b.stream); b.d_ent.reset(); }
+    b.cnt.resize((size_t)b.ncell_hot + 1);
+    {
+        hipError_t ec = hipMemcpyAsync(b.cnt.data(), b.d_cnt, b.cnt.size() * sizeof(uint32_t), hipMemcpyDeviceToHost, b.stream);
+        if (ec == hipSuccess) ec = hipStreamSynchronize(b.stream);
+        if (ec != hipSuccess) return fail(TCGNN_ERR_HIP, "cell count: %s", hipGetErrorString(ec));
+    }
     FlatEntries ent = flat_entries(b.nwg, b.maxw, b.rbase, b.rlist, b.cnt, b.dense_mx, b.with_dense(), b.flat_tpc != 0);
     hipError_t e = hipSuccess;
     if (b.flat_tpc) {
@@ -641,7 +674,7 @@
 }
 static int cells_wavefront_cold_lists(CellBuild& b) {
     hipError_t e = hipSuccess;
-    if (!b.val && b.flat_tpc && b.cold_tiles > 0 && b.cold_tiles < (1ll << 28) && flat_cold_fits(lds_stream_nt(b.slot), b.maxw, b.flat_tpc)) {
+    if (!b.val && b.flat_tpc && b.cold_tiles > 0 && b.cold_tiles < (1ll << 28) && flat_cold_fits(lds_stream_nt(b.slot), b.maxw, b.flat_tpc, b.long_ranges())) {
         std::vector<int32_t>& wptr = b.wptr;
         std::vector<uint32_t>& wlist = b.wlist;
         wptr.assign((size_t)b.nwg * kLdsWaves + 1, 0);
@@ -725,15 +758,10 @@
                     (void*)cs.d_cold_eidx16}) (void)hipFree(q);
 }
 
-static int build_lds_cells(tcgnn_plan* p, hipStream_t stream, int slot, size_t* build_only_bytes = nullptr) {
-    static std::mutex mu;
-    std::lock_guard<std::mutex> lock(mu);
-    if (p->lds[slot].nranges > 0) return TCGNN_OK;
-    if (p->nw_eff <= 0 || p->Nc <= 0) return fail(TCGNN_ERR_INVALID_ARG, "LDS-range SpMM: empty graph");
-    CellBuild b;
+static constexpr int kLongMinEntries = 32;
+static void cells_begin(CellBuild& b, tcgnn_plan* p, hipStream_t stream, int slot) {
     b.p = p; b.stream = stream; b.slot = slot;
     b.val = slot == kLdsValSlot;
-    if (b.val && !p->d_xwb_ptr) return fail(TCGNN_ERR_INVALID_ARG, "edge-valued LDS-resident SpMM: the single-edge stream has not been built");
     b.s_wb = b.val ? p->d_xwb_ptr : p->d_wb_ptr;
     b.s_cols = b.val ? p->d_xcols : p->d_cols;
     b.s_mask = b.val ? p->d_xmask : p->d_mask;
@@ -747,12 +775,64 @@
     b.ncell = (int64_t)b.nwg * b.nranges * b.per_wg;
     b.npairs_all = (int64_t)b.nwg * b.nranges;
     b.verbose = verbose_level() > 0;
+}
+static double cells_price(const CellBuild& b) {
+    const double entries = (double)b.npairs + (b.flat_tpc == 1 ? (double)b.ndense_entries : 0.0);
+    double steps;
+    if (b.flat_tpc == 1) steps = (double)(b.npairs * b.maxw) + 1.6 * (double)b.dense_steps + 4.0 * (double)b.ndense_entries;
+    else if (b.flat_tpc == 2) steps = 2.0 * (double)(b.npairs * b.maxw);
+    else steps = (double)b.classic_steps / 0.75;
+    const double per_wg = (6.0 * entries + steps) / std::max(b.nwg, 1);
+    return per_wg + 2.0 * (double)b.trial_tiles / ((double)std::max(b.nwg, 1) * kLdsWaves) + 10.0 * (double)std::max<int64_t>(b.worst_tail, 0);
+}
+static int cells_plan(CellBuild& b) {
     if (const int rc = cells_window_weights(b)) return rc;
     if (const int rc = cells_choose_placement(b)) return rc;
     if (const int rc = cells_hot_pairs(b)) return rc;
     cells_dense_pairs(b);
     cells_flat_or_ordinary(b);
     if (const int rc = cells_hub_row_trial(b)) return rc;
+    b.price = cells_price(b);
+    return TCGNN_OK;
+}
+static int build_lds_cells(tcgnn_plan* p, hipStream_t stream, int slot, size_t* build_only_bytes = nullptr) {
+    static std::mutex mu;
+    std::lock_guard<std::mutex> lock(mu);
+    const bool two_lengths = slot == lds_stream_of(2, kLdsMaxW2) || slot == kLdsLongSlot;
+    int8_t decided = two_lengths ? p->lds_long.load(std::memory_order_acquire) : (int8_t)0;
+    if (two_lengths) slot = lds_stream_of(2, kLdsMaxW2, decided == 1);
+    if (p->lds[slot].nranges > 0) return TCGNN_OK;
+    if (p->nw_eff <= 0 || p->Nc <= 0) return fail(TCGNN_ERR_INVALID_ARG, "LDS-range SpMM: empty graph");
+    if (slot == kLdsValSlot && !p->d_xwb_ptr) return fail(TCGNN_ERR_INVALID_ARG, "edge-valued LDS-resident SpMM: the single-edge stream has not been built");
+    std::unique_ptr<CellBuild> bp(new CellBuild);
+    cells_begin(*bp, p, stream, slot);
+    if (const int rc = cells_plan(*bp)) return rc;
+    if (two_lengths && decided < 0) {
+        CellBuild& s = *bp;
+        const double cells = (double)std::max<int64_t>(s.npairs, 1) * std::min<double>(s.per_wg, std::ceil((double)p->nw_eff / std::max(s.nwg, 1)));
+        const double fill_long = (double)(s.hot_cols - s.over_dense) / cells * (double)(lds_stream_buf_rows(kLdsLongSlot) - 8) / (double)s.rows;
+        bool take_long = false;
+        const int knob = lds_long_knob();
+        if (knob == 0) { if (s.verbose) fprintf(stderr, "[tcgnn] range length: 760 rows (TCGNN_LDS_LONG=0)\n"); }
+        else if (knob < 0 && s.npairs < (int64_t)kLongMinEntries * s.nwg) {
+            if (s.verbose) fprintf(stderr, "[tcgnn] range length: 760 rows; 952-row ranges not priced: %lld entries in %d workgroups\n", (long long)s.npairs, s.nwg);
+        } else if (knob < 0 && fill_long > 30.0) {
+            if (s.verbose) fprintf(stderr, "[tcgnn] range length: 760 rows, price %.0f steps per workgroup; 952-row ranges not priced: their ordinary cells would hold %.1f columns of 32\n", s.price, fill_long);
+        } else {
+            std::unique_ptr<CellBuild> bl(new CellBuild);
+            cells_begin(*bl, p, stream, kLdsLongSlot);
+            if (const int rc = cells_plan(*bl)) return rc;
+            const bool buildable = bl->flat_tpc == 1;
+            take_long = buildable && (knob == 1 || bl->price < s.price);
+            if (s.verbose) fprintf(stderr, "[tcgnn] range length: 760 rows: %lld entries, price %.0f steps per workgroup; 952 rows: %lld entries, price %.0f%s: %d-row ranges%s\n",
+                                   (long long)(s.npairs + (s.flat_tpc == 1 ? s.ndense_entries : 0)), s.price, (long long)(bl->npairs + (bl->flat_tpc == 1 ? bl->ndense_entries : 0)), bl->price,
+                                   buildable ? "" : " (not a flat stream with one tile per cell: cannot be built)", take_long ? 952 : 760, knob == 1 ? " (TCGNN_LDS_LONG=1)" : "");
+            (void)hipStreamSynchronize(stream);
+            if (take_long) { bp = std::move(bl); slot = kLdsLongSlot; }
+        }
+        p->lds_long.store(take_long ? 1 : 0, std::memory_order_release);
+    }
+    CellBuild& b = *bp;
     if (const int rc = cells_entries(b)) return rc;
     if (b.val && b.flat_tpc != 1)
         return fail(TCGNN_ERR_UNSUPPORTED, "edge-valued LDS-resident SpMM: the single-edge cells of this graph are not uniform enough for a flat stream");
diff --git a/tc-gnn_atc23_amd/csrc/tcgnn_lds_spmm.inc b/tc-gnn_atc23_amd/csrc/tcgnn_lds_spmm.inc
--- a/tc-gnn_atc23_amd/csrc/tcgnn_lds_spmm.inc
+++ b/tc-gnn_atc23_amd/csrc/tcgnn_lds_spmm.inc
@@ -2,13 +2,14 @@
 static constexpr int kLdsWaves = 16;
 static constexpr int kLdsMaxW = 4;
 static constexpr int kLdsMaxW2 = 8;
-static constexpr int kLdsStreams = 7;
+static constexpr int kLdsStreams = 8;
 static constexpr int kLdsValSlot = 6;
-__host__ __device__ constexpr int lds_stream_of(int nt, int maxw) { return maxw == 8 ? (nt == 2 ? 4 : 5) : (nt >= 4 ? 0 : (nt == 2 ? 1 : (nt == 1 ? 2 : 3))); }
-__host__ __device__ constexpr int lds_stream_buf_rows(int slot) { return slot == 0 ? 512 : (slot == 1 ? 768 : (slot == 2 ? 1536 : (slot == 3 ? 640 : (slot == 4 || slot == 6 ? 768 : 512)))); }
+static constexpr int kLdsLongSlot = 7;
+__host__ __device__ constexpr int lds_stream_of(int nt, int maxw, bool long_ranges = false) { return maxw == 8 ? (nt == 2 ? (long_ranges ? 7 : 4) : 5) : (nt >= 4 ? 0 : (nt == 2 ? 1 : (nt == 1 ? 2 : 3))); }
+__host__ __device__ constexpr int lds_stream_buf_rows(int slot) { return slot == 7 ? 960 : (slot == 0 ? 512 : (slot == 1 ? 768 : (slot == 2 ? 1536 : (slot == 3 ? 640 : (slot == 4 || slot == 6 ? 768 : 512))))); }
 __host__ __device__ constexpr int lds_stream_maxw(int slot) { return slot >= 4 ? 8 : 4; }
-__host__ __device__ constexpr int lds_stream_nt(int slot) { return slot == 0 ? 4 : (slot == 1 ? 2 : (slot == 2 ? 1 : (slot == 3 ? 3 : (slot == 4 || slot == 6 ? 2 : 1)))); }
-__host__ __device__ constexpr int lds_buf_rows(int nt, int maxw) { return lds_stream_buf_rows(lds_stream_of(nt, maxw)); }
+__host__ __device__ constexpr int lds_stream_nt(int slot) { return slot == 0 ? 4 : (slot == 1 ? 2 : (slot == 2 ? 1 : (slot == 3 ? 3 : (slot == 4 || slot == 6 || slot == 7 ? 2 : 1)))); }
+__host__ __device__ constexpr int lds_buf_rows(int nt, int maxw, bool long_ranges = false) { return lds_stream_buf_rows(lds_stream_of(nt, maxw, long_ranges)); }
 static constexpr int lds_pad_tiles(int maxw, int buf_rows) { return maxw != 4 ? (buf_rows == 768 ? 12 : 16) : (buf_rows == 512 ? 6 : (buf_rows == 1536 ? 12 : 8)); }
 static constexpr int kCellWords = 32;
 static constexpr int lds_chunk_dims(int maxw) { return 256 / maxw; }
@@ -125,6 +126,17 @@
     const int64_t pair = idx / per_wg;
     const int k = kmap[pair];
     if (k >= 0) cnt[(int64_t)k * per_wg + (idx - pair * per_wg)] = (cellcols[idx] + 31u) / 32u;
+}
+__global__ __launch_bounds__(256) void cell_dense_stats_kernel(const uint32_t* __restrict__ cnt, int64_t npairs, int32_t maxw, uint32_t* __restrict__ extra_mx, uint32_t* __restrict__ cell_mx) {
+    const int64_t k = (int64_t)blockIdx.x * blockDim.x + threadIdx.x;
+    if (k >= npairs) return;
+    uint32_t mx = 0, cmx = 0;
+    for (int v = 0; v < kLdsWaves; ++v) {
+        uint32_t ex = 0;
+        for (int j = 0; j < maxw; ++j) { const uint32_t c = cnt[(k * kLdsWaves + v) * maxw + j]; ex += c > 1u ? c - 1u : 0u; cmx = c > cmx ? c : cmx; }
+        mx = ex > mx ? ex : mx;
+    }
+    extra_mx[k] = mx; cell_mx[k] = cmx;
 }
 __device__ __forceinline__ bool pair_is_dense(const int32_t* ent, int32_t k) { return ent && ent[2 * k + 1] >= 0; }
 __global__ __launch_bounds__(256) void cell_cold_count_kernel(const uint32_t* __restrict__ cellcols, const int32_t* __restrict__ kmap, const int32_t* __restrict__ order,
diff --git a/tc-gnn_atc23_amd/csrc/tcgnn_spmm_dispatch.inc b/tc-gnn_atc23_amd/csrc/tcgnn_spmm_dispatch.inc
--- a/tc-gnn_atc23_amd/csrc/tcgnn_spmm_dispatch.inc
+++ b/tc-gnn_atc23_amd/csrc/tcgnn_spmm_dispatch.inc
@@ -39,7 +39,7 @@
 static LdsStreamFacts lds_stream_facts(const tcgnn_plan* plan, const LdsPass* passes, int npass) {
     LdsStreamFacts f{npass > 0, false, false, false};
     for (int i = 0; i < npass; ++i) {
-        const tcgnn_plan::CellStream& ci = plan->lds[lds_stream_of(passes[i].nt, passes[i].maxw)];
+        const tcgnn_plan::CellStream& ci = plan->lds[lds_pass_slot(plan, passes[i])];
         if (ci.nranges == 0) { f.all_built = false; continue; }
         if (ci.flat_tpc) f.flat_cold = f.flat_cold || flat_cold_behind(ci);
         else f.rows_cold = f.rows_cold || ci.cold_tiles > 0;
@@ -57,7 +57,7 @@
     }
     if (f.thin && mode != 3) { *settle = true; return false; }
     if (f.rows_cold && planar_staged) return false;
-    if (f.rows_cold) *cold = &plan->lds[lds_stream_of(passes[0].nt, passes[0].maxw)];
+    if (f.rows_cold) *cold = &plan->lds[lds_pass_slot(plan, passes[0])];
     return true;
 }
 static bool stream_is_capturing(hipStream_t stream) {
@@ -72,8 +72,8 @@
 static int ensure_lds_streams(const tcgnn_plan* plan, hipStream_t stream, int mode, int dpad, const LdsPass* passes, int npass, LdsBuild who, bool* ok) {
     *ok = true;
     for (int i = 0; i < npass; ++i) {
+        if (plan->lds[lds_pass_slot(plan, passes[i])].nranges > 0) continue;
         const int slot = lds_stream_of(passes[i].nt, passes[i].maxw);
-        if (plan->lds[slot].nranges > 0) continue;
         if (who == LdsBuild::kInCall && stream_is_capturing(stream)) {
             *ok = false;
             return mode == 3 ? fail(TCGNN_ERR_INVALID_ARG, "LDS-resident SpMM: the cell stream of this width has to be built before the call is captured into a graph") : TCGNN_OK;
@@ -120,7 +120,7 @@
         int total_chunks = 0;
         for (int i = 0; i < r->npass; ++i) total_chunks += r->passes[i].nchunks;
         r->accumulate = (c.d_W && total_chunks > 1) ? 1 : 0;
-        r->own_fb = r->npass == 1 && !r->cold && !c.d_W && !staged && c.stride() == D && !flat_cold_behind(plan->lds[lds_stream_of(r->passes[0].nt, r->passes[0].maxw)]) &&
+        r->own_fb = r->npass == 1 && !r->cold && !c.d_W && !staged && c.stride() == D && !flat_cold_behind(plan->lds[lds_pass_slot(plan, r->passes[0])]) &&
                     !c.scaled();
         r->walk = Walk::kLds;
         return TCGNN_OK;
@@ -262,13 +262,14 @@
         if (const int rc = stage_features(plan, c.d_X, nullptr, D, static_cast<char*>(c.ws) + image, c.ws_bytes - image, stream, o, &rows)) return rc;
         x16_rows = rows.x16;
     }
-    const tcgnn_plan::CellStream& cs0 = plan->lds[lds_stream_of(r.passes[0].nt, r.passes[0].maxw)];
+    const tcgnn_plan::CellStream& cs0 = plan->lds[lds_pass_slot(plan, r.passes[0])];
     const SpmmSmallArgs fb = small_args(c, r.own_fb ? im.hdr : nullptr);
     KernelTimer timer(plan, stream, r.cold ? "spmm_lds_kernel + spmm_kernel (cold remainder)" :
                                     (cs0.flat_tpc ? (flat_cold_behind(cs0) ? "spmm_lds_flat_kernel + spmm_cold_planar_kernel (cold remainder)" : "spmm_lds_flat_kernel") : "spmm_lds_kernel"));
     for (int i = 0; i < r.npass; ++i) {
         const LdsPass& p = r.passes[i];
-        const tcgnn_plan::CellStream& cs = plan->lds[lds_stream_of(p.nt, p.maxw)];
+        const int slot = lds_pass_slot(plan, p);
+        const tcgnn_plan::CellStream& cs = plan->lds[slot];
         if (cs.flat_tpc) {
             const bool has_cold = flat_cold_behind(cs);
             SpmmFlatArgs f{};
@@ -276,7 +277,7 @@
             f.N = plan->N; f.D = D; f.stride = im.dpad / 16; f.chunk0 = p.chunk0; f.xrows = plan->Nc + 1; f.nw = plan->nw_eff; f.nwg = cs.nwg;
             f.dbg = g_lds_dbg; f.relu = has_cold ? 0 : c.relu; f.rbase = cs.d_rbase; f.rl2 = cs.d_rl2; f.nent = std::max(cs.npairs, 1);
             f.w = c.d_W; f.dout = c.D_out; f.accumulate = r.accumulate; f.fill_quota = g_lds_fill_quota; f.wcold_ptr = cs.d_wcold_ptr; f.wcold = cs.d_wcold; f.fb = fb;
-            HIP_TRY(launch_flat_any(p.maxw, p.nt, cs.flat_tpc, f, p.nchunks, stream, cs.dense_entries > 0, has_cold ? no_epi : epi));
+            HIP_TRY(launch_flat_any(p.maxw, p.nt, cs.flat_tpc, f, p.nchunks, stream, cs.dense_entries > 0, has_cold ? no_epi : epi, slot == kLdsLongSlot));
             if (has_cold && !(g_lds_dbg & 16)) {
                 const int cd = lds_chunk_dims(p.maxw);
                 const int col0 = p.chunk0 * cd, ncols = std::min(p.nchunks * cd, im.dpad - col0);
```

Result: faster. 219.2 GTEPS (SpMM, edges/s/1e9) (median of 6 runs) (+4.6%).
